# yardenas/ethz-safe-learning

Measured on AMD Instinct MI355X. Metric: planning steps/sec (CEM-MPC, N=2000 K=5 H=30), higher is better.
Workload: dtype f32

## Files before the change

### ethz_safe_learning_amd/_capi.py

```python
from __future__ import annotations

import ctypes as C
import os

CEM_ABI_VERSION = 4
CEM_MAX_ACT = 32
CEM_MAX_COST_KINDS = 4
CEM_COMM_ID_BYTES = 128
CEM_MAX_BATCH = 256
CEM_TRAIN_MAX_BATCH = 4096
CEM_INIT_COLD, CEM_INIT_EXPLICIT, CEM_INIT_SHIFT = 0, 1, 2
CEM_VARIANT_CEM, CEM_VARIANT_SAFE, CEM_VARIANT_COST = 0, 1, 2
CEM_PARTICLES_MEAN, CEM_PARTICLES_LOWER_TAIL = 0, 1
CEM_CONSTRAINT_BETA, CEM_CONSTRAINT_BUDGET = 0, 1
CEM_REFIT_UNIFORM, CEM_REFIT_SOFTMAX = 0, 1
CEM_NOISE_WHITE, CEM_NOISE_MIXED = 0, 1
CEM_FORWARD_SPLIT, CEM_FORWARD_ALL = 0, 1
CEM_TASK_SAFETY_GYM, CEM_TASK_QUADRATIC = 0, 1

_HERE = os.path.dirname(os.path.abspath(__file__))
LIB_PATH = os.environ.get('CEM_MPC_LIB') or os.path.join(_HERE, 'lib', 'libcem_mpc_gfx950.so')

EXPORTED_SYMBOLS = [
    'cem_abi_version', 'cem_status_string', 'cem_last_hip_error', 'cem_weight_blob_floats',
    'cem_packed_weight_floats', 'cem_workspace_bytes', 'cem_pack_weights_host', 'cem_plan_tiles_host', 'cem_plan_segments_host', 'cem_rollout_residency',
    'cem_planner_create', 'cem_planner_destroy', 'cem_planner_layout', 'cem_planner_set_weights', 'cem_planner_set_weights_dev',
    'cem_planner_set_normaliser', 'cem_planner_plan', 'cem_plan_begin', 'cem_plan_rollout', 'cem_plan_select',
    'cem_plan_end', 'cem_comm_unique_id', 'cem_planner_comm_init', 'cem_planner_comm_destroy', 'cem_planner_comm_ranks', 'cem_plan_exchange', 'cem_planner_graph_status', 'cem_planner_graph_nodes', 'cem_planner_launches_per_iteration', 'cem_planner_rollout_path', 'cem_planner_rollout_form', 'cem_unfold_sequences', 'cem_compute_objective', 'cem_scorer_reward', 'cem_scorer_cost', 'cem_fill_noise', 'cem_philox_words', 'cem_planner_set_timing', 'cem_planner_last_timing', 'cem_planner_last_timing_detail', 'cem_planner_select_mode', 'cem_planner_inject_fault',
    'cem_batch_workspace_bytes', 'cem_batch_planner_create', 'cem_planner_plan_batch', 'cem_planner_batch_capacity',
    'cem_planner_set_warm_start', 'cem_planner_set_initial_distribution', 'cem_planner_set_init_mode', 'cem_planner_reset_carry',
    'cem_planner_get_carry', 'cem_planner_set_carry_slots', 'cem_planner_set_particle_objective', 'cem_planner_get_particle_objective',
    'cem_planner_set_constraint', 'cem_planner_get_constraint', 'cem_planner_set_cost_budget', 'cem_planner_constraint_costs',
    'cem_planner_set_refit', 'cem_planner_get_refit', 'cem_planner_refit_stats',
    'cem_planner_set_action_noise', 'cem_planner_get_action_noise', 'cem_planner_action_noise_dev',
    'cem_planner_set_elite_carry', 'cem_planner_get_elite_carry', 'cem_planner_elite_store',
    'cem_planner_set_population_schedule', 'cem_planner_get_population_schedule', 'cem_planner_iteration_plan',
    'cem_planner_set_mean_candidate', 'cem_planner_get_mean_candidate',
    'cem_planner_set_plan_readout', 'cem_planner_get_plan_readout', 'cem_planner_plan_readout',
    'cem_planner_set_task', 'cem_planner_task_trajectories', 'cem_task_score',
    'cem_trainer_workspace_bytes', 'cem_trainer_blob_floats', 'cem_trainer_create', 'cem_trainer_destroy', 'cem_trainer_set_state',
    'cem_trainer_get_state', 'cem_trainer_weights_dev', 'cem_trainer_step', 'cem_trainer_steps', 'cem_trainer_eval', 'cem_trainer_forward',
]


class CemScorer(C.Structure):
    _fields_ = [
        ('goal_mode', C.c_int32), ('goal_lo', C.c_int32), ('goal_hi', C.c_int32),
        ('lidar_max_dist', C.c_float), ('goal_size', C.c_float), ('goal_reached_dist', C.c_float), ('reward_distance', C.c_float),
        ('reward_goal', C.c_float), ('reward_clip', C.c_float),
        ('constrain_indicator', C.c_int32), ('n_cost_kinds', C.c_int32),
        ('cost_lo', C.c_int32 * CEM_MAX_COST_KINDS), ('cost_hi', C.c_int32 * CEM_MAX_COST_KINDS),
        ('cost_size', C.c_float * CEM_MAX_COST_KINDS),
    ]


class CemConfig(C.Structure):
    _fields_ = [
        ('abi_version', C.c_int32), ('obs_dim', C.c_int32), ('act_dim', C.c_int32),
        ('units', C.c_int32), ('n_layers', C.c_int32), ('activation', C.c_int32), ('ensemble_size', C.c_int32),
        ('particles', C.c_int32), ('n_samples', C.c_int32), ('horizon', C.c_int32),
        ('n_elite', C.c_int32), ('iterations', C.c_int32),
        ('smoothing', C.c_float), ('one_minus_smoothing', C.c_float), ('stddev_threshold', C.c_float), ('noise_stddev', C.c_float),
        ('variant', C.c_int32), ('posterior_mean_threashold', C.c_float),
        ('sampling_propagation', C.c_int32), ('scale_features', C.c_int32),
        ('act_lb', C.c_float * CEM_MAX_ACT), ('act_ub', C.c_float * CEM_MAX_ACT),
        ('act_mu0', C.c_float * CEM_MAX_ACT), ('act_sigma0', C.c_float * CEM_MAX_ACT),
        ('scorer', CemScorer),
        ('world_size', C.c_int32), ('rank', C.c_int32), ('chunks_per_tile', C.c_int32), ('use_graph', C.c_int32),
        ('select_mode', C.c_int32), ('rollout_segments', C.c_int32), ('precision', C.c_int32),
    ]


class CemTrainConfig(C.Structure):
    _fields_ = [('abi_version', C.c_int32), ('inputs_dim', C.c_int32), ('outputs_dim', C.c_int32), ('units', C.c_int32),
                ('n_layers', C.c_int32), ('ensemble_size', C.c_int32), ('batch_size', C.c_int32), ('activation', C.c_int32),
                ('dropout_rate', C.c_float), ('dropout_seed_lo', C.c_uint32), ('dropout_seed_hi', C.c_uint32),
                ('beta1', C.c_float), ('beta2', C.c_float), ('epsilon', C.c_float), ('clipvalue', C.c_float)]


class CemWarmStart(C.Structure):
    _fields_ = [('shift', C.c_int32), ('tail', C.c_int32), ('sigma_rule', C.c_int32), ('sigma_floor', C.c_float * CEM_MAX_ACT)]


class CemEliteCarry(C.Structure):
    _fields_ = [('n_keep', C.c_int32), ('across_plans', C.c_int32), ('shift', C.c_int32), ('reserved', C.c_int32)]


class CemIterationPlan(C.Structure):
    _fields_ = [(n, C.c_int32) for n in ('n_samples', 'chunks_per_tile', 'n_tiles', 'n_segments', 'n_pinned', 'launches', 'rollout_path', 'reserved')]


class CemPlanReadout(C.Structure):
    _fields_ = [('score', C.c_float), ('candidate', C.c_int32), ('iteration', C.c_int32), ('flags', C.c_int32)]


class CemTask(C.Structure):
    _fields_ = [('kind', C.c_int32)] + [(n, C.POINTER(C.c_float)) for n in ('q', 'g', 'c', 'goal_mask', 'lo', 'hi', 'rho')] + \
               [('goal_radius', C.c_float), ('reward_goal', C.c_float), ('reward_clip', C.c_float)]


class CemLayout(C.Structure):
    _fields_ = [(n, C.c_size_t) for n in
                ('scores_local', 'scores_global', 'actions', 'mu_sigma', 'elite_idx', 'returns', 'costs', 'result', 'stamps', 'total',
                 'wpack', 'wpack_bytes', 'bias_h', 'bias_mu', 'bias_var', 'etab', 'etab_bytes')]


class CemError(RuntimeError):
    def __init__(self, status, where, lib=None):
        msg = lib.cem_status_string(status).decode() if lib is not None else str(status)
        hip = lib.cem_last_hip_error() if lib is not None else 0
        super().__init__('%s failed: status %d (%s)%s' % (where, status, msg, (', hip error %d' % hip) if status == 5 else ''))
        self.status = status


_lib = None


def load():
    global _lib
    if _lib is not None:
        return _lib
    if not os.path.exists(LIB_PATH):
        raise ImportError('HIP extension %s is missing: run `python -c "import __graft_entry__ as g; g.build()"` '
                          'or `make -C ethz_safe_learning_amd/csrc`. There is no CPU fallback.' % LIB_PATH)
    import torch
    lib = C.CDLL(LIB_PATH)
    vp, fp, i32p = C.c_void_p, C.POINTER(C.c_float), C.POINTER(C.c_int32)
    cfgp = C.POINTER(CemConfig)
    lib.cem_abi_version.restype = C.c_int
    lib.cem_status_string.restype = C.c_char_p
    lib.cem_status_string.argtypes = [C.c_int]
    lib.cem_last_hip_error.restype = C.c_int
    for f in ('cem_weight_blob_floats', 'cem_packed_weight_floats', 'cem_workspace_bytes'):
        getattr(lib, f).restype = C.c_size_t
        getattr(lib, f).argtypes = [cfgp]
    lib.cem_pack_weights_host.argtypes = [cfgp, vp, vp]
    lib.cem_plan_tiles_host.argtypes = [cfgp, i32p, i32p, vp, C.c_int32]
    lib.cem_plan_segments_host.argtypes = [cfgp, i32p, i32p]
    lib.cem_rollout_residency.argtypes = [C.c_int32, C.c_int32, i32p, i32p]
    lib.cem_planner_create.argtypes = [cfgp, vp, C.c_size_t, vp, C.POINTER(vp)]
    lib.cem_planner_destroy.argtypes = [vp]
    lib.cem_planner_layout.argtypes = [vp, C.POINTER(CemLayout)]
    lib.cem_planner_set_weights.argtypes = [vp, vp, C.c_size_t]
    lib.cem_planner_set_weights_dev.argtypes = [vp, vp, C.c_size_t]
    lib.cem_planner_set_normaliser.argtypes = [vp, vp, vp]
    lib.cem_planner_plan.argtypes = [vp, vp, C.c_uint64, C.c_uint64, vp, vp, vp, vp, fp, i32p]
    lib.cem_plan_begin.argtypes = [vp, vp, C.c_uint64, C.c_uint64, vp, vp]
    lib.cem_plan_rollout.argtypes = [vp, C.c_int32]
    lib.cem_plan_select.argtypes = [vp, C.c_int32]
    lib.cem_plan_end.argtypes = [vp, vp, vp, fp, i32p]
    lib.cem_unfold_sequences.argtypes = [vp, vp, vp, C.c_int32, C.c_int32, vp, C.c_uint64, C.c_uint64, vp, vp, vp]
    lib.cem_comm_unique_id.argtypes = [vp]
    lib.cem_planner_comm_init.argtypes = [vp, vp, C.c_int32, C.c_int32]
    lib.cem_planner_comm_destroy.argtypes = [vp]
    lib.cem_plan_exchange.argtypes = [vp]
    lib.cem_planner_graph_status.argtypes = [vp, i32p]
    lib.cem_planner_graph_nodes.argtypes = [vp, i32p]
    lib.cem_planner_comm_ranks.argtypes = [vp, i32p]
    lib.cem_planner_launches_per_iteration.argtypes = [vp, i32p]
    lib.cem_planner_rollout_path.argtypes = [vp, i32p]
    lib.cem_planner_rollout_form.argtypes = [vp, C.c_int32, i32p]
    lib.cem_compute_objective.argtypes = [vp, vp, C.c_int32, C.c_int32, vp]
    lib.cem_scorer_reward.argtypes = [vp, vp, vp, C.c_int32, vp, vp]
    lib.cem_scorer_cost.argtypes = [vp, vp, C.c_int32, vp]
    lib.cem_fill_noise.argtypes = [vp, C.c_uint64, C.c_uint64, vp, vp, vp]
    lib.cem_philox_words.argtypes = [vp, C.c_uint64, C.c_uint64] + [C.c_uint32] * 6 + [vp]
    lib.cem_planner_select_mode.argtypes = [vp, i32p]
    lib.cem_planner_inject_fault.argtypes = [vp, C.c_int32]
    lib.cem_planner_set_timing.argtypes = [vp, C.c_int32]
    lib.cem_planner_last_timing.argtypes = [vp, fp, i32p, fp]
    lib.cem_planner_last_timing_detail.argtypes = [vp, fp, fp]
    lib.cem_batch_workspace_bytes.restype = C.c_size_t
    lib.cem_batch_workspace_bytes.argtypes = [cfgp, C.c_int32]
    lib.cem_batch_planner_create.argtypes = [cfgp, C.c_int32, vp, C.c_size_t, vp, C.POINTER(vp)]
    lib.cem_planner_plan_batch.argtypes = [vp, C.c_int32, vp, C.c_uint64, vp, vp, vp, vp, vp, vp, vp]
    lib.cem_planner_batch_capacity.argtypes = [vp, i32p]
    lib.cem_planner_set_warm_start.argtypes = [vp, C.POINTER(CemWarmStart)]
    lib.cem_planner_set_initial_distribution.argtypes = [vp, C.c_int32, vp, vp]
    lib.cem_planner_set_init_mode.argtypes = [vp, C.c_int32, C.c_int32]
    lib.cem_planner_reset_carry.argtypes = [vp, C.c_int32]
    lib.cem_planner_get_carry.argtypes = [vp, C.c_int32, vp, vp, i32p]
    lib.cem_planner_set_carry_slots.argtypes = [vp, C.c_int32, vp]
    lib.cem_planner_set_particle_objective.argtypes = [vp, C.c_int32, C.c_int32]
    lib.cem_planner_get_particle_objective.argtypes = [vp, i32p, i32p]
    lib.cem_planner_set_constraint.argtypes = [vp, C.c_int32, C.c_int32]
    lib.cem_planner_get_constraint.argtypes = [vp, i32p, i32p]
    lib.cem_planner_set_cost_budget.argtypes = [vp, vp, C.c_int32]
    lib.cem_planner_constraint_costs.argtypes = [vp, C.c_int32, vp, C.c_int32]
    lib.cem_planner_set_refit.argtypes = [vp, C.c_int32, C.c_float]
    lib.cem_planner_get_refit.argtypes = [vp, i32p, fp]
    lib.cem_planner_refit_stats.argtypes = [vp, C.c_int32, vp, C.c_int32]
    lib.cem_planner_set_action_noise.argtypes = [vp, C.c_int32, vp]
    lib.cem_planner_get_action_noise.argtypes = [vp, i32p, vp]
    lib.cem_planner_action_noise_dev.argtypes = [vp, C.POINTER(vp), C.POINTER(C.c_size_t)]
    lib.cem_planner_set_elite_carry.argtypes = [vp, C.POINTER(CemEliteCarry)]
    lib.cem_planner_get_elite_carry.argtypes = [vp, C.POINTER(CemEliteCarry)]
    lib.cem_planner_elite_store.argtypes = [vp, C.c_int32, vp, i32p]
    lib.cem_planner_set_population_schedule.argtypes = [vp, i32p, C.c_int32]
    lib.cem_planner_get_population_schedule.argtypes = [vp, i32p, C.c_int32, i32p]
    lib.cem_planner_iteration_plan.argtypes = [vp, C.c_int32, C.POINTER(CemIterationPlan)]
    lib.cem_planner_set_mean_candidate.argtypes = [vp, C.c_int32]
    lib.cem_planner_get_mean_candidate.argtypes = [vp, i32p]
    lib.cem_planner_set_plan_readout.argtypes = [vp, C.c_int32]
    lib.cem_planner_get_plan_readout.argtypes = [vp, i32p]
    lib.cem_planner_plan_readout.argtypes = [vp, C.c_int32, C.POINTER(CemPlanReadout), vp, vp, vp]
    lib.cem_planner_set_task.argtypes = [vp, C.POINTER(CemTask)]
    lib.cem_planner_task_trajectories.argtypes = [vp, vp]
    lib.cem_task_score.argtypes = [vp, vp, vp, C.c_int32, C.c_int32, vp, vp]
    tcfgp = C.POINTER(CemTrainConfig)
    for f in ('cem_trainer_workspace_bytes', 'cem_trainer_blob_floats'):
        getattr(lib, f).restype = C.c_size_t
        getattr(lib, f).argtypes = [tcfgp]
    lib.cem_trainer_create.argtypes = [tcfgp, vp, C.c_size_t, vp, C.POINTER(vp)]
    lib.cem_trainer_destroy.argtypes = [vp]
    lib.cem_trainer_set_state.argtypes = [vp, vp, vp, vp]
    lib.cem_trainer_get_state.argtypes = [vp, vp, vp, vp]
    lib.cem_trainer_weights_dev.argtypes = [vp, C.POINTER(vp), C.POINTER(C.c_size_t)]
    lib.cem_trainer_step.argtypes = [vp, vp, vp, vp, C.c_int32, C.c_int32, C.c_int32, C.c_float, vp]
    lib.cem_trainer_steps.argtypes = [vp, vp, vp, vp, C.c_int32, C.c_int32, vp, vp, vp, vp]
    lib.cem_trainer_eval.argtypes = [vp, vp, vp, C.c_int32, fp]
    lib.cem_trainer_forward.argtypes = [vp, vp, C.c_int32, C.c_int32, vp, C.c_uint64, C.c_uint64, vp, vp, vp, vp]
    for name in EXPORTED_SYMBOLS:
        fn = getattr(lib, name)
        if name not in ('cem_status_string', 'cem_weight_blob_floats', 'cem_packed_weight_floats', 'cem_workspace_bytes',
                        'cem_batch_workspace_bytes', 'cem_trainer_workspace_bytes', 'cem_trainer_blob_floats'):
            fn.restype = C.c_int
    if lib.cem_abi_version() != CEM_ABI_VERSION:
        raise ImportError('ABI mismatch: library %d, binding %d' % (lib.cem_abi_version(), CEM_ABI_VERSION))
    _lib = lib
    return lib


def check(status, where):
    if status != 0:
        raise CemError(status, where, _lib)
```

### ethz_safe_learning_amd/csrc/cem_capi.hip

```cpp
#include "cem_device.h"
#include "cem_rollout_lean.h"
#include "cem_score.h"
#include "cem_refit_weighted.h"
#include "cem_noise_mix.h"
#include "cem_elite_carry.h"
#include "cem_plan_readout.h"
#include "cem_task_score.h"
#include "cem_population.h"
#include "cem_train.h"
#include "cem_train_tile.h"
#include "cem_forward.h"
#include "cem_rollout_split.h"
#include "cem_rollout_bf16.h"
#include "cem_rollout_wide.h"
#include "cem_pack.h"
#include "../../include/cem_mpc.h"
#include "cem_plan_options.h"

#include <dlfcn.h>
#include <link.h>

#include <algorithm>
#include <atomic>
#include <chrono>
// ... 464 lines not shown
    pl.n_seg = (d.H + pl.seg_len - 1) / pl.seg_len;
    pl.n_pinned = pl.n_seg > 1 ? (pl.n_tiles / num_cus()) * num_cus() : pl.n_tiles;
    if (c->rollout_segments > 1 && pl.n_pinned == pl.n_tiles && pl.n_seg > 1) pl.n_pinned = 0;
    return pl;
}

Layout make_layout(const cem_config_t *c, const Dims &d, size_t max_tiles, int mb = 0)
{
    Layout l{}; size_t o = 0;
    const size_t nb = mb > 0 ? (size_t)mb : 1;
    auto take = [&](size_t bytes) { size_t r = o; o = align256(o + bytes); return r; };
    l.ctrl = take(nb * sizeof(CtrlBlock));
    l.musig = take(nb * 2 * d.H * d.A * 4);
    l.act_bounds = take(64 * 4);
    l.scores_local = take(nb * d.Nloc * 4);
    l.scores_global = d.W > 1 ? take((size_t)d.N * 4) : l.scores_local;
    l.actions = take(nb * d.N * d.H * d.A * 4);
    l.act_pad = take(nb * d.N * d.H * d.act_nq * 16);
    l.elite = take(nb * d.k * 4);
    l.returns = take(nb * d.Bloc * 4);
    l.costs = take(nb * d.H * d.Bloc);
    l.result = take(mb > 0 ? nb * CEM_RESULT_WORDS * 4 : 64 * 4);
    l.wpack = take(d.wide ? (size_t)d.E * (align256(d.nat_member_floats * 4) + wide_image_floats(d) * 4) : (size_t)d.E * d.member_stride_f4 * 16);
    l.bias_h = take((size_t)d.E * d.L * CEM_U * 4);
    l.bias_mu = take((size_t)d.E * CEM_U * 4);
    l.bias_var = take((size_t)d.E * CEM_U * 4);
    l.nmin = take(CEM_U * 4);
    l.ndelta = take(CEM_U * 4);
    l.omask = take(2 * CEM_U * 4);
    l.kind_sel = take(CEM_NKIND * CEM_U * 4);
    l.etab = take((size_t)d.E * etab_rows(d) * CEM_U * 4);
    l.tiles = take(max_tiles * sizeof(TileDesc));
    l.eps_out = take(nb * CEM_MAX_ACT * 4);
    l.stamps = take(std::max<size_t>(max_tiles * 4 * 8, 128) * sizeof(long long));
    const Plan pl = make_plan(c, d);
    l.seg_queue = take(256);
    const size_t n_float = (size_t)(pl.n_tiles - pl.n_pinned);
    l.seg_flags = take(std::max<size_t>(n_float * std::max(pl.n_seg - 1, 1), 1) * 4);
    l.seg_state = take(pl.n_seg > 1 ? std::max<size_t>(n_float, 1) * (2 * d.NFW * pl.rc * 256 + 64) * 16 : 16);
    const size_t msG = ((size_t)d.N + CEM_MS_KEYS - 1) / CEM_MS_KEYS, msG2 = ((size_t)d.k + CEM_MS_EPG - 1) / CEM_MS_EPG;
    l.ms_hist = take(3 * CEM_MS_BINS * 4); l.ms_sel = take(256);
    l.ms_counts = take(msG * 2 * 4); l.ms_best_sc = take(msG * 4); l.ms_best_ix = take(msG * 4);
    l.ms_part = take(2 * msG2 * (size_t)d.H * d.A * 4); l.ms_colmean = take((size_t)d.H * d.A * 4);
    l.carry = take(nb * 2 * d.H * d.A * 4); l.expl = take(nb * 2 * d.H * d.A * 4);
    l.total = o;
    return l;
}

size_t max_tiles_of(const Dims &d) { std::vector<Tile6> t; build_plan_tiles(d, 1, t); return t.size(); }

int validate_batch(const cem_config_t *c, int32_t mb)
{
    const int st = validate(c); if (st) return st;
    if (mb < 1 || mb > CEM_MAX_BATCH) return CEM_ERR_INVALID_ARG;
    if (c->world_size > 1 || c->precision != CEM_PRECISION_FP32) return CEM_ERR_UNSUPPORTED;
    const Dims d = make_dims(c);
    if (d.wide) return CEM_ERR_UNSUPPORTED;
    if (c->select_mode == 2 || c->select_mode == 3) return CEM_ERR_UNSUPPORTED;
    if (resolve_select_mode(c->select_mode, d.N, d.k, (long long)d.H * d.A, 140 * 1024, true, nullptr) != 1) return CEM_ERR_UNSUPPORTED;
    if ((long long)mb * (long long)max_tiles_of(d) > 0x7fffffffll) return CEM_ERR_UNSUPPORTED;
    return CEM_OK;
}

}

namespace {
struct CemNcclId { char internal[CEM_COMM_ID_BYTES]; };
struct Rccl {
    void *lib = nullptr;
    int (*GetUniqueId)(CemNcclId *) = nullptr;
    int (*CommInitRank)(void **, int, CemNcclId, int) = nullptr;
    int (*CommDestroy)(void *) = nullptr;
    int (*AllGather)(const void *, void *, size_t, int, void *, hipStream_t) = nullptr;
    int (*CommCount)(void *, int *) = nullptr;
};
Rccl *rccl()
{
    static Rccl r;
    static std::once_flag once;
    std::call_once(once, [] {
        if (const char *over = std::getenv("CEM_RCCL_LIBRARY")) {
            r.lib = dlopen(over, RTLD_NOW | RTLD_LOCAL);
            if (!r.lib) std::fprintf(stderr, "cem_mpc: CEM_RCCL_LIBRARY=%s: %s\n", over, dlerror());
        } else {
            for (const char *name : {"librccl.so.1", "librccl.so", "/opt/rocm/lib/librccl.so.1"}) {
                r.lib = dlopen(name, RTLD_NOW | RTLD_LOCAL);
                if (r.lib) break;
            }
        }
        if (r.lib) {
            r.GetUniqueId = (decltype(r.GetUniqueId))dlsym(r.lib, "ncclGetUniqueId");
            r.CommInitRank = (decltype(r.CommInitRank))dlsym(r.lib, "ncclCommInitRank");
            r.CommDestroy = (decltype(r.CommDestroy))dlsym(r.lib, "ncclCommDestroy");
            r.AllGather = (decltype(r.AllGather))dlsym(r.lib, "ncclAllGather");
            r.CommCount = (decltype(r.CommCount))dlsym(r.lib, "ncclCommCount");
            if (!r.GetUniqueId || !r.CommInitRank || !r.CommDestroy || !r.AllGather) r.lib = nullptr;
        }
        if (const char *over = std::getenv("CEM_RCCL_LIBRARY"))
            std::fprintf(stderr, r.lib ? "cem_mpc: RCCL entry points bound from CEM_RCCL_LIBRARY=%s%s\n" : "cem_mpc: CEM_RCCL_LIBRARY=%s lacks a required entry point%s\n",
                         over, (r.lib && !r.CommCount) ? " (no ncclCommCount: cem_planner_comm_ranks unavailable)" : "");
    });
    return r.lib ? &r : nullptr;
}
const int kNcclFloat32 = 7;
}
#define NCCLCHK(x) do { int e_ = (x); if (e_ != 0) { g_last_hip = e_; return CEM_ERR_COMM; } } while (0)

namespace {
int count_hip_runtimes(struct dl_phdr_info *info, size_t, void *data)
{
    if (info->dlpi_name && std::strstr(info->dlpi_name, "libamdhip64")) {
        auto *v = static_cast<std::vector<std::string> *>(data);
        if (std::find(v->begin(), v->end(), std::string(info->dlpi_name)) == v->end()) v->push_back(info->dlpi_name);
    }
    return 0;
}
void warn_if_two_hip_runtimes()
{
    static std::once_flag once;
    std::call_once(once, [] {
        std::vector<std::string> libs;
        dl_iterate_phdr(count_hip_runtimes, &libs);
        if (libs.size() > 1) {
            std::fprintf(stderr, "cem_mpc: %zu HIP runtimes are loaded in this process:", libs.size());
            for (const auto &l : libs) std::fprintf(stderr, " %s", l.c_str());
            std::fprintf(stderr, "\ncem_mpc: device memory and streams of one are foreign to the other — load libcem_mpc_gfx950.so AFTER the runtime that owns them (INTEGRATION.md)\n");
        }
    });
}
}

struct IterPlan {
    Dims d;
    int rc, n_tiles, n_seg, seg_len, n_pinned;
    bool sample_in_rollout, lean_rollout;
    size_t tiles_off;
};

struct cem_planner {
    cem_config_t cfg;
    Dims d;
    Layout lay;
    char *ws;
    hipStream_t stream;
    bool own_stream;
    int rc;
    int n_tiles;
    int n_seg, seg_len, n_pinned;
    bool have_weights;
    bool in_plan;
    bool sample_in_rollout;
    bool lean_rollout;
    bool lean_branchy;
    const float *eps_act, *eps_model;
    CtrlBlock *h_ctrl;
    float *h_result;
    WarmCtl *h_warm; const WarmCtl *d_h_warm;
    uint32_t plan_seq;
    const CtrlBlock *d_h_ctrl; float *d_h_result;
    bool timing; std::vector<hipEvent_t> ev; float roll_ms, sel_ms, red_ms, samp_ms; int roll_n;
    std::vector<std::pair<int, int>> ev_kind;
    hipGraph_t graph; hipGraphExec_t gexec; bool graph_ready;
    ScorerDev sc;
    ScorerDev sc_roll;
    float alpha, beta;
    void *comm;
    int plans_since_comm;
    bool graph_failed;
    size_t sel_dyn_limit;
    int fused_resident;
    bool sel_zeroed;
    bool fuse_banned;
    bool inject_capture_fail;
    uint32_t inject_next;
    char *scratch; size_t scratch_bytes;
    std::vector<float> h_etab;
    PackDesc *pack_desc; uint32_t n_pack_desc;
    int batch;
    int n_states;
    cem_warm_start_t warm;
    std::vector<int32_t> slot_mode;
    std::vector<uint8_t> carry_valid, have_expl;
    std::vector<int32_t> carry_at;
    std::vector<int32_t> slot_of;
    bool warm_save_skipped;
    int warm_staged;
    std::vector<float> h_expl;
    PlanOptions opt;
    float *budget_dev;
    std::vector<float> h_budget;
    float *cstat_obj; size_t cstat_obj_n;
    const float *last_cstat; int last_cstat_n, last_cstat_problems;
    float refit_beta;
    float *refit_dev;
    bool refit_ran;
    std::vector<float> h_mix, h_mix_t;
    float *noise_dev;
    float *noise_eps; size_t noise_floats;
    float *elite_dev;
    int elite_cap;
    bool elite_clear;
    std::vector<IterPlan> pop;
    char *pop_dev;
    uint32_t *pop_seg_flags; f4 *pop_seg_state;
    int pop_n_ready;
    uint32_t *readout_dev;
    float *task_dev;
    TaskScoreParams task;
};

namespace {

int warm_slots(const cem_planner *h) { return h->batch ? h->batch : 1; }

struct IterView {
    const Dims *d; int rc, n_tiles, n_seg, seg_len, n_pinned; bool sample_in_rollout, lean_rollout;
    const TileDesc *tiles; uint32_t *seg_flags; f4 *seg_state;
};
IterView iter_view(const cem_planner *h, int it)
{
    const Layout &l = h->lay;
    if (h->pop.empty())
        return IterView{&h->d, h->rc, h->n_tiles, h->n_seg, h->seg_len, h->n_pinned, h->sample_in_rollout, h->lean_rollout,
                        (const TileDesc *)(h->ws + l.tiles), (uint32_t *)(h->ws + l.seg_flags), (f4 *)(h->ws + l.seg_state)};
    const IterPlan &ip = h->pop[std::min(std::max(it, 0), h->d.I - 1)];
    return IterView{&ip.d, ip.rc, ip.n_tiles, ip.n_seg, ip.seg_len, ip.n_pinned, ip.sample_in_rollout, ip.lean_rollout,
                    ip.tiles_off == (size_t)-1 ? (const TileDesc *)(h->ws + l.tiles) : (const TileDesc *)(h->pop_dev + ip.tiles_off),
                    h->pop_seg_flags, h->pop_seg_state};
}

int lean_form(const cem_planner *h, int it)
{
    const Dims &d = *iter_view(h, it).d; const ScorerDev &sc = h->sc_roll;
    bool straight = launch_rollout_lean_straight != nullptr && !h->lean_branchy && !sc.goal_mode && sc.n_cost <= 1 && d.L == 4 && d.NFW == 1;
    for (int w = 0; w < 4; ++w) straight = straight && d.wave_groups[w] == 4 + 3 * CEM_NG + (w < d.KB_obs ? CEM_NG : 0);
    return straight ? 2 : 1;
}
size_t task_tab_floats() { return (size_t)CEM_TASK_TABLES * CEM_U; }
float *task_traj(const cem_planner *h) { return h->task_dev + task_tab_floats(); }
int32_t *elite_counts(const cem_planner *h) { return reinterpret_cast<int32_t *>(h->elite_dev); }
size_t elite_count_floats(const cem_planner *h) { return ((size_t)warm_slots(h) + 63) & ~(size_t)63; }
float *elite_store(const cem_planner *h) { return h->elite_dev + elite_count_floats(h); }

int select_mode_for(const cem_planner *h, int N, bool *cache = nullptr)
{
    const Dims &d = h->d;
    const bool can_fuse = (N + CEM_MS_KEYS - 1) / CEM_MS_KEYS <= h->fused_resident && !h->fuse_banned;
    return resolve_select_mode(h->cfg.select_mode, N, d.k, (long long)d.H * d.A, h->sel_dyn_limit, can_fuse, cache);
}
int select_mode_now(const cem_planner *h, bool *cache = nullptr) { return select_mode_for(h, h->d.N, cache); }

void drop_graph(cem_planner *h)
{
    if (h->gexec) { hipGraphExecDestroy(h->gexec); h->gexec = nullptr; }
    if (h->graph) { hipGraphDestroy(h->graph); h->graph = nullptr; }
    h->graph_ready = false;
}

struct LaunchRecipe {
    bool sampler_launch;
    bool inject_elites, inject_mean;
    int lean_form;
    bool fold_reduce;
    int select_mode; bool select_cache;
    bool one_workgroup_only;
    bool weighted, keep_elites, track;
    bool task;
};
LaunchRecipe recipe_of(const cem_planner *h, int it, bool own_noise)
{
    const IterView v = iter_view(h, it); const PlanOptions &o = h->opt;
    LaunchRecipe r{};
    r.inject_elites = o.elite.n_keep != 0;
    r.inject_mean = o.mean_cand && it == h->d.I - 1;
    r.task = o.task != 0;
    const bool rewritten = r.inject_elites || r.inject_mean || r.task;
    r.sampler_launch = !v.sample_in_rollout || rewritten;
    r.lean_form = v.lean_rollout && !rewritten && !own_noise && o.noise_kind != CEM_NOISE_MIXED ? lean_form(h, it) : 0;
    r.select_mode = select_mode_for(h, v.d->N, &r.select_cache);
    r.fold_reduce = h->d.W == 1 && !h->comm && h->cfg.variant == CEM_VARIANT_CEM && !o.tail_m && r.select_mode == 1 && r.select_cache;
    r.weighted = o.refit_kind == CEM_REFIT_SOFTMAX; r.keep_elites = o.elite.n_keep != 0; r.track = o.readout != 0;
    r.one_workgroup_only = r.weighted || r.keep_elites || r.track || !h->pop.empty();
    return r;
}

int launches_of(const cem_planner *h, int it)
{
    const LaunchRecipe r = recipe_of(h, it, false);
    return 1 + r.sampler_launch + r.inject_elites + r.inject_mean + !r.fold_reduce + (r.select_mode == 2 ? 8 : r.select_mode == 3 ? 2 : 1) +
           r.weighted + r.keep_elites + r.track + r.task;
}

PlanOptions options_of(const cem_planner *h) { PlanOptions o = h->opt; o.comm = h->comm != nullptr; return o; }

constexpr long long kBudgetTotalLimit = 1ll << 23;

HandleFacts facts_of(const cem_planner *h, const PlanOptions &next)
{
    const Dims &d = h->d;
    HandleFacts f;
    f.W = d.W; f.batch = h->batch; f.variant = h->cfg.variant; f.N = d.N; f.k = d.k; f.H = d.H; f.A = d.A; f.I = d.I; f.P = d.P;
    f.select_mode = select_mode_now(h);
    for (int32_t n : next.pop) f.pop_select_mode.push_back(select_mode_for(h, n));
    f.tail_max_p = CEM_TAIL_MAX_P; f.budget_max_tail_p = CEM_BUDGET_MAX_TAIL_P; f.elite_max_k = CEM_ELITE_MAX_K; f.mix_max_h = CEM_MIX_MAX_H;
    f.readout_max_p = CEM_READOUT_MAX_P; f.max_cost_kinds = CEM_MAX_COST_KINDS; f.budget_total_limit = kBudgetTotalLimit;
    f.refit_lds_bytes = CEM_REFIT_LDS_BYTES(d.k, d.H * d.A); f.refit_lds_limit = h->sel_dyn_limit;
    f.can_mix = launch_mix_action_noise && prepare_mix_action_noise; f.can_carry = launch_elite_keep && launch_elite_inject;
    f.can_mean = launch_mean_candidate != nullptr; f.can_track = launch_plan_track != nullptr; f.can_task = launch_task_score != nullptr;
    return f;
}
int admit_on(const cem_planner *h, const PlanOptions &next, PlanChange change = PLAN_CHANGE_OTHER) { return admit(facts_of(h, next), next, change); }

template <typename SwapIn>
int commit_launch_change(cem_planner *h, PlanOptions &next, bool always, SwapIn swap_in)
{
    if (always || h->graph_ready) HIPCHK(hipStreamSynchronize(h->stream));
    if (const int st = swap_in()) return st;
    drop_graph(h);
    h->opt = std::move(next);
    return CEM_OK;
}
int commit_launch_change(cem_planner *h, PlanOptions &next, bool always) { return commit_launch_change(h, next, always, [] { return (int)CEM_OK; }); }

struct DevBlock {
    void *p = nullptr;
    DevBlock() = default;
    DevBlock(const DevBlock &) = delete; DevBlock &operator=(const DevBlock &) = delete;
    ~DevBlock() { if (p) hipFree(p); }
    hipError_t alloc(size_t bytes) { return hipMalloc(&p, bytes); }
    template <typename T> T *release() { T *q = static_cast<T *>(p); p = nullptr; return q; }
};

void release_handle(cem_planner *h)
{
    if (h->h_ctrl) hipHostFree(h->h_ctrl);
    if (h->h_result) hipHostFree(h->h_result);
    if (h->h_warm) hipHostFree(h->h_warm);
    if (h->pack_desc) hipFree(h->pack_desc);
    if (h->budget_dev) hipFree(h->budget_dev);
    if (h->refit_dev) hipFree(h->refit_dev);
    if (h->noise_dev) hipFree(h->noise_dev);
    if (h->elite_dev) hipFree(h->elite_dev);
    if (h->readout_dev) hipFree(h->readout_dev);
    if (h->task_dev) hipFree(h->task_dev);
    if (h->pop_dev) hipFree(h->pop_dev);
    if (h->cstat_obj) hipFree(h->cstat_obj);
    if (h->own_stream) hipStreamDestroy(h->stream);
    delete h;
}

}

extern "C" {

int cem_abi_version(void) { return CEM_ABI_VERSION; }
int cem_last_hip_error(void) { return g_last_hip; }

const char *cem_status_string(int s)
{
    switch (s) {
    case CEM_OK: return "ok";
    case CEM_ERR_INVALID_ARG: return "invalid argument";
    case CEM_ERR_UNSUPPORTED: return "unsupported configuration (units <= 256, obs+act <= 128, task 'goal')";
    case CEM_ERR_SPLIT: return "particles*n_samples is not divisible by ensemble_size (tf.split would raise)";
    case CEM_ERR_WORKSPACE: return "workspace too small or misaligned";
    case CEM_ERR_HIP: return "HIP runtime error (see cem_last_hip_error)";
    case CEM_ERR_NO_WEIGHTS: return "set_weights has not been called";
    case CEM_ERR_STATE: return "stepwise plan calls out of order, or a standalone call while a plan is in flight";
    case CEM_ERR_COMM: return "RCCL: library not found or a collective call failed (see cem_last_hip_error for the ncclResult_t)";
    case CEM_ERR_DEVICE: return "a kernel could not finish its work (a floating rollout segment starved of its work-queue entry, or an expired fused-select barrier whose recovery did not run): result not valid";
    default: return "unknown status";
    }
}

size_t cem_weight_blob_floats(const cem_config_t *cfg)
{
    if (validate(cfg) != CEM_OK) return 0;
    const Dims d = make_dims(cfg);
    return d.nat_member_floats * d.E;
}

size_t cem_packed_weight_floats(const cem_config_t *cfg)
{
    if (validate(cfg) != CEM_OK) return 0;
    const Dims d = make_dims(cfg);
    if (d.wide) return 0;
    return (size_t)d.member_stride_f4 * 4 * d.E;
}

size_t cem_workspace_bytes(const cem_config_t *cfg)
{
    if (validate(cfg) != CEM_OK) return 0;
    const Dims d = make_dims(cfg);
    return make_layout(cfg, d, max_tiles_of(d)).total;
}

int cem_pack_weights_host(const cem_config_t *cfg, const float *blob, float *packed)
{
    int st = validate(cfg); if (st) return st;
    if (!blob || !packed) return CEM_ERR_INVALID_ARG;
    const Dims d = make_dims(cfg);
    if (d.wide) return CEM_ERR_UNSUPPORTED;
    for (int m = 0; m < d.E; ++m) {
        if (d.chunked()) pack_member_chunked(d, blob + (size_t)m * d.nat_member_floats, reinterpret_cast<uint16_t *>(packed + (size_t)m * d.member_stride_f4 * 4));
        else pack_member(d, blob + (size_t)m * d.nat_member_floats, packed + (size_t)m * d.member_stride_f4 * 4);
    }
    return CEM_OK;
}

int cem_plan_tiles_host(const cem_config_t *cfg, int32_t *rc_out, int32_t *n_tiles_out, int32_t *tiles_out, int32_t max_tiles)
{
    int st = validate(cfg); if (st) return st;
    const Dims d = make_dims(cfg);
    const int rc = make_plan(cfg, d).rc;
    std::vector<Tile6> t; build_plan_tiles(d, rc, t);
    if (rc_out) *rc_out = rc;
    if (n_tiles_out) *n_tiles_out = (int32_t)t.size();
    if (tiles_out) {
        if ((int)t.size() > max_tiles) return CEM_ERR_INVALID_ARG;
        std::memcpy(tiles_out, t.data(), t.size() * sizeof(Tile6));
    }
    return CEM_OK;
}

int cem_plan_segments_host(const cem_config_t *cfg, int32_t *segments_out, int32_t *steps_per_segment_out)
{
    int st = validate(cfg); if (st) return st;
    const Dims d = make_dims(cfg);
    const Plan pl = make_plan(cfg, d);
    if (segments_out) *segments_out = pl.n_seg;
    if (steps_per_segment_out) *steps_per_segment_out = pl.seg_len;
    return CEM_OK;
}

int cem_rollout_residency(int32_t chunks_per_tile, int32_t input_blocks_per_wave, int32_t *table_out, int32_t *runtime_out)
{
    if (chunks_per_tile < 1 || chunks_per_tile > 4 || input_blocks_per_wave < 1 || input_blocks_per_wave > 2) return CEM_ERR_INVALID_ARG;
    for (int seg = 0; seg < 2; ++seg) {
        if (table_out) table_out[seg] = kResidentStatic[seg][input_blocks_per_wave - 1][chunks_per_tile - 1];
        if (runtime_out)
            runtime_out[seg] = with_tile_shape(chunks_per_tile, input_blocks_per_wave, 0, [&](auto R, auto F) { return query_resident<R(), F()>(seg != 0); });
    }
    return CEM_OK;
}

}

static bool lean_eligible(const cem_planner *h, const Dims &d, int rc, bool sample_in_rollout)
{
    return launch_rollout_lean != nullptr && !d.wide && !d.chunked() && rc == 1 && d.NFW == 1 && d.L == 4 && d.O % 4 == 0 && h->cfg.world_size == 1 && !h->batch &&
           sample_in_rollout && CEM_LEAN_ACT_LDS_BYTES(d.H, (d.A + 3) / 4) <= CEM_LEAN_ACT_LDS_MAX;
}

static void place_sampler(const cem_planner *h, const Dims &d, const Plan &pl, bool *sample_in_rollout, bool *lean_rollout)
{
    const size_t nb = (size_t)warm_slots(h);
    const int slots = real_cus() * ((d.wide || d.chunked()) ? 1 : resident_workgroups(d.NFW, pl.rc, pl.n_seg > 1));
    *sample_in_rollout = (long long)nb * pl.n_tiles <= slots;
    if (const char *e = std::getenv("CEM_FORCE_SAMPLER"))
        *sample_in_rollout = std::strcmp(e, "kernel") != 0;
    *lean_rollout = lean_eligible(h, d, pl.rc, *sample_in_rollout);
    if (const char *e = std::getenv("CEM_FORCE_ROLLOUT"))
        *lean_rollout = *lean_rollout && std::strcmp(e, "generic") != 0;
}

static int planner_create(const cem_config_t *cfg, int32_t mb, void *workspace, size_t workspace_bytes, void *hip_stream, cem_planner_t **out)
{
    int st = mb ? validate_batch(cfg, mb) : validate(cfg); if (st) return st;
    if (!workspace || !out) return CEM_ERR_INVALID_ARG;
    if (cfg->precision == CEM_PRECISION_BF16 && (launch_rollout_bf16 == nullptr || launch_pack_bf16 == nullptr)) return CEM_ERR_UNSUPPORTED;
    warn_if_two_hip_runtimes();
    cem_planner *h = new (std::nothrow) cem_planner();
    if (!h) return CEM_ERR_INVALID_ARG;
    h->cfg = *cfg; h->d = make_dims(cfg);
    h->batch = mb; h->n_states = warm_slots(h);
    const size_t nb = (size_t)warm_slots(h);
    h->lay = make_layout(cfg, h->d, max_tiles_of(h->d), mb);
    if (workspace_bytes < h->lay.total || ((uintptr_t)workspace & 255)) { delete h; return CEM_ERR_WORKSPACE; }
    h->ws = (char *)workspace; h->stream = (hipStream_t)hip_stream; h->own_stream = false;
    if (!h->stream) {
        if (hipStreamCreateWithFlags(&h->stream, hipStreamNonBlocking) != hipSuccess) { g_last_hip = (int)hipGetLastError(); delete h; return CEM_ERR_HIP; }
        h->own_stream = true;
    }
    { const Plan pl = make_plan(cfg, h->d, mb); h->rc = pl.rc; h->n_seg = pl.n_seg; h->seg_len = pl.seg_len; h->n_pinned = pl.n_pinned;
      place_sampler(h, h->d, pl, &h->sample_in_rollout, &h->lean_rollout); }
    { const char *e = std::getenv("CEM_FORCE_ROLLOUT"); h->lean_branchy = e && std::strcmp(e, "lean_branchy") == 0; }
    h->have_weights = false; h->in_plan = false; h->eps_act = h->eps_model = nullptr;
    h->timing = false; h->roll_ms = h->sel_ms = h->red_ms = h->samp_ms = 0.f; h->roll_n = 0;
    h->graph = nullptr; h->gexec = nullptr; h->graph_ready = false;
    h->budget_dev = nullptr; h->cstat_obj = nullptr; h->cstat_obj_n = 0; h->last_cstat = nullptr; h->last_cstat_n = h->last_cstat_problems = 0;
    h->refit_beta = 0.f; h->refit_dev = nullptr; h->refit_ran = false;
    h->noise_dev = nullptr; h->noise_eps = nullptr; h->noise_floats = 0;
    h->elite_dev = nullptr; h->elite_cap = 0; h->elite_clear = false;
    h->readout_dev = nullptr;
    h->task_dev = nullptr; h->task = TaskScoreParams{};
    h->pop_dev = nullptr; h->pop_seg_flags = nullptr; h->pop_seg_state = nullptr; h->pop_n_ready = 0;
    h->h_budget.assign(nb, std::numeric_limits<float>::infinity());
    h->comm = nullptr; h->plans_since_comm = 0; h->graph_failed = false;
    h->h_ctrl = nullptr; h->h_result = nullptr; h->h_warm = nullptr; h->d_h_warm = nullptr; h->pack_desc = nullptr; h->n_pack_desc = 0;
    h->warm = cem_warm_start_t{}; h->warm.shift = 1; h->warm_staged = 0; h->warm_save_skipped = false;
    h->slot_mode.assign(nb, CEM_INIT_COLD); h->carry_valid.assign(nb, 0); h->have_expl.assign(nb, 0); h->carry_at.assign(nb, -1);
    h->slot_of.resize(nb); for (size_t b = 0; b < nb; ++b) h->slot_of[b] = (int32_t)b;
    h->h_expl.assign(nb * 2 * h->d.H * h->d.A, 0.f);
    h->scratch = nullptr; h->scratch_bytes = 0; h->sel_zeroed = false; h->plan_seq = 0; h->fuse_banned = false; h->inject_next = 0; h->inject_capture_fail = false;
    auto fail = [&](int status) { g_last_hip = (int)hipGetLastError(); release_handle(h); return status; };
    const size_t result_bytes = mb ? nb * CEM_RESULT_WORDS * 4 : 64 * 4;
    if (hipHostMalloc((void **)&h->h_ctrl, nb * sizeof(CtrlBlock), hipHostMallocMapped | hipHostMallocCoherent) != hipSuccess ||
        hipHostMalloc((void **)&h->h_result, result_bytes, hipHostMallocMapped | hipHostMallocCoherent) != hipSuccess ||
        hipHostMalloc((void **)&h->h_warm, sizeof(WarmCtl) + nb * sizeof(WarmProb), hipHostMallocMapped | hipHostMallocCoherent) != hipSuccess) return fail(CEM_ERR_HIP);
    {
        const std::vector<PackDesc> table = build_pack_table(h->d);
        h->n_pack_desc = (uint32_t)table.size();
        const size_t image_bytes = h->d.wide ? wide_image_floats(h->d) * 4 : (size_t)h->d.member_stride_f4 * 16 - 4096;
        if (table.size() * (h->d.group_bytes() / 2) != image_bytes) return fail(CEM_ERR_STATE);
        if (hipMalloc((void **)&h->pack_desc, table.size() * sizeof(PackDesc)) != hipSuccess ||
            hipMemcpy(h->pack_desc, table.data(), table.size() * sizeof(PackDesc), hipMemcpyHostToDevice) != hipSuccess) return fail(CEM_ERR_HIP);
    }
    std::memset(h->h_warm, 0, sizeof(WarmCtl) + nb * sizeof(WarmProb));
    std::memset(h->h_ctrl, 0, nb * sizeof(CtrlBlock));
    std::memset(h->h_result, 0, result_bytes);
    {
        void *dc = nullptr, *dr = nullptr, *dw = nullptr;
        if (hipHostGetDevicePointer(&dc, h->h_ctrl, 0) != hipSuccess || hipHostGetDevicePointer(&dr, h->h_result, 0) != hipSuccess ||
            hipHostGetDevicePointer(&dw, h->h_warm, 0) != hipSuccess) return fail(CEM_ERR_HIP);
        h->d_h_ctrl = (const CtrlBlock *)dc; h->d_h_result = (float *)dr; h->d_h_warm = (const WarmCtl *)dw;
    }
    auto upload = [&](size_t off, const void *src, size_t bytes) {
        return hipMemcpyAsync(h->ws + off, src, bytes, hipMemcpyHostToDevice, h->stream) == hipSuccess;
    };

    const cem_scorer_t &s = cfg->scorer;
    ScorerDev &sc = h->sc;
    sc.goal_mode = s.goal_mode; sc.goal_lo = s.goal_lo; sc.goal_hi = s.goal_hi; sc.D = s.lidar_max_dist;
    sc.goal_thresh = s.goal_reached_dist;
    sc.reward_distance = s.reward_distance; sc.reward_goal = s.reward_goal; sc.reward_clip = s.reward_clip;
    sc.indicator = s.constrain_indicator; sc.n_cost = s.n_cost_kinds;
    for (int i = 0; i < 4; ++i) { sc.cost_lo[i] = s.cost_lo[i]; sc.cost_hi[i] = s.cost_hi[i]; sc.cost_size[i] = s.cost_size[i]; }
    h->sc_roll = sc;
    if (cfg->variant == CEM_VARIANT_COST) h->sc_roll.goal_thresh = -std::numeric_limits<float>::infinity();
    {
        const float mu = 0.5f, sg = 0.27f;
        const float alpha = (((1.0f - mu) / (sg * sg)) - 1.0f / mu) * (mu * mu);
        h->alpha = alpha; h->beta = alpha * (1.0f / mu - 1.0f);
    }

    std::vector<Tile6> tiles; build_plan_tiles(h->d, h->rc, tiles);
    h->n_tiles = (int)tiles.size();
    const Dims &d = h->d;
    std::vector<float> om(2 * CEM_U, 0.f), ks(CEM_NKIND * CEM_U, std::numeric_limits<float>::infinity());
    const float ninf = -std::numeric_limits<float>::infinity();
    for (int f = 0; f < CEM_U; ++f) {
        om[f] = f < d.O ? 1.f : 0.f;
        om[CEM_U + f] = (f >= d.O && f < d.O + d.A) ? 1.f : 0.f;
        const int ghi = s.goal_mode ? s.goal_lo + 1 : s.goal_hi;
        if (f >= s.goal_lo && f < ghi && f < d.O) ks[f] = ninf;
        for (int k = 0; k < s.n_cost_kinds; ++k)
            if (f >= s.cost_lo[k] && f < s.cost_hi[k] && f < d.O) ks[(k + 1) * CEM_U + f] = ninf;
    }
    std::vector<float> mn(CEM_U, 0.f), dl(CEM_U, 1.f);
    const size_t et_rows = etab_rows(d);
    h->h_etab.assign((size_t)d.E * et_rows * CEM_U, 0.f);
    for (int m = 0; m < d.E; ++m) {
        float *et = &h->h_etab[(size_t)m * et_rows * CEM_U];
        for (int f = 0; f < CEM_U; ++f) {
            et[CEM_ET_RDELTA * CEM_U + f] = 1.f;
            et[CEM_ET_OBS * CEM_U + f] = om[f]; et[CEM_ET_ACT * CEM_U + f] = om[CEM_U + f];
            et[CEM_ET_SEL0 * CEM_U + f] = ks[f]; et[CEM_ET_SEL1 * CEM_U + f] = ks[CEM_U + f];
        }
    }
    float bounds[64] = {0.f};
    for (int a = 0; a < d.A; ++a) { bounds[a] = cfg->act_lb[a]; bounds[32 + a] = cfg->act_ub[a]; }
    if (!upload(h->lay.act_bounds, bounds, sizeof(bounds)) ||
        !upload(h->lay.tiles, tiles.data(), tiles.size() * sizeof(Tile6)) || !upload(h->lay.omask, om.data(), om.size() * 4) ||
        !upload(h->lay.kind_sel, ks.data(), ks.size() * 4) || !upload(h->lay.nmin, mn.data(), CEM_U * 4) ||
        !upload(h->lay.ndelta, dl.data(), CEM_U * 4) || !upload(h->lay.etab, h->h_etab.data(), h->h_etab.size() * 4) ||
        hipMemsetAsync(h->ws + h->lay.act_pad, 0, nb * d.N * d.H * d.act_nq * 16, h->stream) != hipSuccess ||
        hipStreamSynchronize(h->stream) != hipSuccess)
        return fail(CEM_ERR_HIP);

    h->sel_dyn_limit = 48 * 1024;
    if (hipFuncSetAttribute(reinterpret_cast<const void *>(&cem_select_kernel<true, false>), hipFuncAttributeMaxDynamicSharedMemorySize,
                            140 * 1024) == hipSuccess &&
        hipFuncSetAttribute(reinterpret_cast<const void *>(&cem_select_kernel<true, true>), hipFuncAttributeMaxDynamicSharedMemorySize,
                            140 * 1024) == hipSuccess &&
        hipFuncSetAttribute(reinterpret_cast<const void *>(&cem_select_kernel<false, false>), hipFuncAttributeMaxDynamicSharedMemorySize,
                            140 * 1024) == hipSuccess) h->sel_dyn_limit = 140 * 1024;
    else (void)hipGetLastError();
    {
        int per_cu = 0;
        if (hipOccupancyMaxActiveBlocksPerMultiprocessor(&per_cu, cem_msel_fused_kernel, 1024, 0) != hipSuccess || per_cu < 1) { (void)hipGetLastError(); per_cu = 0; }
        h->fused_resident = per_cu * real_cus();
    }
    if (mb && select_mode_now(h) != 1) { release_handle(h); return CEM_ERR_UNSUPPORTED; }
    *out = h;
    return CEM_OK;
}

extern "C" {

int cem_planner_create(const cem_config_t *cfg, void *workspace, size_t workspace_bytes, void *hip_stream, cem_planner_t **out)
{
    return planner_create(cfg, 0, workspace, workspace_bytes, hip_stream, out);
}

size_t cem_batch_workspace_bytes(const cem_config_t *cfg, int32_t max_batch)
{
    if (validate_batch(cfg, max_batch) != CEM_OK) return 0;
    const Dims d = make_dims(cfg);
    return make_layout(cfg, d, max_tiles_of(d), max_batch).total;
}

int cem_batch_planner_create(const cem_config_t *cfg, int32_t max_batch, void *workspace, size_t workspace_bytes, void *hip_stream,
                             cem_planner_t **out)
{
    const int st = validate_batch(cfg, max_batch); if (st) return st;
    return planner_create(cfg, max_batch, workspace, workspace_bytes, hip_stream, out);
}

int cem_planner_batch_capacity(const cem_planner_t *h, int32_t *max_batch_out)
{
    if (!h || !max_batch_out) return CEM_ERR_INVALID_ARG;
    *max_batch_out = h->batch;
    return CEM_OK;
}

int cem_planner_destroy(cem_planner_t *h)
{
    if (!h) return CEM_ERR_INVALID_ARG;
    if (hipStreamSynchronize(h->stream) != hipSuccess) (void)hipGetLastError();
    if (h->scratch) hipFree(h->scratch);
    if (h->comm) { if (Rccl *r = rccl()) r->CommDestroy(h->comm); h->comm = nullptr; }
    drop_graph(h);
    for (auto e : h->ev) hipEventDestroy(e);
    release_handle(h);
    return CEM_OK;
}

int cem_planner_layout(const cem_planner_t *h, cem_layout_t *o)
{
// ... 168 lines not shown
    else hipLaunchKernelGGL(cem_rollout_wide_kernel<1>, dim3(n_tiles), dim3(256), CEM_WIDE_SMEM, h->stream, wp);
    return hipGetLastError();
}

void fill_rollout_common(const cem_planner *h, RolloutParams &p, const Dims *dv = nullptr)
{
    const Dims &d = dv ? *dv : h->d; const Layout &l = h->lay; char *ws = h->ws;
    std::memset(&p, 0, sizeof(p));
    p.wpack = (const f4 *)(ws + l.wpack); p.bias_h = (const float *)(ws + l.bias_h);
    p.bias_mu = (const float *)(ws + l.bias_mu); p.bias_var = (const float *)(ws + l.bias_var);
    p.nmin = (const float *)(ws + l.nmin); p.nrdelta = (const float *)(ws + l.ndelta);
    p.omask = (const float *)(ws + l.omask); p.kind_sel = (const float *)(ws + l.kind_sel);
    p.etab = (const float *)(ws + l.etab);
    p.act_pad = (const f4 *)(ws + l.act_pad); p.act_pad_bytes = (uint32_t)((size_t)d.N * d.H * d.act_nq * 16); p.act_q0 = d.act_q0; p.act_nq = d.act_nq;
    p.ctrl = (const CtrlBlock *)(ws + l.ctrl);
    p.member_stride_f4 = d.member_stride_f4;
    for (int w = 0; w < 4; ++w) { p.wave_off_f4[w] = d.wave_off_f4[w]; p.wave_groups[w] = (uint32_t)d.wave_groups[w]; }
    p.O = d.O; p.A = d.A; p.L = d.L; p.KB_in = d.KB_in; p.KB_obs = d.KB_obs;
    p.sampling = h->cfg.sampling_propagation; p.sc = h->sc_roll;
}

hipEvent_t get_event(cem_planner *h, size_t i)
{
    while (h->ev.size() <= i) { hipEvent_t e; hipEventCreate(&e); h->ev.push_back(e); }
    return h->ev[i];
}

struct TimedLaunch {
    cem_planner *h; size_t e0;
    TimedLaunch(cem_planner *h_, int kind) : h(h_->timing ? h_ : nullptr), e0(0)
    {
        if (!h) return;
        e0 = h->ev_kind.size() * 2; h->ev_kind.push_back({(int)e0, kind}); hipEventRecord(get_event(h, e0), h->stream);
    }
    void stop() { if (h) hipEventRecord(get_event(h, e0 + 1), h->stream); h = nullptr; }
    ~TimedLaunch() { stop(); }
};

void warm_handed_over(cem_planner *h);

int enqueue_begin(cem_planner *h)
{
    const Dims &d = h->d; const Layout &l = h->lay;
    InitParams ip{}; ip.ctrl = (CtrlBlock *)(h->ws + l.ctrl); ip.musig = (float *)(h->ws + l.musig); ip.HA = d.H * d.A; ip.A = d.A;
    ip.host_ctrl = h->d_h_ctrl;
    for (int a = 0; a < d.A; ++a) { ip.mu0[a] = h->cfg.act_mu0[a]; ip.sigma0[a] = h->cfg.act_sigma0[a]; }
    if (!h->pop.empty()) {
        if (h->pop_n_ready > 0) { ip.seg_queue = (uint32_t *)(h->ws + l.seg_queue); ip.seg_flags = h->pop_seg_flags; ip.n_ready = h->pop_n_ready; }
    } else
    if (h->n_seg > 1) { ip.seg_queue = (uint32_t *)(h->ws + l.seg_queue); ip.seg_flags = (uint32_t *)(h->ws + l.seg_flags); ip.n_ready = (h->n_tiles - h->n_pinned) * (h->n_seg - 1); }
    ip.n_prob = h->batch;
    ip.warm = h->d_h_warm; ip.carry = (float *)(h->ws + l.carry); ip.expl = (const float *)(h->ws + l.expl);
    const int n = warm_slots(h) * std::max<int>(ip.HA, (int)(sizeof(CtrlBlock) / 4));
    hipLaunchKernelGGL(cem_init_kernel, dim3((n + 255) / 256), dim3(256), 0, h->stream, ip);
    HIPCHK(hipGetLastError());
    if (h->opt.noise_kind == CEM_NOISE_MIXED && !h->eps_act) {
        MixParams mp{}; mp.mix_t = h->noise_dev; mp.eps = h->noise_eps; mp.ctrl = (const CtrlBlock *)(h->ws + l.ctrl);
        mp.I = d.I; mp.N = d.N; mp.H = d.H; mp.A = d.A;
        HIPCHK(launch_mix_action_noise(mp, warm_slots(h), h->stream));
    }
    {
        hipStreamCaptureStatus cs = hipStreamCaptureStatusNone;
        if (hipStreamIsCapturing(h->stream, &cs) != hipSuccess) { (void)hipGetLastError(); cs = hipStreamCaptureStatusNone; }
        if (cs == hipStreamCaptureStatusNone) warm_handed_over(h);
    }
    return CEM_OK;
}

void note_plan_cstat(cem_planner *h)
{
    const int nb = warm_slots(h);
    h->last_cstat = h->budget_dev + nb; h->last_cstat_n = h->d.Nloc; h->last_cstat_problems = nb;
}

ReduceParams fill_score(const cem_planner *h, const float *ret, const uint8_t *costs, float *scores, float *cstat, int Nloc, int H, int check_done, bool clear_select)
{
    ReduceParams p{}; p.ret = ret; p.costs = costs; p.scores = scores; p.ctrl = (const CtrlBlock *)(h->ws + h->lay.ctrl);
    p.Nloc = Nloc; p.P = h->d.P; p.H = H; p.variant = h->cfg.variant; p.check_done = check_done;
    p.alpha = h->alpha; p.beta = h->beta; p.thr = h->cfg.posterior_mean_threashold;
    if (clear_select) { p.zero = (uint32_t *)(h->ws + h->lay.ms_hist); p.zero_n = CEM_MS_CLEAR_BYTES / 4; }
    p.m = h->opt.cost_m ? h->opt.cost_m : h->opt.tail_m; p.cstat = cstat; p.budget = h->budget_dev;
    return p;
}

hipError_t launch_score(const cem_planner *h, const ReduceParams &p, int n_problems)
{
    const dim3 grid((p.Nloc + 63) / 64, n_problems), block(CEM_SCORE_THREADS);
    if (h->cfg.variant == CEM_VARIANT_COST) hipLaunchKernelGGL(cem_constraint_reduce_kernel, grid, block, 0, h->stream, p);
    else if (h->opt.cost_m) hipLaunchKernelGGL(cem_constrained_budget_kernel, grid, block, CEM_BUDGET_LDS_BYTES(p.P, p.m), h->stream, p);
    else if (h->opt.tail_m) hipLaunchKernelGGL(cem_constraint_tail_kernel, grid, block, CEM_TAIL_LDS_BYTES(p.P), h->stream, p);
    else hipLaunchKernelGGL(cem_reduce_kernel, grid, block, 0, h->stream, p);
    return hipGetLastError();
}

EliteCarryParams fill_elite(const cem_planner *h, int it)
{
    const IterView v = iter_view(h, it);
    const Dims &d = *v.d; const Layout &l = h->lay; char *ws = h->ws;
    EliteCarryParams ep{}; ep.scores = (const float *)(ws + l.scores_global); ep.actions = (float *)(ws + l.actions); ep.act_pad = (float *)(ws + l.act_pad);
    ep.ctrl = (const CtrlBlock *)(ws + l.ctrl); ep.elite_idx = (const int32_t *)(ws + l.elite); ep.store = elite_store(h); ep.count = elite_counts(h);
    ep.N = d.N; ep.k = d.k; ep.m = h->opt.elite.n_keep; ep.H = d.H; ep.A = d.A; ep.it = it; ep.shift = h->opt.elite.across_plans ? h->opt.elite.shift : 0;
    ep.pad_shift = d.O - 4 * d.act_q0; ep.pad_floats = 4 * d.act_nq;
    return ep;
}

int enqueue_rollout(cem_planner *h, int it, bool whole_plan)
{
    const LaunchRecipe rc = recipe_of(h, it, h->eps_act || h->eps_model);
    const IterView v = iter_view(h, it);
    const Dims &d = *v.d; const Layout &l = h->lay; char *ws = h->ws;
    const bool queued = v.n_seg > 1 && !h->eps_model && !rc.task;
    if (rc.task && !h->task_dev) return CEM_ERR_UNSUPPORTED;
    RolloutParams rp; fill_rollout_common(h, rp, v.d);
    rp.tiles = v.tiles; rp.s0 = nullptr; rp.actions = (const float *)(ws + l.actions);
    rp.eps_model = h->eps_model ? h->eps_model + (size_t)it * d.H * h->d.Btot * d.O : nullptr;
    const bool cost_obj = h->cfg.variant == CEM_VARIANT_COST;
    rp.ret = (float *)(ws + l.returns); rp.costs = h->cfg.variant != CEM_VARIANT_CEM ? (uint8_t *)(ws + l.costs) : nullptr;
    rp.H = d.H; rp.Bloc = d.Bloc; rp.Btot = d.Btot; rp.it = it; rp.variant = cost_obj ? (int)CEM_VARIANT_SAFE : h->cfg.variant; rp.check_done = 1;
    rp.stamps = (long long *)(ws + l.stamps);
    const float *eps_act = h->eps_act ? h->eps_act : (h->opt.noise_kind == CEM_NOISE_MIXED ? h->noise_eps : nullptr);
    rp.musig = (const float *)(ws + l.musig); rp.eps_act = eps_act ? eps_act + (size_t)it * h->d.N * d.H * d.A : nullptr;
    rp.act_bounds = (const float *)(ws + l.act_bounds); rp.actions_w = (float *)(ws + l.actions); rp.act_pad_w = (float *)(ws + l.act_pad);
    rp.pad_shift = d.O - 4 * d.act_q0; rp.pad_floats = 4 * d.act_nq; rp.N = d.N; rp.Nloc = d.Nloc; rp.n_off = d.n_off; rp.n_tiles = v.n_tiles;
    const int nb = warm_slots(h);
    rp.tiles_per_problem = h->batch ? v.n_tiles : 0;
    rp.eps_act_pstride = (long long)d.I * h->d.N * d.H * d.A; rp.eps_model_pstride = (long long)d.I * d.H * h->d.Btot * d.O;
    if (rc.sampler_launch) {
        const int total = d.N * d.H * ((d.A + 3) / 4);
        TimedLaunch timed(h, 3);
        hipLaunchKernelGGL(cem_sample_kernel, dim3(std::min((total + 255) / 256, 2048), nb), dim3(256), 0, h->stream, rp);
        HIPCHK(hipGetLastError());
        rp.musig = nullptr;
        if (rc.inject_elites && (it > 0 || h->opt.elite.across_plans)) {
            EliteCarryParams ep = fill_elite(h, it);
            HIPCHK(launch_elite_inject(ep, nb, h->stream));
        }
        if (rc.inject_mean) {
            MeanCandidateParams mc{}; mc.musig = (const float *)(ws + l.musig); mc.act_bounds = rp.act_bounds; mc.ctrl = rp.ctrl;
            mc.actions = rp.actions_w; mc.act_pad = rp.act_pad_w; mc.N = d.N; mc.row = d.N - 1; mc.H = d.H; mc.A = d.A;
            mc.pad_shift = rp.pad_shift; mc.pad_floats = rp.pad_floats;
            HIPCHK(launch_mean_candidate(mc, nb, h->stream));
        }
    }
    const bool mode1 = rp.eps_model || rc.task;
    if (rc.task) rp.traj = task_traj(h);
    TimedLaunch timed(h, 0);
    const auto queue_grid = [&] {
        rp.seg_queue = (uint32_t *)(ws + l.seg_queue); rp.seg_flags = v.seg_flags; rp.seg_state = v.seg_state;
        rp.seg_len = v.seg_len; rp.n_seg = v.n_seg; rp.n_pinned = v.n_pinned;
        return v.n_pinned + v.n_seg * (v.n_tiles - v.n_pinned);
    };
    if (rc.lean_form) {
        const int grid = queued ? queue_grid() : v.n_tiles;
        if (rc.lean_form == 2 && (rp.variant == 1) == (rp.costs != nullptr)) HIPCHK(launch_rollout_lean_straight(rp, grid, h->stream, queued));
        else HIPCHK(launch_rollout_lean(rp, grid, h->stream, queued));
    }
    else if (d.wide) HIPCHK(launch_rollout_wide(h, rp, v.n_tiles, mode1 ? 1 : 0));
    else if (d.chunked()) HIPCHK(launch_rollout_chunked(d, v.rc, mode1 ? 1 : 0, rp, v.n_tiles, h->stream));
    else if (mode1) HIPCHK(launch_rollout<1>(v.rc, d.NFW, rp, nb * v.n_tiles, h->stream));
    else if (queued) HIPCHK(launch_rollout_seg(v.rc, d.NFW, rp, queue_grid(), h->stream));
    else HIPCHK(launch_rollout<0>(v.rc, d.NFW, rp, nb * v.n_tiles, h->stream));
    timed.stop();
    if (rc.task) {
        TaskScoreParams tp = h->task;
        tp.traj = rp.traj; tp.actions = rp.actions; tp.ctrl = rp.ctrl; tp.ret = rp.ret; tp.costs = rp.costs;
        tp.rows = d.Bloc; tp.N = d.N; tp.H = d.H; tp.O = d.O; tp.A = d.A; tp.variant = rp.variant; tp.check_done = 1;
        if (cost_obj) tp.r2 = 0.f;
        TimedLaunch timed_task(h, 2);
        HIPCHK(launch_task_score(tp, h->stream));
    }
    if (whole_plan && rc.fold_reduce) return CEM_OK;

    const ReduceParams sp = fill_score(h, rp.ret, rp.costs, (float *)(ws + l.scores_local), h->opt.cost_m ? h->budget_dev + nb : nullptr, d.Nloc, d.H, 1, true);
    h->sel_zeroed = true;
    if (h->opt.cost_m) note_plan_cstat(h);
    TimedLaunch timed_reduce(h, 2);
    HIPCHK(launch_score(h, sp, nb));
    return CEM_OK;
}

int enqueue_select(cem_planner *h, int it, bool whole_plan, bool have_eps_out = false, bool *folded = nullptr)
{
    if (folded) *folded = false;
    const LaunchRecipe rc = recipe_of(h, it, h->eps_act || h->eps_model);
    const bool fold_reduce = whole_plan && rc.fold_reduce, fold_final = whole_plan;
    const Dims &d = *iter_view(h, it).d; const Layout &l = h->lay; char *ws = h->ws;
    SelectParams p{}; p.scores = (const float *)(ws + l.scores_global); p.actions = (const float *)(ws + l.actions);
    p.musig = (float *)(ws + l.musig); p.ctrl = (CtrlBlock *)(ws + l.ctrl); p.elite_idx = (int32_t *)(ws + l.elite);
    p.N = d.N; p.k = d.k; p.HA = d.H * d.A; p.A = d.A; p.check_done = 1;
    p.smoothing = h->cfg.smoothing; p.one_minus_smoothing = h->cfg.one_minus_smoothing; p.threshold = h->cfg.stddev_threshold;
    p.stamps = (long long *)(ws + l.stamps) + 64;
    if (fold_reduce) { p.ret = (const float *)(ws + l.returns); p.P = d.P; p.scores_w = (float *)(ws + l.scores_local); }
    size_t lds = (size_t)((d.k + 3) & ~3) * 4 + (size_t)2 * d.H * d.A * 4;
    const int G = (d.N + CEM_MS_KEYS - 1) / CEM_MS_KEYS;
    const int mode = rc.select_mode; const bool cache = rc.select_cache;
    if (mode == 0) return CEM_ERR_UNSUPPORTED;
    const bool weighted = rc.weighted;
    if (rc.one_workgroup_only && (mode != 1 || (weighted && !h->refit_dev) || (rc.keep_elites && !h->elite_dev) || (rc.track && !h->readout_dev))) return CEM_ERR_UNSUPPORTED;
    if (weighted) { p.musig = h->refit_dev; p.threshold = -std::numeric_limits<float>::infinity(); }
    TimedLaunch timed(h, 1);
    if (mode >= 2) {
        MSelParams m{}; m.scores = p.scores; m.actions = p.actions; m.musig = p.musig; m.ctrl = p.ctrl; m.elite_idx = p.elite_idx;
        m.hist = (uint32_t *)(ws + l.ms_hist); m.sel = (uint32_t *)(ws + l.ms_sel); m.wg_counts = (uint32_t *)(ws + l.ms_counts);
        m.bar = m.sel + 8;
        m.best_sc = (float *)(ws + l.ms_best_sc); m.best_ix = (int32_t *)(ws + l.ms_best_ix);
        m.part = (float *)(ws + l.ms_part); m.colmean = (float *)(ws + l.ms_colmean);
        m.N = d.N; m.k = d.k; m.HA = p.HA; m.A = d.A; m.check_done = 1; m.smoothing = p.smoothing; m.one_minus_smoothing = p.one_minus_smoothing; m.threshold = p.threshold;
        m.G = G; m.G2 = (d.k + CEM_MS_EPG - 1) / CEM_MS_EPG;
        if (!h->sel_zeroed) HIPCHK(hipMemsetAsync(m.hist, 0, CEM_MS_CLEAR_BYTES, h->stream));
        h->sel_zeroed = false;
        if (mode == 3) {
            hipLaunchKernelGGL(cem_msel_fused_kernel, dim3(m.G), dim3(1024), 0, h->stream, m);
            hipLaunchKernelGGL(cem_msel_solo_kernel, dim3(1), dim3(1024), 0, h->stream, m);
        } else {
            hipLaunchKernelGGL(cem_msel_hist_kernel<0>, dim3(m.G), dim3(1024), 0, h->stream, m);
            hipLaunchKernelGGL(cem_msel_hist_kernel<1>, dim3(m.G), dim3(1024), 0, h->stream, m);
            hipLaunchKernelGGL(cem_msel_hist_kernel<2>, dim3(m.G), dim3(1024), 0, h->stream, m);
            hipLaunchKernelGGL(cem_msel_count_kernel, dim3(m.G), dim3(1024), 0, h->stream, m);
            hipLaunchKernelGGL(cem_msel_compact_kernel, dim3(m.G), dim3(1024), 0, h->stream, m);
            hipLaunchKernelGGL(cem_msel_moments_kernel<0>, dim3(m.G2), dim3(256), 0, h->stream, m);
            hipLaunchKernelGGL(cem_msel_moments_kernel<1>, dim3(m.G2), dim3(256), 0, h->stream, m);
            hipLaunchKernelGGL(cem_msel_final_kernel, dim3(1), dim3(256), 0, h->stream, m);
        }
    } else {
        if (fold_final && !h->batch && !weighted) {
            p.is_last = it == d.I - 1;
            p.result = h->d_h_result; p.result_dev = (uint32_t *)(ws + l.result); p.eps_out = have_eps_out ? (const float *)(ws + l.eps_out) : nullptr; p.noise_stddev = h->cfg.noise_stddev;
            if (folded) *folded = true;
        }
        if (cache) lds += (size_t)CEM_SEL_KWORDS(d.N) * 4;
        const dim3 grid(warm_slots(h));
        if (cache && h->cfg.variant != CEM_VARIANT_CEM) hipLaunchKernelGGL((cem_select_kernel<true, true>), grid, dim3(1024), lds, h->stream, p);
        else if (cache) hipLaunchKernelGGL((cem_select_kernel<true, false>), grid, dim3(1024), lds, h->stream, p);
        else hipLaunchKernelGGL((cem_select_kernel<false, false>), grid, dim3(1024), lds, h->stream, p);
        if (weighted) {
            HIPCHK(hipGetLastError());
            RefitWeightedParams rw{}; rw.scores = p.scores; rw.actions = p.actions; rw.musig = (float *)(ws + l.musig); rw.ctrl = p.ctrl; rw.elite_idx = p.elite_idx;
            rw.stat = h->refit_dev + (size_t)warm_slots(h) * 2 * p.HA;
            rw.N = d.N; rw.k = d.k; rw.HA = p.HA; rw.I = d.I; rw.beta = h->refit_beta;
            rw.smoothing = p.smoothing; rw.one_minus_smoothing = p.one_minus_smoothing; rw.threshold = h->cfg.stddev_threshold;
            HIPCHK(launch_refit_weighted(rw, warm_slots(h), h->stream));
            h->refit_ran = true;
        }
        if (rc.keep_elites) {
            HIPCHK(hipGetLastError());
            const EliteCarryParams ep = fill_elite(h, it);
            HIPCHK(launch_elite_keep(ep, warm_slots(h), h->stream));
        }
        if (rc.track) {
            HIPCHK(hipGetLastError());
            PlanTrackParams tp{}; tp.scores = p.scores; tp.actions = p.actions; tp.ret = (const float *)(ws + l.returns);
            tp.costs = h->cfg.variant != CEM_VARIANT_CEM ? (const uint8_t *)(ws + l.costs) : nullptr;
            tp.ctrl = p.ctrl; tp.elite_idx = p.elite_idx; tp.block = h->readout_dev;
            tp.N = d.N; tp.k = d.k; tp.H = d.H; tp.A = d.A; tp.P = d.P; tp.it = it; tp.stride = (int32_t)CEM_READOUT_WORDS(h->d.H, h->d.A, h->d.P);
            HIPCHK(launch_plan_track(tp, warm_slots(h), h->stream));
        }
    }
    HIPCHK(hipGetLastError());
    return CEM_OK;
}

int enqueue_exchange(cem_planner *h)
{
    if (!h->comm) return CEM_OK;
    Rccl *r = rccl(); if (!r) return CEM_ERR_COMM;
    const Dims &d = h->d; const Layout &l = h->lay;
    NCCLCHK(r->AllGather(h->ws + l.scores_local, h->ws + l.scores_global, (size_t)d.Nloc, kNcclFloat32, h->comm, h->stream));
    return CEM_OK;
}

int enqueue_end(cem_planner *h, bool have_eps_out)
{
    const Dims &d = h->d; const Layout &l = h->lay; char *ws = h->ws;
    if (h->batch) {
        FinalBatchParams fb{}; fb.ctrl = (const CtrlBlock *)(ws + l.ctrl); fb.eps_out = have_eps_out ? (const float *)(ws + l.eps_out) : nullptr;
        fb.result = h->d_h_result; fb.result_dev = (uint32_t *)(ws + l.result); fb.A = d.A; fb.n_prob = h->batch; fb.noise_stddev = h->cfg.noise_stddev;
        hipLaunchKernelGGL(cem_final_batch_kernel, dim3(1), dim3(256), 0, h->stream, fb);
        HIPCHK(hipGetLastError());
        return CEM_OK;
    }
    FinalParams fp{}; fp.ctrl = (const CtrlBlock *)(ws + l.ctrl); fp.eps_out = have_eps_out ? (const float *)(ws + l.eps_out) : nullptr;
    fp.result = h->d_h_result; fp.result_dev = (uint32_t *)(ws + l.result); fp.A = d.A; fp.noise_stddev = h->cfg.noise_stddev;
    hipLaunchKernelGGL(cem_final_kernel, dim3(1), dim3(64), 0, h->stream, fp);
    HIPCHK(hipGetLastError());
    return CEM_OK;
}

void collect_timing(cem_planner *h)
{
    h->roll_ms = 0.f; h->sel_ms = 0.f; h->red_ms = 0.f; h->samp_ms = 0.f; h->roll_n = 0;
    for (auto &ek : h->ev_kind) {
        float ms = 0.f;
        if (hipEventElapsedTime(&ms, h->ev[ek.first], h->ev[ek.first + 1]) == hipSuccess) {
            if (ek.second == 0) { h->roll_ms += ms; h->roll_n++; }
            else if (ek.second == 1) h->sel_ms += ms;
            else if (ek.second == 2) h->red_ms += ms;
            else h->samp_ms += ms;
        }
    }
    h->ev_kind.clear();
}

bool finite_bits(float x) { uint32_t u; std::memcpy(&u, &x, 4); return (u & 0x7f800000u) != 0x7f800000u; }

int check_warm(const cem_planner *h, int n)
{
    for (int b = 0; b < n; ++b) {
// ... 696 lines not shown
    return commit_launch_change(h, next, false);
}

int cem_planner_get_mean_candidate(const cem_planner_t *h, int32_t *enable_out)
{
    if (!h || !enable_out) return CEM_ERR_INVALID_ARG;
    *enable_out = h->opt.mean_cand;
    return CEM_OK;
}

int cem_planner_set_initial_distribution(cem_planner_t *h, int32_t slot, const float *mu, const float *sigma)
{
    if (!h || !mu || !sigma || slot < 0 || slot >= warm_slots(h)) return CEM_ERR_INVALID_ARG;
    if (h->in_plan) return CEM_ERR_STATE;
    const size_t HA = (size_t)h->d.H * h->d.A;
    for (size_t i = 0; i < HA; ++i) if (!finite_bits(mu[i]) || !finite_bits(sigma[i]) || sigma[i] < 0.f) return CEM_ERR_INVALID_ARG;
    float *dst = h->h_expl.data() + (size_t)slot * 2 * HA;
    std::memcpy(dst, mu, HA * 4); std::memcpy(dst + HA, sigma, HA * 4);
    HIPCHK(hipMemcpyAsync(h->ws + h->lay.expl + (size_t)slot * 2 * HA * 4, dst, 2 * HA * 4, hipMemcpyHostToDevice, h->stream));
    h->have_expl[slot] = 1;
    return CEM_OK;
}

int cem_planner_set_init_mode(cem_planner_t *h, int32_t slot, int32_t mode)
{
    if (!h || slot < -1 || slot >= warm_slots(h)) return CEM_ERR_INVALID_ARG;
    if (mode != CEM_INIT_COLD && mode != CEM_INIT_EXPLICIT && mode != CEM_INIT_SHIFT) return CEM_ERR_INVALID_ARG;
    for (int s = 0; s < warm_slots(h); ++s) if (slot < 0 || s == slot) h->slot_mode[s] = mode;
    return CEM_OK;
}

int cem_planner_reset_carry(cem_planner_t *h, int32_t slot)
{
    if (!h || slot < -1 || slot >= warm_slots(h)) return CEM_ERR_INVALID_ARG;
    for (int s = 0; s < warm_slots(h); ++s) if (slot < 0 || s == slot) { h->carry_valid[s] = 0; h->carry_at[s] = -1; }
    if (h->elite_dev) HIPCHK(hipMemsetAsync(elite_counts(h) + (slot < 0 ? 0 : slot), 0, (size_t)(slot < 0 ? warm_slots(h) : 1) * 4, h->stream));
    return CEM_OK;
}

int cem_planner_get_carry(cem_planner_t *h, int32_t slot, float *mu, float *sigma, int32_t *valid)
{
    if (!h || slot < 0 || slot >= warm_slots(h)) return CEM_ERR_INVALID_ARG;
    const size_t HA = (size_t)h->d.H * h->d.A;
    if (h->in_plan) return CEM_ERR_STATE;
    const bool ok = h->carry_valid[slot] != 0;
    if (valid) *valid = ok ? 1 : 0;
    if (!ok) {
        if (mu) std::memset(mu, 0, HA * 4);
        if (sigma) std::memset(sigma, 0, HA * 4);
        return CEM_OK;
    }
    const char *src = h->carry_at[slot] >= 0 ? h->ws + h->lay.musig + (size_t)h->carry_at[slot] * 2 * HA * 4 : h->ws + h->lay.carry + (size_t)slot * 2 * HA * 4;
    if (mu) HIPCHK(hipMemcpyAsync(mu, src, HA * 4, hipMemcpyDeviceToHost, h->stream));
    if (sigma) HIPCHK(hipMemcpyAsync(sigma, src + HA * 4, HA * 4, hipMemcpyDeviceToHost, h->stream));
    HIPCHK(hipStreamSynchronize(h->stream));
    return CEM_OK;
}

int cem_planner_set_carry_slots(cem_planner_t *h, int32_t n, const int32_t *slots)
{
    if (!h) return CEM_ERR_INVALID_ARG;
    if (!h->batch) return CEM_ERR_STATE;
    if (n < 1 || n > h->batch) return CEM_ERR_INVALID_ARG;
    std::vector<int32_t> map(h->batch); std::vector<uint8_t> used(h->batch, 0);
    for (int b = 0; b < n; ++b) {
        const int32_t s = slots ? slots[b] : b;
        if (s < 0 || s >= h->batch || used[s]) return CEM_ERR_INVALID_ARG;
        used[s] = 1; map[b] = s;
    }
    for (int b = n, s = 0; b < h->batch; ++b) { while (used[s]) ++s; used[s] = 1; map[b] = s; }
    h->slot_of.swap(map);
    return CEM_OK;
}

int cem_comm_unique_id(void *id_out)
{
    if (!id_out) return CEM_ERR_INVALID_ARG;
    Rccl *r = rccl(); if (!r) return CEM_ERR_COMM;
    CemNcclId id;
    NCCLCHK(r->GetUniqueId(&id));
    std::memcpy(id_out, id.internal, CEM_COMM_ID_BYTES);
    return CEM_OK;
}

int cem_planner_comm_init(cem_planner_t *h, const void *id, int32_t n_ranks, int32_t rank)
{
    if (!h || !id) return CEM_ERR_INVALID_ARG;
    if (h->batch) return CEM_ERR_STATE;
    if (n_ranks != h->d.W || rank != h->d.R) return CEM_ERR_INVALID_ARG;
    if (h->in_plan) return CEM_ERR_STATE;
    PlanOptions next = options_of(h); next.comm = true;
    { const int st = admit_on(h, next); if (st) return st; }
    Rccl *r = rccl(); if (!r) return CEM_ERR_COMM;
    if (h->comm) { r->CommDestroy(h->comm); h->comm = nullptr; }
    CemNcclId nid; std::memcpy(nid.internal, id, CEM_COMM_ID_BYTES);
    void *comm = nullptr;
    NCCLCHK(r->CommInitRank(&comm, n_ranks, nid, rank));
    h->comm = comm; h->plans_since_comm = 0;
    drop_graph(h); h->graph_failed = false;
    return CEM_OK;
}

int cem_planner_comm_ranks(const cem_planner_t *h, int32_t *n_ranks_out)
{
    if (!h || !n_ranks_out) return CEM_ERR_INVALID_ARG;
    *n_ranks_out = 0;
    if (!h->comm) return CEM_OK;
    Rccl *r = rccl(); if (!r || !r->CommCount) return CEM_ERR_COMM;
    int n = 0;
    NCCLCHK(r->CommCount(h->comm, &n));
    *n_ranks_out = n;
    return CEM_OK;
}

int cem_planner_comm_destroy(cem_planner_t *h)
{
    if (!h) return CEM_ERR_INVALID_ARG;
    if (h->in_plan) return CEM_ERR_STATE;
    if (h->comm) {
        HIPCHK(hipStreamSynchronize(h->stream));
        if (Rccl *r = rccl()) r->CommDestroy(h->comm);
        h->comm = nullptr;
        drop_graph(h);
    }
    return CEM_OK;
}

int cem_planner_graph_status(const cem_planner_t *h, int32_t *status_out)
{
    if (!h || !status_out) return CEM_ERR_INVALID_ARG;
    *status_out = h->graph_ready ? 1 : (h->graph_failed ? 2 : 0);
    return CEM_OK;
}

int cem_planner_graph_nodes(const cem_planner_t *h, int32_t *nodes_out)
{
    if (!h || !nodes_out) return CEM_ERR_INVALID_ARG;
    size_t n = 0;
    if (h->graph_ready && h->graph) HIPCHK(hipGraphGetNodes(h->graph, nullptr, &n));
    *nodes_out = (int32_t)n;
    return CEM_OK;
}

int cem_planner_rollout_path(const cem_planner_t *h, int32_t *path_out)
{
    if (!h || !path_out) return CEM_ERR_INVALID_ARG;
    *path_out = recipe_of(h, 0, false).lean_form ? 1 : 0;
    return CEM_OK;
}

int cem_planner_rollout_form(const cem_planner_t *h, int32_t it, int32_t *form_out)
{
    if (!h || !form_out || it < 0 || it >= h->d.I) return CEM_ERR_INVALID_ARG;
    *form_out = recipe_of(h, it, false).lean_form;
    return CEM_OK;
}

int cem_planner_launches_per_iteration(const cem_planner_t *h, int32_t *launches_out)
{
    if (!h || !launches_out) return CEM_ERR_INVALID_ARG;
    *launches_out = launches_of(h, 0);
    return CEM_OK;
}

int cem_planner_iteration_plan(const cem_planner_t *h, int32_t it, cem_iteration_plan_t *out)
{
    if (!h || !out || it < 0 || it >= h->d.I) return CEM_ERR_INVALID_ARG;
    const IterView v = iter_view(h, it);
    out->n_samples = v.d->N; out->chunks_per_tile = v.rc; out->n_tiles = v.n_tiles; out->n_segments = v.n_seg; out->n_pinned = v.n_pinned;
    out->launches = launches_of(h, it);
    out->rollout_path = recipe_of(h, it, false).lean_form ? 1 : 0;
    out->reserved = 0;
    return CEM_OK;
}

int cem_plan_exchange(cem_planner_t *h)
{
    if (!h) return CEM_ERR_INVALID_ARG;
    if (!h->in_plan || !h->comm) return CEM_ERR_STATE;
    return enqueue_exchange(h);
}

static int ensure_scratch(cem_planner *h, size_t bytes)
{
    if (bytes <= h->scratch_bytes) return CEM_OK;
    if (h->scratch) { HIPCHK(hipStreamSynchronize(h->stream)); HIPCHK(hipFree(h->scratch)); h->scratch = nullptr; h->scratch_bytes = 0; }
    const size_t want = align256(bytes + bytes / 2);
    HIPCHK(hipMalloc((void **)&h->scratch, want));
    h->scratch_bytes = want;
    return CEM_OK;
}

static int upload_key(cem_planner *h, uint64_t seed, uint64_t call)
{
    CtrlBlock *c = h->h_ctrl;
    c->seed_lo = (uint32_t)seed; c->seed_hi = (uint32_t)(seed >> 32); c->call_lo = (uint32_t)call; c->call_hi = (uint32_t)(call >> 32);
    HIPCHK(hipMemcpyAsync(h->ws + h->lay.ctrl, c, 16, hipMemcpyHostToDevice, h->stream));
    return CEM_OK;
}

int cem_unfold_sequences(cem_planner_t *h, const float *s0_dev, const float *actions_dev, int32_t n_rows, int32_t horizon,
                         const float *eps_model_dev, uint64_t seed, uint64_t call, float *traj_out_dev, float *mu_out_dev, float *sd_out_dev)
{
    if (!h || !s0_dev || !actions_dev || n_rows < 1 || horizon < 1 || horizon > 65535) return CEM_ERR_INVALID_ARG;
    if (h->batch) return CEM_ERR_STATE;
    if (!h->have_weights) return CEM_ERR_NO_WEIGHTS;
    if (h->in_plan) return CEM_ERR_STATE;
    const Dims &d = h->d;
    if (n_rows % d.E != 0) return CEM_ERR_SPLIT;
    if ((long long)n_rows * (horizon + 1) * d.O > 0x7fffffff00ll) return CEM_ERR_UNSUPPORTED;
    const int chunk = n_rows / d.E;
    const int rc = d.wide ? 1 : (d.split() ? (n_rows >= 256 * 32 ? 2 : 1) : (n_rows >= 256 * 64 ? 4 : (n_rows >= 256 * 32 ? 2 : 1)));
    std::vector<Tile6> tiles;
    for (int m = 0; m < d.E; ++m)
        for (int r = m * chunk; r < (m + 1) * chunk; r += 16 * rc) {
            Tile6 t; t.v[0] = r; t.v[1] = std::min(16 * rc, (m + 1) * chunk - r); t.v[2] = m; t.v[3] = r; t.v[4] = r; t.v[5] = r;
            tiles.push_back(t);
        }
    const size_t tile_bytes = align256(tiles.size() * sizeof(Tile6));
    int st = ensure_scratch(h, tile_bytes + (size_t)n_rows * 4); if (st) return st;
    TileDesc *dt = (TileDesc *)h->scratch; float *ret = (float *)(h->scratch + tile_bytes);
    HIPCHK(hipMemcpyAsync(dt, tiles.data(), tiles.size() * sizeof(Tile6), hipMemcpyHostToDevice, h->stream));
    st = upload_key(h, seed, call); if (st) return st;
    RolloutParams rp; fill_rollout_common(h, rp);
    rp.tiles = dt; rp.s0 = s0_dev; rp.actions = actions_dev; rp.eps_model = eps_model_dev; rp.ret = ret; rp.costs = nullptr;
    rp.traj = traj_out_dev; rp.mu_out = mu_out_dev; rp.sd_out = sd_out_dev;
    rp.H = horizon; rp.Bloc = n_rows; rp.Btot = n_rows; rp.it = 0; rp.variant = 0; rp.check_done = 0;
    hipError_t e = d.wide ? launch_rollout_wide(h, rp, (int)tiles.size(), 1)
                 : d.chunked() ? launch_rollout_chunked(d, rc, 1, rp, (int)tiles.size(), h->stream)
                               : launch_rollout<1>(rc, d.NFW, rp, (int)tiles.size(), h->stream);
    hipError_t e2 = hipStreamSynchronize(h->stream);
    HIPCHK(e); HIPCHK(e2);
    return CEM_OK;
}

int cem_compute_objective(cem_planner_t *h, const float *traj_dev, int32_t n_rows, int32_t horizon, float *scores_out_dev)
{
    if (!h || !traj_dev || !scores_out_dev || n_rows < 1 || horizon < 1 || horizon > 65535) return CEM_ERR_INVALID_ARG;
    if (h->batch) return CEM_ERR_STATE;
    const Dims &d = h->d;
    if (n_rows % d.P != 0) return CEM_ERR_INVALID_ARG;
    if ((long long)n_rows * horizon > 0x7fffffffll) return CEM_ERR_UNSUPPORTED;
    const bool cost_obj = h->cfg.variant == CEM_VARIANT_COST;
    const bool safe = h->cfg.variant == CEM_VARIANT_SAFE || cost_obj;
    if (h->opt.cost_m && (long long)horizon * h->opt.cost_m * CEM_MAX_COST_KINDS >= kBudgetTotalLimit) return CEM_ERR_UNSUPPORTED;
    const size_t ret_bytes = align256((size_t)n_rows * 4);
    int st = ensure_scratch(h, ret_bytes + (safe ? (size_t)n_rows * horizon : 0)); if (st) return st;
    ObjectiveParams op{}; op.traj = traj_dev; op.ret = (float *)h->scratch; op.costs = safe ? (uint8_t *)(h->scratch + ret_bytes) : nullptr;
    op.B = n_rows; op.H = horizon; op.O = d.O; op.variant = safe ? (int)CEM_VARIANT_SAFE : h->cfg.variant; op.sc = h->sc_roll;
    hipLaunchKernelGGL(cem_objective_kernel, dim3((unsigned)(((size_t)n_rows * 16 + 255) / 256)), dim3(256), 0, h->stream, op);
    HIPCHK(hipGetLastError());
    const int n_cand = n_rows / d.P;
    if (h->opt.cost_m && (size_t)n_cand > h->cstat_obj_n) {
        if (h->cstat_obj) { HIPCHK(hipStreamSynchronize(h->stream)); HIPCHK(hipFree(h->cstat_obj)); h->cstat_obj = nullptr; h->cstat_obj_n = 0; if (h->last_cstat_problems == 0) h->last_cstat = nullptr; }
        const size_t want = (size_t)n_cand + (size_t)n_cand / 2;
        HIPCHK(hipMalloc((void **)&h->cstat_obj, want * 4));
        h->cstat_obj_n = want;
    }
    const ReduceParams sp = fill_score(h, op.ret, op.costs, scores_out_dev, h->opt.cost_m ? h->cstat_obj : nullptr, n_cand, horizon, 0, false);
    HIPCHK(launch_score(h, sp, 1));
    HIPCHK(hipStreamSynchronize(h->stream));
    if (h->opt.cost_m) { h->last_cstat = sp.cstat; h->last_cstat_n = n_cand; h->last_cstat_problems = 0; }
    return CEM_OK;
}

static int scorer_op(cem_planner *h, const float *obs, const float *next_obs, int32_t n, float *out, uint8_t *flag, int what)
{
    ScorerOpParams sp{}; sp.obs = obs; sp.next_obs = next_obs; sp.out = out; sp.flag = flag; sp.n = n; sp.O = h->d.O; sp.what = what; sp.sc = h->sc;
    hipLaunchKernelGGL(cem_scorer_kernel, dim3((unsigned)(((size_t)n * 16 + 255) / 256)), dim3(256), 0, h->stream, sp);
    HIPCHK(hipGetLastError());
    HIPCHK(hipStreamSynchronize(h->stream));
    return CEM_OK;
}

int cem_scorer_reward(cem_planner_t *h, const float *obs_dev, const float *next_obs_dev, int32_t n, float *reward_out_dev,
                      uint8_t *goal_achieved_out_dev)
{
    if (!h || !obs_dev || !next_obs_dev || !reward_out_dev || n < 1) return CEM_ERR_INVALID_ARG;
    if (h->batch) return CEM_ERR_STATE;
    return scorer_op(h, obs_dev, next_obs_dev, n, reward_out_dev, goal_achieved_out_dev, 0);
}

int cem_scorer_cost(cem_planner_t *h, const float *obs_dev, int32_t n, float *cost_out_dev)
{
    if (!h || !obs_dev || !cost_out_dev || n < 1) return CEM_ERR_INVALID_ARG;
    if (h->batch) return CEM_ERR_STATE;
    return scorer_op(h, obs_dev, nullptr, n, cost_out_dev, nullptr, 1);
}

int cem_fill_noise(cem_planner_t *h, uint64_t seed, uint64_t call, float *eps_act_dev, float *eps_model_dev, float *eps_out_dev)
{
    if (!h) return CEM_ERR_INVALID_ARG;
    if (h->in_plan) return CEM_ERR_STATE;
    const Dims &d = h->d;
    int st = upload_key(h, seed, call); if (st) return st;
    FillParams fp{}; fp.eps_act = eps_act_dev; fp.eps_model = eps_model_dev; fp.eps_out = eps_out_dev;
    fp.ctrl = (const CtrlBlock *)(h->ws + h->lay.ctrl); fp.I = d.I; fp.N = d.N; fp.H = d.H; fp.A = d.A; fp.B = d.Btot; fp.O = d.O;
    hipLaunchKernelGGL(cem_fill_noise_kernel, dim3(2048), dim3(256), 0, h->stream, fp);
    HIPCHK(hipGetLastError());
    HIPCHK(hipStreamSynchronize(h->stream));
    return CEM_OK;
}

int cem_philox_words(cem_planner_t *h, uint64_t seed, uint64_t call, uint32_t stream, uint32_t iteration, uint32_t t, uint32_t sub,
                     uint32_t idx0, uint32_t n, uint32_t *words_out_dev)
{
// ... 342 lines not shown
```

### ethz_safe_learning_amd/csrc/cem_rollout_lean.h

```cpp
#pragma once
#include "cem_device.h"

#define CEM_LEAN_ACT_LDS_BYTES(H_, AZ_) (((size_t)(H_) + 1) * (AZ_) * (32 + 17 * 16))
#define CEM_LEAN_LDS_BYTES(H_, AZ_) (CEM_ROLLOUT_LDS_BYTES(1) + CEM_LEAN_ACT_LDS_BYTES(H_, AZ_))
#define CEM_LEAN_ACT_LDS_MAX 16384

__attribute__((weak)) hipError_t launch_rollout_lean(const RolloutParams &p, int grid, hipStream_t st, bool seg);
__attribute__((weak)) hipError_t launch_rollout_lean_straight(const RolloutParams &p, int grid, hipStream_t st, bool seg);

template <int V> struct LeanConst { static constexpr int value = V; };
```

### ethz_safe_learning_amd/csrc/cem_rollout_lean.hip

```cpp
#define CEM_DEVICE_PRIMITIVES_ONLY
#include "cem_rollout_lean.h"

namespace {

template <int KF, int NOWN, bool L0IN>
__device__ __forceinline__ void cem_lean_stage(f4 (&acc0)[1], f4 (&acc1)[1], f4 (&hB)[CEM_NG][1], WRing &wq, const char *const *rb, const int xoff)
{
    static_assert(KF % 4 == 0, "stage lengths must keep the ring phase");
#pragma unroll
    for (int P = 0; P < KF; ++P) {
        wq.slot[(P + 3) & 3] = wq.ld(wq.pos);
        wq.pos = (wq.pos + 1 == wq.n) ? 0 : wq.pos + 1;
        __builtin_amdgcn_sched_barrier(0);
        if (P == 1) {
            __syncthreads();
#pragma unroll
            for (int Q = NOWN; Q < KF; ++Q) hB[Q][0] = *reinterpret_cast<const f4 *>(rb[Q - NOWN] + xoff + (Q - NOWN) * 1024);
        }
        const AGroup g = wq.slot[P & 3];
        const int Pb = (!L0IN && P < 2) ? (P ^ 1) : P;
#pragma unroll
        for (int r = 0; r < 4; ++r) {
            acc0[0] = CEM_MFMA(g.a[r], hB[P][0][r], acc0[0]);
            acc1[0] = CEM_MFMA(g.b[r], hB[Pb][0][r], acc1[0]);
        }
    }
}

#define CEM_LEAN_TILE_TEMPLATE template <bool SEG>
#define CEM_LEAN_TILE cem_lean_tile
#define CEM_LEAN_HANDOVER_DECL const int wbk = 0; const __amdgpu_buffer_rsrc_t seg_rs = CEM_LEAN_SEG_RSRC();
#define CEM_LEAN_BKWAVE (w == wbk)
#define CEM_LEAN_HANDOVER seg_rs
#define CEM_LEAN_RING WRing wq; wq.init(p.wpack + (size_t)member_u * p.member_stride_f4 + p.wave_off_f4[w], lane, (int)p.wave_groups[w]);
#define CEM_LEAN_STAGE(KF, NOWN, L0IN, BASE) cem_lean_stage<KF, NOWN, L0IN>
#define CEM_LEAN_BOOKS_DECL \
    const int nk = 1 + p.sc.n_cost; \
    const float csz[4] = {p.sc.cost_size[0], p.sc.cost_size[1], p.sc.cost_size[2], p.sc.cost_size[3]}; \
    const float ind_cap = p.sc.indicator ? 1.0f : __builtin_inff(), clipv = p.sc.reward_clip > 0.f ? p.sc.reward_clip : __builtin_inff(); \
    const __amdgpu_buffer_rsrc_t cost_rs = __builtin_amdgcn_make_buffer_rsrc(p.costs, 0, p.costs ? (uint32_t)(H * p.Bloc) : 0u, 0x00020000);
#define CEM_LEAN_SCORE_D p.sc.D
#define CEM_LEAN_STORE_TERMS CEM_RARE_KINDS_AND_STORE(RC, NFW, p, part, w, q, j, nk, s, pm, tab_v, CEM_SEL0_LDS, tabl)
#define CEM_LEAN_PRIO_DECL \
    const bool prio_rot = !(SEG && tile_idx >= p.n_pinned); \
    const int prio_r0 = (tile_idx >> 8) % 3;
#define CEM_LEAN_PRIO_STEP \
    if (prio_rot) { \
        const int lvl = (t + prio_r0) % 3; \
        if (lvl == 0) __builtin_amdgcn_s_setprio(0); else if (lvl == 1) __builtin_amdgcn_s_setprio(1); else __builtin_amdgcn_s_setprio(2); \
    }
#define CEM_LEAN_BOOKS_AT(T_) CEM_BOOKKEEP(p, td, part, w, wbk, lane, nk, csz, ind_cap, clipv, cost_rs, d_prev, c_prev, cum, done, T_);
#define CEM_LEAN_BOOKS_STEP if (!(resumed && first)) CEM_LEAN_BOOKS_AT(t - 1)
#define CEM_LEAN_BOOKS_END CEM_LEAN_BOOKS_AT(t_end - 1)
#define CEM_LEAN_HIDDEN_LAYERS _Pragma("unroll") for (int l = 1; l < 4; ++l) CEM_LEAN_HIDDEN(l + 1 < 4 ? l + 1 : 0, 0)
#define CEM_LEAN_HEADS (w < p.KB_obs)
#define CEM_LEAN_ISACT const f4 isact4 = CEM_TAB(tabl, CEM_ET_ACT, tv);
#define CEM_LEAN_NEXT_INPUT \
    f4 xin = sn; \
    if (wact) { \
        f4 act4; CEM_LEAN_ACTION(act4, e4, tn); \
        CEM_LEAN_KEEP(act4, t + 1); \
        xin = __builtin_elementwise_fma(isact4, act4, sn); \
    } \
    const f4 x = cem_sub4(xin, mn4) * rd4; \
    *reinterpret_cast<f4 *>(pub0 + xw) = x; \
    hB[0][0] = x;
#include "cem_rollout_lean_tile.h"
#undef CEM_LEAN_BOOKS_AT

}

__global__ __launch_bounds__(256) void cem_rollout_lean_kernel(const RolloutParams p)
{
    extern __shared__ __attribute__((aligned(16))) char smem[];
    if (p.check_done && p.ctrl->done) return;
    cem_lean_tile<false>(p, smem, (int)blockIdx.x, 0, p.H);
}

__global__ __launch_bounds__(256) void cem_rollout_lean_seg_kernel(const RolloutParams p)
{
    extern __shared__ __attribute__((aligned(16))) char smem[];
    __shared__ uint32_t item_s;
    if (p.check_done && p.ctrl->done) return;
    if ((int)blockIdx.x < p.n_pinned) {
        cem_lean_tile<true>(p, smem, (int)blockIdx.x, 0, p.H);
        return;
    }
    CEM_SEG_SCHEDULE(p, item_s, tile, seg, t0, t1, (cem_lean_tile<true>(p, smem, tile, t0, t1)))
}

hipError_t launch_rollout_lean(const RolloutParams &p, int grid, hipStream_t st, bool seg)
{
    const size_t lds = CEM_LEAN_LDS_BYTES(p.H, (p.A + 3) / 4);
    if (seg) hipLaunchKernelGGL(cem_rollout_lean_seg_kernel, dim3(grid), dim3(256), lds, st, p);
    else hipLaunchKernelGGL(cem_rollout_lean_kernel, dim3(grid), dim3(256), lds, st, p);
    return hipGetLastError();
}
```

### ethz_safe_learning_amd/csrc/cem_rollout_lean_straight.hip

```cpp
#define CEM_DEVICE_PRIMITIVES_ONLY
#include "cem_rollout_lean.h"

namespace {

constexpr int SL_GROUPS_BODY = 4 + 3 * CEM_NG, SL_GROUPS_HEADS = SL_GROUPS_BODY + CEM_NG;

struct StraightRing {
    __amdgpu_buffer_rsrc_t rsrc;
    int voff, n;
    AGroup slot[4];
    template <int G> __device__ __forceinline__ AGroup ld() const
    {
        const int g = G < SL_GROUPS_BODY ? G : (G >= n ? G - n : G);
        const int soff = (g >> 1) * 4096;
        constexpr int half = (G & 1) * 2048;
        AGroup r;
        r.a = __builtin_bit_cast(f4, __builtin_amdgcn_raw_buffer_load_b128(rsrc, voff + half, soff, 0));
        r.b = __builtin_bit_cast(f4, __builtin_amdgcn_raw_buffer_load_b128(rsrc, voff + half + 1024, soff, 0));
        return r;
    }
    __device__ __forceinline__ void init(const f4 *b, int lane_, int n_)
    {
        rsrc = __builtin_amdgcn_make_buffer_rsrc(const_cast<f4 *>(b), 0, n_ * 2048, 0x00020000);
        voff = lane_ * 16; n = n_;
        slot[0] = ld<0>(); slot[1] = ld<1>(); slot[2] = ld<2>(); slot[3] = slot[2];
    }
};

template <int KF, int NOWN, bool L0IN, int BASE>
__device__ __forceinline__ void cem_straight_stage(f4 (&acc0)[1], f4 (&acc1)[1], f4 (&hB)[CEM_NG][1], StraightRing &wq, const char *const *rb, const int xoff)
{
    static_assert(KF % 4 == 0 && BASE % 4 == 0, "stage lengths must keep the ring phase");
    auto group = [&](auto PC) __attribute__((always_inline)) {
        constexpr int P = decltype(PC)::value;
        wq.slot[(P + 3) & 3] = wq.template ld<BASE + P + 3>();
        __builtin_amdgcn_sched_barrier(0);
        if (P == 1) {
            __syncthreads();
#pragma unroll
            for (int Q = NOWN; Q < KF; ++Q) hB[Q][0] = *reinterpret_cast<const f4 *>(rb[Q - NOWN] + xoff + (Q - NOWN) * 1024);
        }
        const AGroup g = wq.slot[P & 3];
        constexpr int Pb = (!L0IN && P < 2) ? (P ^ 1) : P;
#pragma unroll
        for (int r = 0; r < 4; ++r) {
            acc0[0] = CEM_MFMA(g.a[r], hB[P][0][r], acc0[0]);
            acc1[0] = CEM_MFMA(g.b[r], hB[Pb][0][r], acc1[0]);
        }
    };
    group(LeanConst<0>{}); group(LeanConst<1>{}); group(LeanConst<2>{}); group(LeanConst<3>{});
    if constexpr (KF == 8) { group(LeanConst<4>{}); group(LeanConst<5>{}); group(LeanConst<6>{}); group(LeanConst<7>{}); }
}

#define CEM_LEAN_TILE_TEMPLATE template <bool SEG, bool SAFE>
#define CEM_LEAN_TILE cem_straight_tile
#define CEM_LEAN_BKWAVE bkwave
#define CEM_LEAN_HANDOVER_DECL const bool bkwave = w == 0; auto seg_buffer = [&]() __attribute__((always_inline)) { return CEM_LEAN_SEG_RSRC(); };
#define CEM_LEAN_HANDOVER seg_buffer()
#define CEM_LEAN_RING \
    const bool heads = w < p.KB_obs; \
    StraightRing wq; \
    wq.init(p.wpack + (size_t)member_u * p.member_stride_f4 + p.wave_off_f4[w], lane, heads ? SL_GROUPS_HEADS : SL_GROUPS_BODY);
#define CEM_LEAN_STAGE(KF, NOWN, L0IN, BASE) cem_straight_stage<KF, NOWN, L0IN, BASE>
#define CEM_LEAN_BOOKS_DECL \
    const float scD = p.sc.D, goal_thresh = p.sc.goal_thresh, reward_distance = p.sc.reward_distance, reward_goal = p.sc.reward_goal; \
    const float clipv = p.sc.reward_clip > 0.f ? p.sc.reward_clip : __builtin_inff(); \
    const float csz0 = p.sc.n_cost > 0 ? p.sc.cost_size[0] : -__builtin_inff(); \
    auto terms = [&](float &dn, float &cn) __attribute__((always_inline)) { \
        dn = CEM_PART_MIN4(part, lane, 0); \
        const float dk = CEM_PART_MIN4(part, lane, 1); \
        cn = (dk <= csz0) ? 1.0f : 0.0f;                       \
    }; \
    auto settle = [&](const float dn, const float cn, const int T) __attribute__((always_inline)) { \
        const bool ga = d_prev <= goal_thresh; \
        float r = (d_prev - dn) * reward_distance + (ga ? 1.0f : 0.0f) * reward_goal; \
        r = fminf(fmaxf(r, -clipv), clipv); \
        if (SAFE) { \
            done = done || ga; \
            const float nd = done ? 0.0f : 1.0f; \
            const float cst = c_prev * nd; \
            if (lane < td.cnt) { \
                const __amdgpu_buffer_rsrc_t cost_rs = __builtin_amdgcn_make_buffer_rsrc(p.costs, 0, (uint32_t)(H * p.Bloc), 0x00020000); \
                __builtin_amdgcn_raw_buffer_store_b8((uint8_t)cst, cost_rs, td.row_base + lane, __builtin_amdgcn_readfirstlane(T * p.Bloc), 0); \
            } \
            cum = cum + r * nd; \
        } else { \
            const float nd = done ? 0.0f : 1.0f; \
            cum = cum + r * nd; \
            done = done || ga; \
        } \
        d_prev = dn; c_prev = cn; \
    };
#define CEM_LEAN_SCORE_D scD
#define CEM_LEAN_STORE_TERMS CEM_PAIR_MIN_STORE(part, w, q, j, 0, pm[0][0], pm[1][0], true, 0)
#define CEM_LEAN_PRIO_DECL \
    static_assert(CEM_FLOAT_PRIO == 3, "level 3 of the step's priority switch is the floating segments' priority"); \
    int lvl = (SEG && tile_idx >= p.n_pinned) ? 3 : (t_begin + (tile_idx >> 8) % 3) % 3;
#define CEM_LEAN_PRIO_STEP \
    if (lvl < 2) { if (lvl == 0) __builtin_amdgcn_s_setprio(0); else __builtin_amdgcn_s_setprio(1); } \
    else { if (lvl == 2) __builtin_amdgcn_s_setprio(2); else __builtin_amdgcn_s_setprio(3); } \
    lvl = lvl == 2 ? 0 : (lvl == 3 ? 3 : lvl + 1); \
    asm volatile("" : "+s"(lvl));
#define CEM_LEAN_BOOKS_STEP \
    if (bkwave) { \
        if (first) { \
            if (!resumed) terms(d_prev, c_prev); \
        } else { \
            float dn, cn; \
            terms(dn, cn); \
            settle(dn, cn, t - 1); \
        } \
    }
#define CEM_LEAN_BOOKS_END \
    if (bkwave) { \
        float dn, cn; \
        terms(dn, cn); \
        settle(dn, cn, t_end - 1); \
    }
#define CEM_LEAN_HIDDEN_LAYERS CEM_LEAN_HIDDEN(2, 4) CEM_LEAN_HIDDEN(3, 12) CEM_LEAN_HIDDEN(0, 20)
#define CEM_LEAN_HEADS heads
#define CEM_LEAN_ISACT
#define CEM_LEAN_NEXT_INPUT \
    if (wact) { \
        const f4 isact4 = CEM_TAB(tabl, CEM_ET_ACT, tv); \
        f4 act4; CEM_LEAN_ACTION(act4, e4, tn); \
        CEM_LEAN_KEEP(act4, t + 1); \
        const f4 x = cem_sub4(__builtin_elementwise_fma(isact4, act4, sn), mn4) * rd4; \
        *reinterpret_cast<f4 *>(pub0 + xw) = x; \
        hB[0][0] = x; \
    } else { \
        const f4 x = cem_sub4(sn, mn4) * rd4; \
        *reinterpret_cast<f4 *>(pub0 + xw) = x; \
        hB[0][0] = x; \
    }
#include "cem_rollout_lean_tile.h"

}

template <bool SAFE>
__global__ __launch_bounds__(256) void cem_rollout_lean_straight_kernel(const RolloutParams p)
{
    extern __shared__ __attribute__((aligned(16))) char smem[];
    if (p.check_done && p.ctrl->done) return;
    cem_straight_tile<false, SAFE>(p, smem, (int)blockIdx.x, 0, p.H);
}

template <bool SAFE>
__global__ __launch_bounds__(256) void cem_rollout_lean_straight_seg_kernel(const RolloutParams p)
{
    extern __shared__ __attribute__((aligned(16))) char smem[];
    __shared__ uint32_t item_s;
    if (p.check_done && p.ctrl->done) return;
    if ((int)blockIdx.x < p.n_pinned) {
        cem_straight_tile<true, SAFE>(p, smem, (int)blockIdx.x, 0, p.H);
        return;
    }
    CEM_SEG_SCHEDULE(p, item_s, tile, seg, t0, t1, (cem_straight_tile<true, SAFE>(p, smem, tile, t0, t1)))
}

hipError_t launch_rollout_lean_straight(const RolloutParams &p, int grid, hipStream_t st, bool seg)
{
    const size_t lds = CEM_LEAN_LDS_BYTES(p.H, (p.A + 3) / 4);
    const bool safe = p.variant == 1;
    if (seg) {
        if (safe) hipLaunchKernelGGL(cem_rollout_lean_straight_seg_kernel<true>, dim3(grid), dim3(256), lds, st, p);
        else hipLaunchKernelGGL(cem_rollout_lean_straight_seg_kernel<false>, dim3(grid), dim3(256), lds, st, p);
    } else {
        if (safe) hipLaunchKernelGGL(cem_rollout_lean_straight_kernel<true>, dim3(grid), dim3(256), lds, st, p);
        else hipLaunchKernelGGL(cem_rollout_lean_straight_kernel<false>, dim3(grid), dim3(256), lds, st, p);
    }
    return hipGetLastError();
}
```

### ethz_safe_learning_amd/csrc/cem_rollout_lean_tile.h

```cpp

#define CEM_LEAN_SEG_RSRC() __builtin_amdgcn_make_buffer_rsrc( \
        SEG ? const_cast<f4 *>(p.seg_state + (size_t)(tile_idx - p.n_pinned) * (2 * 256 + 64)) : const_cast<f4 *>(p.wpack), 0, (2 * 256 + 64) * 16, 0x00020000)
CEM_LEAN_TILE_TEMPLATE
__device__ __forceinline__ void CEM_LEAN_TILE(const RolloutParams &p, char *smem, const int tile_idx, const int t_begin, const int t_end)
{
    constexpr int RC = 1, NFW = 1;
    const int tid = (int)((threadIdx.x + 64u * (unsigned)((tile_idx + (tile_idx >> 8)) & 3)) & 255u);
    const int w = __builtin_amdgcn_readfirstlane(tid >> 6);
    const int lane = tid & 63;
    const int j = lane & 15, q = lane >> 4;
    const TileDesc td = p.tiles[tile_idx];
    const bool resumed = SEG && t_begin > 0;
    CEM_LEAN_HANDOVER_DECL
    const int O = p.O, A = p.A, H = p.H, AZ = (A + 3) >> 2;
    constexpr int XB = CEM_NG * 1024;
    float *part = reinterpret_cast<float *>(smem + 2 * XB);
    const CtrlBlock *const ctrl = p.ctrl;
    const PhiloxKey key = cem_key(ctrl);
    const float rscale = p.sampling ? CEM_BM_RSCALE : 0.0f;

    const int member_u = __builtin_amdgcn_readfirstlane(td.member);
    CEM_LEAN_RING

    const __amdgpu_buffer_rsrc_t et_rs = __builtin_amdgcn_make_buffer_rsrc(
        const_cast<float *>(p.etab + (size_t)member_u * (CEM_ET_ROWS + p.L) * CEM_U), 0, (CEM_ET_ROWS + p.L) * CEM_U * 4, 0x00020000);
    const int tab_v = 64 * w + 16 * q;
    const int bias_v = 128 * w + 16 * q;
    const char *tabl = smem + 2 * XB + CEM_PART_FLOATS * 4;
    const char *actl = tabl + CEM_TAB_LDS_BYTES;
    {
        const int ht = (int)threadIdx.x;
        *reinterpret_cast<f4 *>(const_cast<char *>(tabl) + ht * 16) = cem_ld_tab(et_rs, (ht & 31) * 16, (ht >> 5) * 512);
        const int HA = H * A;
        for (int idx = ht; idx < (H + 1) * AZ; idx += 256) {
            const int t = idx / AZ, z = idx - t * AZ;
            const float *lo = t < H ? p.musig + HA + t * A : p.act_bounds, *hi = t < H ? p.musig + t * A : p.act_bounds + 32;
            f4 u = {0.f, 0.f, 0.f, 0.f}, v = u;
#pragma unroll
            for (int r = 0; r < 4; ++r) if (4 * z + r < A) { u[r] = lo[4 * z + r]; v[r] = hi[4 * z + r]; }
            *reinterpret_cast<f4 *>(const_cast<char *>(actl) + idx * 32) = u;
            *reinterpret_cast<f4 *>(const_cast<char *>(actl) + idx * 32 + 16) = v;
        }
    }
    __syncthreads();

    f4 s[NFW][RC];
    const int slot0 = j < td.cnt ? j : td.cnt - 1;
    {
        const int f0 = 16 * w + 4 * q;
        if (resumed) s[0][0] = cem_ld_coherent(CEM_LEAN_HANDOVER, tid * 16);
        else {
#pragma unroll
            for (int r = 0; r < 4; ++r) {
                const int f = f0 + r;
                float v = 0.f;
                if (f < O) v = td.s0_base < 0 ? ctrl->state[f] : p.s0[(size_t)(td.s0_base + slot0) * O + f];
                s[0][0][r] = v;
            }
        }
    }

    const int zq = 4 * w + q - (O >> 2);
    const bool actlane = zq >= 0 && zq < AZ;
    const bool wact = 4 * w + 3 >= (O >> 2) && 4 * w < (O >> 2) + AZ;
    const int zc = actlane ? zq : 0;
    const uint32_t pc0 = (uint32_t)((actlane ? td.act_base : td.noise_row_base) + slot0);
    const uint32_t pc2 = actlane ? ((uint32_t)zc | (CEM_STREAM_ACT << 16)) : ((uint32_t)(4 * w + q) | (CEM_STREAM_MODEL << 16));
    const uint32_t pc1 = ((uint32_t)p.it << 16) + (actlane ? 1u : 0u);
    const float prs = actlane ? CEM_BM_RSCALE : rscale;
    const char *const actl_v = actl + zc * 32;
#define CEM_LEAN_ACTION(DST, E_, T_) do { \
        const char *m_ = actl_v + (T_) * AZ * 32, *b_ = actl_v + H * AZ * 32; \
        const f4 sg_ = *reinterpret_cast<const f4 *>(m_), mu_ = *reinterpret_cast<const f4 *>(m_ + 16); \
        const f4 lb_ = *reinterpret_cast<const f4 *>(b_), ub_ = *reinterpret_cast<const f4 *>(b_ + 16); \
        f4 v_ = (E_) * sg_; v_ = v_ + mu_; \
        _Pragma("unroll") for (int r = 0; r < 4; ++r) DST[r] = fminf(fmaxf(v_[r], lb_[r]), ub_[r]); } while (0)
    const bool act_keep = actlane && j < td.cnt && td.row_base < p.Nloc;
    char *const stage = const_cast<char *>(actl) + (H + 1) * AZ * 32;
    char *const stage_v = stage + ((act_keep ? j : 16) * (H + 1) * AZ + zc) * 16;
#define CEM_LEAN_KEEP(V_, T_) do { *reinterpret_cast<f4 *>(stage_v + (T_) * AZ * 16) = (V_); } while (0)

    float d_prev = 0.f, c_prev = 0.f, cum = 0.f;
    bool done = false;
    CEM_LEAN_BOOKS_DECL

    f4 hB[CEM_NG][RC];
    if (resumed) {
        const __amdgpu_buffer_rsrc_t ho = CEM_LEAN_HANDOVER;
        const f4 x = cem_ld_coherent(ho, (256 + tid) * 16);
        hB[0][0] = x;
        *reinterpret_cast<f4 *>(smem + (w * 64 + lane) * 16) = x;
        if (CEM_LEAN_BKWAVE) {
            const f4 b = cem_ld_coherent(ho, (2 * 256 + lane) * 16);
            d_prev = b[0]; c_prev = b[1]; cum = b[2]; done = b[3] != 0.f;
        }
    } else {
        float pm[2][RC];
        pm[0][0] = __builtin_inff(); pm[1][0] = __builtin_inff();
        const int tv = tab_v;
        const f4 mn4 = CEM_TAB(tabl, CEM_ET_NMIN, tv), rd4 = CEM_TAB(tabl, CEM_ET_RDELTA, tv);
        const f4 isact4 = CEM_TAB(tabl, CEM_ET_ACT, tv);
        const f4 sel0 = CEM_TAB(tabl, CEM_ET_SEL0, tv), sel1 = CEM_TAB(tabl, CEM_ET_SEL1, tv);
        const f4 e0 = cem_normal4(pc0, 0u, (uint32_t)p.it, (uint32_t)zc, CEM_STREAM_ACT, key);
        const f4 sn = s[0][0];
        f4 xin = sn;
        if (wact) {
            f4 act4; CEM_LEAN_ACTION(act4, e0, 0);
            CEM_LEAN_KEEP(act4, 0);
            xin = __builtin_elementwise_fma(isact4, act4, sn);
        }
        cem_scorer_terms(sn, CEM_LEAN_SCORE_D, sel0, sel1, pm[0][0], pm[1][0]);
        const f4 x = cem_sub4(xin, mn4) * rd4;
        *reinterpret_cast<f4 *>(smem + (w * 64 + lane) * 16) = x;
        hB[0][0] = x;
        CEM_LEAN_STORE_TERMS;
    }
    f4 nb0 = cem_ld_tab(et_rs, bias_v, CEM_ET_ROWS * 512);
    f4 nb1 = cem_ld_tab(et_rs, bias_v + 64, CEM_ET_ROWS * 512);

    const char *rbh[6], *rb0[3];
#pragma unroll
    for (int k = 0; k < 6; ++k) rbh[k] = smem + lane * 16 + (k < 2 * w ? 0 : 2048);
#pragma unroll
    for (int k = 0; k < 3; ++k) rb0[k] = smem + lane * 16 + (k < w ? 0 : 1024);
    char *const pubh = smem + (2 * w * 64 + lane) * 16, *const pub0 = smem + (w * 64 + lane) * 16;
    CEM_LEAN_PRIO_DECL
    auto step = [&](auto XW0, const int t, const bool first) __attribute__((always_inline)) {
        int xw = decltype(XW0)::value;
        CEM_LEAN_PRIO_STEP
#define CEM_RELU_PUBLISH() do { \
            f4 h0 = acc0[0], h1 = acc1[0]; \
            _Pragma("unroll") for (int r = 0; r < 4; ++r) { h0[r] = fmaxf(h0[r], 0.f); h1[r] = fmaxf(h1[r], 0.f); } \
            *reinterpret_cast<f4 *>(pubh + xw) = h0; \
            *reinterpret_cast<f4 *>(pubh + xw + 1024) = h1; \
            hB[0][0] = h0; hB[1][0] = h1; \
            xw ^= XB; } while (0)
#define CEM_NEXT_BIAS(LN) do { \
            nb0 = cem_ld_tab(et_rs, bias_v, (CEM_ET_ROWS + (LN)) * 512); \
            nb1 = cem_ld_tab(et_rs, bias_v + 64, (CEM_ET_ROWS + (LN)) * 512); } while (0)
#define CEM_LEAN_HIDDEN(LN, BASE) { \
            f4 acc0[RC], acc1[RC]; \
            acc0[0] = nb0; acc1[0] = nb1; \
            CEM_NEXT_BIAS(LN); \
            CEM_LEAN_STAGE(CEM_NG, 2, false, BASE)(acc0, acc1, hB, wq, rbh, xw ^ XB); \
            CEM_RELU_PUBLISH(); }
        {
            f4 acc0[RC], acc1[RC];
            acc0[0] = nb0; acc1[0] = nb1;
            CEM_NEXT_BIAS(1);
            CEM_LEAN_STAGE(4, 1, true, 0)(acc0, acc1, hB, wq, rb0, xw ^ XB);
            CEM_LEAN_BOOKS_STEP
            CEM_RELU_PUBLISH();
        }
        CEM_LEAN_HIDDEN_LAYERS
#undef CEM_LEAN_HIDDEN
#undef CEM_RELU_PUBLISH
#undef CEM_NEXT_BIAS

        float pm[2][RC];
        pm[0][0] = __builtin_inff(); pm[1][0] = __builtin_inff();
        const int tn = (t + 1 < H) ? t + 1 : H - 1;
        {
            const int tv = tab_v;
            f4 accm[RC], accv[RC];
            accm[0] = CEM_TAB(tabl, CEM_ET_BMU, tv); accv[0] = CEM_TAB(tabl, CEM_ET_BVAR, tv);
            if (CEM_LEAN_HEADS) CEM_LEAN_STAGE(CEM_NG, 2, false, 28)(accm, accv, hB, wq, rbh, xw ^ XB);
            else __syncthreads();
            const f4 e4 = cem_normal4(pc0, pc1 + (uint32_t)t, 0u, pc2, 0u, key, prs);
            const f4 mn4 = CEM_TAB(tabl, CEM_ET_NMIN, tv), rd4 = CEM_TAB(tabl, CEM_ET_RDELTA, tv);
            const f4 om4 = CEM_TAB(tabl, CEM_ET_OBS, tv); CEM_LEAN_ISACT
            const f4 sel0 = CEM_TAB(tabl, CEM_ET_SEL0, tv), sel1 = CEM_TAB(tabl, CEM_ET_SEL1, tv);

            const f4 mu = accm[0];
            const f4 var = cem_softplus4(accv[0]) + 1e-4f;
            f4 sd;
#pragma unroll
            for (int r = 0; r < 4; ++r) sd[r] = __builtin_amdgcn_sqrtf(var[r]);
            const f4 d = mu + sd * e4;
            const f4 sn = s[0][0] + d * om4;
            s[0][0] = sn;
            cem_scorer_terms(sn, CEM_LEAN_SCORE_D, sel0, sel1, pm[0][0], pm[1][0]);
            CEM_LEAN_NEXT_INPUT
        }
        CEM_LEAN_STORE_TERMS;
    };
    for (int t = t_begin; t < t_end; t += 2) {
        step(LeanConst<XB>{}, t, t == t_begin);
        if (t + 1 >= t_end) break;
        step(LeanConst<0>{}, t + 1, false);
    }
    __syncthreads();
    CEM_LEAN_BOOKS_END
    if (td.row_base < p.Nloc) {
        const int tlo = resumed ? t_begin + 1 : 0, thi = t_end < H ? t_end : H - 1;
        const int per = (thi - tlo + 1) * A;
        const float *const stagef = reinterpret_cast<const float *>(stage);
        for (int idx = (int)threadIdx.x; idx < td.cnt * per; idx += 256) {
            const int row = idx / per, rem = idx - row * per, tt = tlo + rem / A, a = rem - (rem / A) * A;
            p.actions_w[((size_t)(td.act_base + row) * H + tt) * A + a] = stagef[((row * (H + 1) + tt) * AZ) * 4 + a];
        }
    }
    if (!SEG || t_end == H) {
        if (CEM_LEAN_BKWAVE && lane < td.cnt) p.ret[td.row_base + lane] = cum;
    } else {
        const __amdgpu_buffer_rsrc_t ho = CEM_LEAN_HANDOVER;
        cem_st_coherent(ho, tid * 16, s[0][0]);
        cem_st_coherent(ho, (256 + tid) * 16, hB[0][0]);
        if (CEM_LEAN_BKWAVE) cem_st_coherent(ho, (2 * 256 + lane) * 16, (f4){d_prev, c_prev, cum, done ? 1.0f : 0.0f});
    }
}
#undef CEM_LEAN_ACTION
#undef CEM_LEAN_KEEP
#undef CEM_LEAN_SEG_RSRC
#undef CEM_LEAN_TILE_TEMPLATE
#undef CEM_LEAN_TILE
#undef CEM_LEAN_HANDOVER_DECL
#undef CEM_LEAN_HANDOVER
#undef CEM_LEAN_BKWAVE
#undef CEM_LEAN_RING
#undef CEM_LEAN_STAGE
#undef CEM_LEAN_BOOKS_DECL
#undef CEM_LEAN_SCORE_D
#undef CEM_LEAN_STORE_TERMS
#undef CEM_LEAN_PRIO_DECL
#undef CEM_LEAN_PRIO_STEP
#undef CEM_LEAN_BOOKS_STEP
#undef CEM_LEAN_BOOKS_END
#undef CEM_LEAN_HIDDEN_LAYERS
#undef CEM_LEAN_HEADS
#undef CEM_LEAN_ISACT
#undef CEM_LEAN_NEXT_INPUT
```

### ethz_safe_learning_amd/planner.py

```python
from __future__ import annotations

import ctypes as C
import math
from dataclasses import dataclass, field
from typing import List, NamedTuple, Optional, Sequence, Tuple

import numpy as np

from . import _capi


@dataclass
class ScorerConfig:
    goal_slice: Tuple[int, int]
    observe_goal_lidar: bool = True
    lidar_max_dist: float = 4.0
    goal_size: float = 0.3
    reward_distance: float = 1.0
    reward_goal: float = 1.0
    reward_clip: float = 10.0
    constrain_indicator: bool = True
    cost_kinds: List[Tuple[int, int, float]] = field(default_factory=list)


# ... 324 lines not shown
    def _wait_inputs(self):
        self.stream.wait_stream(self._torch.cuda.current_stream(self.device))

    def stream_context(self):
        return self._torch.cuda.stream(self.stream)

    def synchronize(self):
        self.stream.synchronize()

    def _view(self, off, count, dtype, sync=True):
        t = self._torch
        if sync:
            self.stream.synchronize()
        nb = count * t.tensor([], dtype=dtype).element_size()
        return self._ws_view[off:off + nb].view(dtype)

    @property
    def n_local(self):
        return self.cfg.n_samples // self.cfg.world_size

    def scores_local(self, sync=True):
        return self._view(self.layout.scores_local, self.n_local, self._torch.float32, sync)

    def scores_global(self, sync=True):
        return self._view(self.layout.scores_global, self.cfg.n_samples, self._torch.float32, sync)

    def actions(self, sync=True):
        c = self.cfg
        return self._view(self.layout.actions, c.n_samples * c.horizon * c.act_dim, self._torch.float32, sync).view(
            c.n_samples, c.horizon, c.act_dim)

    def mu_sigma(self, sync=True):
        c = self.cfg
        return self._view(self.layout.mu_sigma, 2 * c.horizon * c.act_dim, self._torch.float32, sync).view(2, c.horizon, c.act_dim)

    def elite_idx(self, sync=True):
        return self._view(self.layout.elite_idx, self.cfg.n_elite, self._torch.int32, sync)

    def returns(self, sync=True):
        c = self.cfg
        return self._view(self.layout.returns, c.particles * self.n_local, self._torch.float32, sync).view(c.particles, self.n_local)

    def costs(self, sync=True):
        c = self.cfg
        return self._view(self.layout.costs, c.horizon * c.particles * self.n_local, self._torch.uint8, sync).view(
            c.horizon, c.particles, self.n_local)

    def result_block(self, sync=True):
        return self._view(self.layout.result, 38, self._torch.int32, sync)

    def set_weights(self, weights):
        blob = flatten_weights(weights)
        expect = self.lib.cem_weight_blob_floats(C.byref(self.ccfg))
        if blob.size != expect:
            raise ValueError('weight blob has %d floats, expected %d' % (blob.size, expect))
        _capi.check(self.lib.cem_planner_set_weights(self.h, _np_ptr(blob), blob.size), 'cem_planner_set_weights')
        self.have_device_weights = False

    def set_weights_dev(self, blob):
        t = self._torch
        if not (t.is_tensor(blob) and blob.is_cuda and blob.device == self.device and blob.dtype == t.float32 and blob.is_contiguous()):
            raise ValueError('set_weights_dev takes a contiguous float32 tensor on %s' % (self.device,))
        self._wait_inputs()
        _capi.check(self.lib.cem_planner_set_weights_dev(self.h, _ptr(blob), blob.numel()), 'cem_planner_set_weights_dev')
        blob.record_stream(self.stream)
        self.have_device_weights = True

    def set_weights_from(self, trainer):
        if trainer.device != self.device:
            self.set_weights(trainer.get_weights())
            return
        t = self._torch
        blob = trainer.weights_dev()
        if trainer.stream != self.stream:
            ev = t.cuda.Event()
            ev.record(trainer.stream)
            self.stream.wait_event(ev)
        _capi.check(self.lib.cem_planner_set_weights_dev(self.h, _ptr(blob), blob.numel()), 'cem_planner_set_weights_dev')
        if trainer.stream != self.stream:
            packed = t.cuda.Event()
            packed.record(self.stream)
            trainer.stream.wait_event(packed)
        self.have_device_weights = True

    def weight_images(self):
        t, lay, c = self._torch, self.layout, self.cfg
        sizes = dict(wpack=lay.wpack_bytes, bias_h=c.ensemble_size * c.n_layers * 512, bias_mu=c.ensemble_size * 512,
                     bias_var=c.ensemble_size * 512, etab=lay.etab_bytes)
        return {k: self._view(getattr(lay, k), n // 4, t.int32).cpu().numpy().view(np.uint32) for k, n in sizes.items()}

    def set_normaliser(self, inputs_min, inputs_max):
        mn = np.ascontiguousarray(np.asarray(inputs_min, np.float32))
        mx = np.ascontiguousarray(np.asarray(inputs_max, np.float32))
        if mn.shape != (self.cfg.obs_dim + self.cfg.act_dim,) or mx.shape != mn.shape:
            raise ValueError('normaliser must have shape [obs_dim + act_dim]')
        _capi.check(self.lib.cem_planner_set_normaliser(self.h, _np_ptr(mn), _np_ptr(mx)), 'cem_planner_set_normaliser')

    def comm_init(self, group=None):
        c = self.cfg
        buf = (C.c_char * _capi.CEM_COMM_ID_BYTES)()
        if c.world_size > 1:
            import torch.distributed as dist
            if not (dist.is_available() and dist.is_initialized()):
                raise RuntimeError('comm_init for world_size > 1 needs an initialised torch.distributed process group (it carries the id)')
            if dist.get_world_size(group) != c.world_size or dist.get_rank(group) != c.rank:
                raise ValueError('the process group does not match the planner\'s (world_size, rank)')
            box = [None]
            if c.rank == 0:
                _capi.check(self.lib.cem_comm_unique_id(buf), 'cem_comm_unique_id')
                box[0] = bytes(buf.raw)
            src = dist.get_global_rank(group, 0) if group is not None else 0
            dist.broadcast_object_list(box, src=src, group=group)
            buf.raw = box[0]
        else:
            _capi.check(self.lib.cem_comm_unique_id(buf), 'cem_comm_unique_id')
        with self._torch.cuda.device(self.device):
            _capi.check(self.lib.cem_planner_comm_init(self.h, buf, c.world_size, c.rank), 'cem_planner_comm_init')
        self.has_comm = True

    def comm_ranks(self):
        n = C.c_int32()
        _capi.check(self.lib.cem_planner_comm_ranks(self.h, C.byref(n)), 'cem_planner_comm_ranks')
        return n.value

    def comm_destroy(self):
        _capi.check(self.lib.cem_planner_comm_destroy(self.h), 'cem_planner_comm_destroy')
        self.has_comm = False

    def graph_status(self):
        st = C.c_int32()
        _capi.check(self.lib.cem_planner_graph_status(self.h, C.byref(st)), 'cem_planner_graph_status')
        return ('eager', 'graph', 'graph-unsupported')[st.value]

    def graph_nodes(self):
        n = C.c_int32()
        _capi.check(self.lib.cem_planner_graph_nodes(self.h, C.byref(n)), 'cem_planner_graph_nodes')
        return n.value

    def launches_per_iteration(self):
        n = C.c_int32()
        _capi.check(self.lib.cem_planner_launches_per_iteration(self.h, C.byref(n)), 'cem_planner_launches_per_iteration')
        return n.value

    def rollout_path(self):
        n = C.c_int32()
        _capi.check(self.lib.cem_planner_rollout_path(self.h, C.byref(n)), 'cem_planner_rollout_path')
        return ('generic', 'lean')[n.value]

    def rollout_form(self, it=0):
        n = C.c_int32()
        _capi.check(self.lib.cem_planner_rollout_form(self.h, int(it), C.byref(n)), 'cem_planner_rollout_form')
        return n.value

    def set_particle_objective(self, kind='mean', m=0):
        if kind not in PARTICLE_OBJECTIVES:
            raise ValueError("kind is 'mean' or 'lower_tail'")
        _capi.check(self.lib.cem_planner_set_particle_objective(self.h, PARTICLE_OBJECTIVES[kind], int(m)), 'cem_planner_set_particle_objective')

    def particle_objective(self):
        kind, m = C.c_int32(), C.c_int32()
        _capi.check(self.lib.cem_planner_get_particle_objective(self.h, C.byref(kind), C.byref(m)), 'cem_planner_get_particle_objective')
        return ('mean', 'lower_tail')[kind.value], m.value

    def set_constraint(self, kind='beta', worst_cost_particles=0):
        if kind not in CONSTRAINTS:
            raise ValueError("kind is 'beta' or 'budget'")
        _capi.check(self.lib.cem_planner_set_constraint(self.h, CONSTRAINTS[kind], int(worst_cost_particles)), 'cem_planner_set_constraint')

    def constraint(self):
        kind, m = C.c_int32(), C.c_int32()
        _capi.check(self.lib.cem_planner_get_constraint(self.h, C.byref(kind), C.byref(m)), 'cem_planner_get_constraint')
        return ('beta', 'budget')[kind.value], m.value

    def set_cost_budget(self, budget):
        b = np.ascontiguousarray(np.asarray(budget, np.float32).reshape(-1))
        self.budget_staged = None
        _capi.check(self.lib.cem_planner_set_cost_budget(self.h, _np_ptr(b), b.size), 'cem_planner_set_cost_budget')

    def constraint_costs(self, problem=0, n=None):
        out = np.zeros(self.n_local if n is None else int(n), np.float32)
        _capi.check(self.lib.cem_planner_constraint_costs(self.h, int(problem), _np_ptr(out), out.size), 'cem_planner_constraint_costs')
        return out

    def set_refit(self, kind='uniform', temperature=0.0):
        if kind not in REFITS:
            raise ValueError("kind is 'uniform' or 'softmax'")
        _capi.check(self.lib.cem_planner_set_refit(self.h, REFITS[kind], float(temperature)), 'cem_planner_set_refit')

    def refit(self):
        kind, t = C.c_int32(), C.c_float()
        _capi.check(self.lib.cem_planner_get_refit(self.h, C.byref(kind), C.byref(t)), 'cem_planner_get_refit')
        return ('uniform', 'softmax')[kind.value], t.value

    def refit_stats(self, problem=0, n=None):
        out = np.zeros(self.cfg.iterations if n is None else int(n), np.float32)
        _capi.check(self.lib.cem_planner_refit_stats(self.h, int(problem), _np_ptr(out), out.size), 'cem_planner_refit_stats')
        return out

    def set_action_noise(self, kind_or_matrix='white', param=None):
        H = self.cfg.horizon
        if isinstance(kind_or_matrix, str):
            M = mixing_matrix(kind_or_matrix, 0.0 if param is None else param, H)
        else:
            M = np.ascontiguousarray(np.asarray(kind_or_matrix, np.float32))
            if M.shape != (H, H):
                raise ValueError('the mixing matrix must have shape [%d, %d]' % (H, H))
        kind = _capi.CEM_NOISE_WHITE if M is None else _capi.CEM_NOISE_MIXED
        _capi.check(self.lib.cem_planner_set_action_noise(self.h, kind, _np_ptr(M)), 'cem_planner_set_action_noise')

    def action_noise(self):
        kind = C.c_int32()
        M = np.zeros((self.cfg.horizon, self.cfg.horizon), np.float32)
        _capi.check(self.lib.cem_planner_get_action_noise(self.h, C.byref(kind), _np_ptr(M)), 'cem_planner_get_action_noise')
        return ('white', None) if kind.value == _capi.CEM_NOISE_WHITE else ('mixed', M)

    def action_noise_floats(self):
        ptr, n = C.c_void_p(), C.c_size_t()
        _capi.check(self.lib.cem_planner_action_noise_dev(self.h, C.byref(ptr), C.byref(n)), 'cem_planner_action_noise_dev')
        return int(n.value) if ptr.value else 0

    def action_noise_tensor(self, problem=0):
        c, t = self.cfg, self._torch
        ptr, n = C.c_void_p(), C.c_size_t()
        _capi.check(self.lib.cem_planner_action_noise_dev(self.h, C.byref(ptr), C.byref(n)), 'cem_planner_action_noise_dev')
        per = c.iterations * c.n_samples * c.horizon * c.act_dim
        if not ptr.value:
            raise RuntimeError('the handle has no mixed action noise (set_action_noise was never given a matrix)')
        if not 0 <= int(problem) < n.value // per:
            raise ValueError('problem out of range')

        class _Dev:
            __cuda_array_interface__ = dict(shape=(per,), typestr='<f4', data=(ptr.value + 4 * per * int(problem), False), version=2)
        self.synchronize()
        with t.cuda.device(self.device):
            out = t.as_tensor(_Dev(), device=self.device).cpu().numpy().copy()
        return out.reshape(c.iterations, c.n_samples, c.horizon, c.act_dim)

    def set_elite_carry(self, n_keep, across_plans=False, shift=1):
        ec = _capi.CemEliteCarry(n_keep=int(n_keep), across_plans=int(bool(across_plans)), shift=int(shift), reserved=0)
        _capi.check(self.lib.cem_planner_set_elite_carry(self.h, C.byref(ec)), 'cem_planner_set_elite_carry')

    def elite_carry(self):
        ec = _capi.CemEliteCarry()
        _capi.check(self.lib.cem_planner_get_elite_carry(self.h, C.byref(ec)), 'cem_planner_get_elite_carry')
        return ec.n_keep, bool(ec.across_plans), ec.shift

    def elite_store(self, problem=0):
        c = self.cfg
        E = np.zeros((self.elite_carry()[0], c.horizon, c.act_dim), np.float32)
        n = C.c_int32()
        _capi.check(self.lib.cem_planner_elite_store(self.h, int(problem), _np_ptr(E), C.byref(n)), 'cem_planner_elite_store')
        return E, n.value

    def set_population_schedule(self, n=None):
        if n is None or len(n) == 0:
            _capi.check(self.lib.cem_planner_set_population_schedule(self.h, None, 0), 'cem_planner_set_population_schedule')
            return
        arr = (C.c_int32 * len(n))(*[int(x) for x in n])
        _capi.check(self.lib.cem_planner_set_population_schedule(self.h, arr, len(n)), 'cem_planner_set_population_schedule')

    def population_schedule(self):
        arr = (C.c_int32 * self.cfg.iterations)()
        on = C.c_int32()
        _capi.check(self.lib.cem_planner_get_population_schedule(self.h, arr, self.cfg.iterations, C.byref(on)), 'cem_planner_get_population_schedule')
        return list(arr), bool(on.value)

    def iteration_plan(self, it):
        ip = _capi.CemIterationPlan()
        _capi.check(self.lib.cem_planner_iteration_plan(self.h, int(it), C.byref(ip)), 'cem_planner_iteration_plan')
        return dict(n_samples=ip.n_samples, chunks_per_tile=ip.chunks_per_tile, n_tiles=ip.n_tiles, n_segments=ip.n_segments,
                    n_pinned=ip.n_pinned, launches=ip.launches, rollout_path='lean' if ip.rollout_path else 'generic')

    def set_mean_candidate(self, enable=True):
        _capi.check(self.lib.cem_planner_set_mean_candidate(self.h, 1 if enable else 0), 'cem_planner_set_mean_candidate')

    def mean_candidate(self):
        on = C.c_int32()
        _capi.check(self.lib.cem_planner_get_mean_candidate(self.h, C.byref(on)), 'cem_planner_get_mean_candidate')
        return bool(on.value)

    def set_plan_readout(self, on=True):
        _capi.check(self.lib.cem_planner_set_plan_readout(self.h, 1 if on else 0), 'cem_planner_set_plan_readout')

    def plan_readout_enabled(self):
        on = C.c_int32()
        _capi.check(self.lib.cem_planner_get_plan_readout(self.h, C.byref(on)), 'cem_planner_get_plan_readout')
        return bool(on.value)

    def plan_readout(self, problem=0) -> 'PlanReadout':
        c = self.cfg
        seq = np.zeros((c.horizon, c.act_dim), np.float32)
        pret = np.zeros(c.particles, np.float32)
        cnt = np.zeros(c.horizon, np.int32)
        head = _capi.CemPlanReadout()
        _capi.check(self.lib.cem_planner_plan_readout(self.h, int(problem), C.byref(head), _np_ptr(seq), _np_ptr(pret), _np_ptr(cnt)),
                    'cem_planner_plan_readout')
        return PlanReadout(seq, np.float32(head.score), int(head.candidate), int(head.iteration), pret, cnt, int(head.flags))

    def set_task(self, task=None):
        if task is None:
            _capi.check(self.lib.cem_planner_set_task(self.h, None), 'cem_planner_set_task')
            self.task = None
            return
        tb = task.tables(self.cfg.obs_dim, self.cfg.act_dim)
        fp = C.POINTER(C.c_float)
        ct = _capi.CemTask(kind=_capi.CEM_TASK_QUADRATIC, goal_radius=float(task.goal_radius), reward_goal=float(task.reward_goal),
# ... 605 lines not shown
```

### include/cem_mpc.h

```cpp
#ifndef CEM_MPC_H
#define CEM_MPC_H

#include <stddef.h>
#include <stdint.h>

#ifdef __cplusplus
extern "C" {
#endif

#define CEM_ABI_VERSION 4
#define CEM_MAX_ACT 32
#define CEM_MAX_COST_KINDS 4
#define CEM_MAX_BATCH 256

enum cem_status {
    CEM_OK = 0,
    CEM_ERR_INVALID_ARG = 1,
    CEM_ERR_UNSUPPORTED = 2,
    CEM_ERR_SPLIT = 3,
    CEM_ERR_WORKSPACE = 4,
    CEM_ERR_HIP = 5,
    CEM_ERR_NO_WEIGHTS = 6,
    CEM_ERR_STATE = 7,
    CEM_ERR_COMM = 8,
    CEM_ERR_DEVICE = 9
};

enum cem_variant { CEM_VARIANT_CEM = 0 , CEM_VARIANT_SAFE = 1 , CEM_VARIANT_COST = 2  };

enum cem_activation { CEM_ACT_RELU = 0, CEM_ACT_TANH = 1, CEM_ACT_SIGMOID = 2, CEM_ACT_ELU = 3, CEM_ACT_LEAKY_RELU = 4, CEM_ACT_SOFTPLUS = 5, CEM_ACT_SELU = 6,
                      CEM_ACT_SWISH = 7, CEM_ACT_GELU = 8 };

typedef struct cem_scorer {
    int32_t goal_mode;
    int32_t goal_lo, goal_hi;
    float lidar_max_dist;
    float goal_size;
    float goal_reached_dist;
    float reward_distance;
    float reward_goal;
    float reward_clip;
    int32_t constrain_indicator;
    int32_t n_cost_kinds;
    int32_t cost_lo[CEM_MAX_COST_KINDS];
    int32_t cost_hi[CEM_MAX_COST_KINDS];
    float cost_size[CEM_MAX_COST_KINDS];
} cem_scorer_t;

enum cem_precision { CEM_PRECISION_FP32 = 0, CEM_PRECISION_SPLIT_BF16X3 = 1, CEM_PRECISION_BF16 = 2 };

typedef struct cem_config {
    int32_t abi_version;
    int32_t obs_dim, act_dim;
    int32_t units, n_layers;
    int32_t activation;
    int32_t ensemble_size;
    int32_t particles;
    int32_t n_samples;
    int32_t horizon;
    int32_t n_elite;
    int32_t iterations;
    float smoothing;
    float one_minus_smoothing;
    float stddev_threshold;
    float noise_stddev;
    int32_t variant;
    float posterior_mean_threashold;
    int32_t sampling_propagation;
    int32_t scale_features;
    float act_lb[CEM_MAX_ACT], act_ub[CEM_MAX_ACT], act_mu0[CEM_MAX_ACT], act_sigma0[CEM_MAX_ACT];
    cem_scorer_t scorer;
    int32_t world_size, rank;
    int32_t chunks_per_tile;
    int32_t use_graph;
    int32_t select_mode;
    int32_t rollout_segments;
    int32_t precision;
} cem_config_t;

typedef struct cem_layout {
    size_t scores_local;
    size_t scores_global;
    size_t actions;
    size_t mu_sigma;
    size_t elite_idx;
    size_t returns;
    size_t costs;
    size_t result;
    size_t stamps;
    size_t total;
    size_t wpack, wpack_bytes;
    size_t bias_h;
    size_t bias_mu, bias_var;
    size_t etab, etab_bytes;
} cem_layout_t;

typedef struct cem_planner cem_planner_t;

int cem_abi_version(void);
const char *cem_status_string(int status);
int cem_last_hip_error(void);

size_t cem_weight_blob_floats(const cem_config_t *cfg);
size_t cem_packed_weight_floats(const cem_config_t *cfg);
size_t cem_workspace_bytes(const cem_config_t *cfg);

int cem_pack_weights_host(const cem_config_t *cfg, const float *blob, float *packed);
int cem_plan_tiles_host(const cem_config_t *cfg, int32_t *chunks_per_tile_out, int32_t *n_tiles_out,
                        int32_t *tiles_out , int32_t max_tiles);
int cem_plan_segments_host(const cem_config_t *cfg, int32_t *segments_out, int32_t *steps_per_segment_out);

int cem_rollout_residency(int32_t chunks_per_tile, int32_t input_blocks_per_wave, int32_t *table_out, int32_t *runtime_out);

int cem_planner_create(const cem_config_t *cfg, void *workspace, size_t workspace_bytes, void *hip_stream, cem_planner_t **out);
int cem_planner_destroy(cem_planner_t *h);
int cem_planner_layout(const cem_planner_t *h, cem_layout_t *out);

int cem_planner_set_weights(cem_planner_t *h, const float *blob, size_t n_floats);
int cem_planner_set_normaliser(cem_planner_t *h, const float *inputs_min, const float *inputs_max );
int cem_planner_set_weights_dev(cem_planner_t *h, const float *blob_dev, size_t n_floats);

int cem_planner_plan(cem_planner_t *h, const float *state, uint64_t seed, uint64_t call,
                     const float *eps_act_dev, const float *eps_model_dev, const float *eps_out_host,
                     float *action_out, float *best_score_out, int32_t *iters_out);

int cem_plan_begin(cem_planner_t *h, const float *state, uint64_t seed, uint64_t call,
                   const float *eps_act_dev, const float *eps_model_dev);
int cem_plan_rollout(cem_planner_t *h, int32_t it);
int cem_plan_select(cem_planner_t *h, int32_t it);
int cem_plan_end(cem_planner_t *h, const float *eps_out_host, float *action_out, float *best_score_out, int32_t *iters_out);

#define CEM_COMM_ID_BYTES 128
int cem_comm_unique_id(void *id_out );
int cem_planner_comm_init(cem_planner_t *h, const void *id , int32_t n_ranks, int32_t rank);
int cem_planner_comm_destroy(cem_planner_t *h);
int cem_planner_comm_ranks(const cem_planner_t *h, int32_t *n_ranks_out);
int cem_plan_exchange(cem_planner_t *h);
int cem_planner_select_mode(const cem_planner_t *h, int32_t *mode_out);
int cem_planner_inject_fault(cem_planner_t *h, int32_t kind);
int cem_planner_graph_status(const cem_planner_t *h, int32_t *status_out);
int cem_planner_graph_nodes(const cem_planner_t *h, int32_t *nodes_out);
int cem_planner_launches_per_iteration(const cem_planner_t *h, int32_t *launches_out);
int cem_planner_rollout_path(const cem_planner_t *h, int32_t *path_out);
int cem_planner_rollout_form(const cem_planner_t *h, int32_t it, int32_t *form_out);

int cem_unfold_sequences(cem_planner_t *h, const float *s0_dev, const float *actions_dev, int32_t n_rows, int32_t horizon,
                         const float *eps_model_dev, uint64_t seed, uint64_t call,
                         float *traj_out_dev, float *mu_out_dev, float *sd_out_dev);

int cem_compute_objective(cem_planner_t *h, const float *traj_dev, int32_t n_rows, int32_t horizon, float *scores_out_dev);

int cem_scorer_reward(cem_planner_t *h, const float *obs_dev, const float *next_obs_dev, int32_t n, float *reward_out_dev,
                      uint8_t *goal_achieved_out_dev);
int cem_scorer_cost(cem_planner_t *h, const float *obs_dev, int32_t n, float *cost_out_dev);

int cem_fill_noise(cem_planner_t *h, uint64_t seed, uint64_t call, float *eps_act_dev, float *eps_model_dev, float *eps_out_dev);

int cem_philox_words(cem_planner_t *h, uint64_t seed, uint64_t call, uint32_t stream, uint32_t iteration, uint32_t t, uint32_t sub,
                     uint32_t idx0, uint32_t n, uint32_t *words_out_dev);

int cem_planner_set_timing(cem_planner_t *h, int32_t enable);
int cem_planner_last_timing(cem_planner_t *h, float *rollout_ms_total, int32_t *rollout_launches, float *select_ms_total);
int cem_planner_last_timing_detail(cem_planner_t *h, float *reduce_ms_total, float *sampler_ms_total);

size_t cem_batch_workspace_bytes(const cem_config_t *cfg, int32_t max_batch);
int cem_batch_planner_create(const cem_config_t *cfg, int32_t max_batch, void *workspace, size_t workspace_bytes, void *hip_stream,
                             cem_planner_t **out);
int cem_planner_plan_batch(cem_planner_t *h, int32_t n_states, const float *states, uint64_t seed, const uint64_t *calls,
                           const float *eps_act_dev, const float *eps_model_dev, const float *eps_out_host, float *actions_out,
                           float *best_scores_out, int32_t *iters_out);
int cem_planner_batch_capacity(const cem_planner_t *h, int32_t *max_batch_out);

enum cem_init_mode { CEM_INIT_COLD = 0, CEM_INIT_EXPLICIT = 1, CEM_INIT_SHIFT = 2 };
typedef struct cem_warm_start {
    int32_t shift;
    int32_t tail;
    int32_t sigma_rule;
    float sigma_floor[CEM_MAX_ACT];
} cem_warm_start_t;
int cem_planner_set_warm_start(cem_planner_t *h, const cem_warm_start_t *ws);
int cem_planner_set_initial_distribution(cem_planner_t *h, int32_t slot, const float *mu, const float *sigma);
int cem_planner_set_init_mode(cem_planner_t *h, int32_t slot, int32_t mode);
int cem_planner_reset_carry(cem_planner_t *h, int32_t slot);
int cem_planner_get_carry(cem_planner_t *h, int32_t slot, float *mu, float *sigma, int32_t *valid);
int cem_planner_set_carry_slots(cem_planner_t *h, int32_t n, const int32_t *slots);

enum cem_particle_objective { CEM_PARTICLES_MEAN = 0, CEM_PARTICLES_LOWER_TAIL = 1 };
int cem_planner_set_particle_objective(cem_planner_t *h, int32_t kind, int32_t m);
int cem_planner_get_particle_objective(const cem_planner_t *h, int32_t *kind_out, int32_t *m_out);

enum cem_constraint_kind { CEM_CONSTRAINT_BETA = 0, CEM_CONSTRAINT_BUDGET = 1 };
int cem_planner_set_constraint(cem_planner_t *h, int32_t kind, int32_t worst_cost_particles);
int cem_planner_get_constraint(const cem_planner_t *h, int32_t *kind_out, int32_t *worst_cost_particles_out);
int cem_planner_set_cost_budget(cem_planner_t *h, const float *budgets, int32_t n);
int cem_planner_constraint_costs(cem_planner_t *h, int32_t problem, float *out_host, int32_t n);

#if defined(__HIPCC__)
#define CEM_INLINE static inline __host__ __device__
#else
#define CEM_INLINE static inline
#endif
#define CEM_INFEASIBLE_BELOW (-0x1p100f)
CEM_INLINE float cem_f32_encode_infeasible(int32_t total) { return -((float)(8388608 + total)) * 0x1p77f; }
CEM_INLINE int cem_f32_score_is_feasible(float score) { return score > CEM_INFEASIBLE_BELOW; }
CEM_INLINE int32_t cem_f32_decode_infeasible(float score) { return (int32_t)(-score * 0x1p-77f) - 8388608; }

enum cem_refit { CEM_REFIT_UNIFORM = 0, CEM_REFIT_SOFTMAX = 1 };
int cem_planner_set_refit(cem_planner_t *h, int32_t kind, float temperature);
int cem_planner_get_refit(const cem_planner_t *h, int32_t *kind_out, float *temperature_out);
int cem_planner_refit_stats(cem_planner_t *h, int32_t problem, float *ess_out_host, int32_t n);

enum cem_action_noise { CEM_NOISE_WHITE = 0, CEM_NOISE_MIXED = 1 };
int cem_planner_set_action_noise(cem_planner_t *h, int32_t kind, const float *mix_host );
int cem_planner_get_action_noise(const cem_planner_t *h, int32_t *kind_out, float *mix_out_host );
int cem_planner_action_noise_dev(cem_planner_t *h, const float **eps_dev_out, size_t *n_floats_out);

typedef struct { int32_t n_keep, across_plans, shift, reserved; } cem_elite_carry_t;
int cem_planner_set_elite_carry(cem_planner_t *h, const cem_elite_carry_t *carry);
int cem_planner_get_elite_carry(const cem_planner_t *h, cem_elite_carry_t *carry_out);
int cem_planner_elite_store(cem_planner_t *h, int32_t problem, float *out_host , int32_t *count_out);

int cem_planner_set_population_schedule(cem_planner_t *h, const int32_t *n , int32_t count);
int cem_planner_get_population_schedule(const cem_planner_t *h, int32_t *n_out , int32_t count, int32_t *enabled_out);
typedef struct { int32_t n_samples, chunks_per_tile, n_tiles, n_segments, n_pinned, launches, rollout_path, reserved; } cem_iteration_plan_t;
int cem_planner_iteration_plan(const cem_planner_t *h, int32_t it, cem_iteration_plan_t *out);

int cem_planner_set_mean_candidate(cem_planner_t *h, int32_t enable);
int cem_planner_get_mean_candidate(const cem_planner_t *h, int32_t *enable_out);

typedef struct { float score; int32_t candidate, iteration, flags; } cem_plan_readout_t;
int cem_planner_set_plan_readout(cem_planner_t *h, int32_t enable);
int cem_planner_get_plan_readout(const cem_planner_t *h, int32_t *enable_out);
int cem_planner_plan_readout(cem_planner_t *h, int32_t problem, cem_plan_readout_t *out,
                             float *sequence_out_host ,
                             float *particle_returns_out_host ,
                             int32_t *cost_counts_out_host );

enum cem_task_kind { CEM_TASK_SAFETY_GYM = 0, CEM_TASK_QUADRATIC = 1 };
typedef struct {
    int32_t kind;
    const float *q, *g, *c, *goal_mask, *lo, *hi;
    const float *rho;
    float goal_radius, reward_goal, reward_clip;
} cem_task_t;
int cem_planner_set_task(cem_planner_t *h, const cem_task_t *task);
int cem_planner_task_trajectories(cem_planner_t *h, float *out_dev);
int cem_task_score(cem_planner_t *h, const float *traj_dev, const float *actions_dev, int32_t n_rows, int32_t horizon,
                   float *ret_out_dev, uint8_t *costs_out_dev);

#define CEM_TRAIN_MAX_BATCH 4096
typedef struct cem_train_config {
    int32_t abi_version;
    int32_t inputs_dim, outputs_dim, units, n_layers, ensemble_size;
    int32_t batch_size;
    int32_t activation;
    float dropout_rate;
    uint32_t dropout_seed_lo, dropout_seed_hi;
    float beta1, beta2, epsilon, clipvalue;
} cem_train_config_t;
typedef struct cem_trainer cem_trainer_t;

size_t cem_trainer_workspace_bytes(const cem_train_config_t *cfg);
size_t cem_trainer_blob_floats(const cem_train_config_t *cfg);
int cem_trainer_create(const cem_train_config_t *cfg, void *workspace, size_t workspace_bytes, void *hip_stream, cem_trainer_t **out);
int cem_trainer_destroy(cem_trainer_t *h);
int cem_trainer_set_state(cem_trainer_t *h, const float *weights, const float *m, const float *v);
int cem_trainer_get_state(cem_trainer_t *h, float *weights, float *m, float *v);
int cem_trainer_weights_dev(cem_trainer_t *h, const float **blob_dev_out, size_t *n_floats_out);
int cem_trainer_step(cem_trainer_t *h, const float *x_dev, const float *y_dev, const int32_t *perm_dev, int32_t nperm,
                     int32_t offset, int32_t bt, float lr_t, float *loss_dev);
int cem_trainer_steps(cem_trainer_t *h, const float *x_dev, const float *y_dev, const int32_t *perm_dev, int32_t nperm,
                      int32_t n_steps, const int32_t *offsets, const int32_t *bts, const float *lr_ts, float *loss_dev);
int cem_trainer_eval(cem_trainer_t *h, const float *x_dev, const float *y_dev, int32_t n, float *loss_out);

enum cem_forward_map { CEM_FORWARD_SPLIT = 0, CEM_FORWARD_ALL = 1 };
int cem_trainer_forward(cem_trainer_t *h, const float *x_dev, int32_t n_rows, int32_t map, const float *eps_dev, uint64_t seed, uint64_t call,
                        float *mu_out_dev, float *var_out_dev, float *sd_out_dev, float *sample_out_dev);

#ifdef __cplusplus
}
#endif
#endif
```

Baseline: 553.9.

## Add resident lean rollout kernel holding table rows in registers with unrolled priority rounds

```diff
diff --git a/ethz_safe_learning_amd/_capi.py b/ethz_safe_learning_amd/_capi.py
--- a/ethz_safe_learning_amd/_capi.py
+++ b/ethz_safe_learning_amd/_capi.py
@@ -26,7 +26,7 @@
     'cem_packed_weight_floats', 'cem_workspace_bytes', 'cem_pack_weights_host', 'cem_plan_tiles_host', 'cem_plan_segments_host', 'cem_rollout_residency',
     'cem_planner_create', 'cem_planner_destroy', 'cem_planner_layout', 'cem_planner_set_weights', 'cem_planner_set_weights_dev',
     'cem_planner_set_normaliser', 'cem_planner_plan', 'cem_plan_begin', 'cem_plan_rollout', 'cem_plan_select',
-    'cem_plan_end', 'cem_comm_unique_id', 'cem_planner_comm_init', 'cem_planner_comm_destroy', 'cem_planner_comm_ranks', 'cem_plan_exchange', 'cem_planner_graph_status', 'cem_planner_graph_nodes', 'cem_planner_launches_per_iteration', 'cem_planner_rollout_path', 'cem_planner_rollout_form', 'cem_unfold_sequences', 'cem_compute_objective', 'cem_scorer_reward', 'cem_scorer_cost', 'cem_fill_noise', 'cem_philox_words', 'cem_planner_set_timing', 'cem_planner_last_timing', 'cem_planner_last_timing_detail', 'cem_planner_select_mode', 'cem_planner_inject_fault',
+    'cem_plan_end', 'cem_comm_unique_id', 'cem_planner_comm_init', 'cem_planner_comm_destroy', 'cem_planner_comm_ranks', 'cem_plan_exchange', 'cem_planner_graph_status', 'cem_planner_graph_nodes', 'cem_planner_launches_per_iteration', 'cem_planner_rollout_path', 'cem_planner_rollout_form', 'cem_planner_lean_form', 'cem_unfold_sequences', 'cem_compute_objective', 'cem_scorer_reward', 'cem_scorer_cost', 'cem_fill_noise', 'cem_philox_words', 'cem_planner_set_timing', 'cem_planner_last_timing', 'cem_planner_last_timing_detail', 'cem_planner_select_mode', 'cem_planner_inject_fault',
     'cem_batch_workspace_bytes', 'cem_batch_planner_create', 'cem_planner_plan_batch', 'cem_planner_batch_capacity',
     'cem_planner_set_warm_start', 'cem_planner_set_initial_distribution', 'cem_planner_set_init_mode', 'cem_planner_reset_carry',
     'cem_planner_get_carry', 'cem_planner_set_carry_slots', 'cem_planner_set_particle_objective', 'cem_planner_get_particle_objective',
@@ -160,6 +160,7 @@
     lib.cem_planner_launches_per_iteration.argtypes = [vp, i32p]
     lib.cem_planner_rollout_path.argtypes = [vp, i32p]
     lib.cem_planner_rollout_form.argtypes = [vp, C.c_int32, i32p]
+    lib.cem_planner_lean_form.argtypes = [vp, C.c_int32, i32p]
     lib.cem_compute_objective.argtypes = [vp, vp, C.c_int32, C.c_int32, vp]
     lib.cem_scorer_reward.argtypes = [vp, vp, vp, C.c_int32, vp, vp]
     lib.cem_scorer_cost.argtypes = [vp, vp, C.c_int32, vp]
diff --git a/ethz_safe_learning_amd/csrc/cem_capi.hip b/ethz_safe_learning_amd/csrc/cem_capi.hip
--- a/ethz_safe_learning_amd/csrc/cem_capi.hip
+++ b/ethz_safe_learning_amd/csrc/cem_capi.hip
@@ -640,6 +640,7 @@
     bool sample_in_rollout;
     bool lean_rollout;
     bool lean_branchy;
+    bool lean_straight;
     const float *eps_act, *eps_model;
     CtrlBlock *h_ctrl;
     float *h_result;
@@ -722,7 +723,8 @@
     const Dims &d = *iter_view(h, it).d; const ScorerDev &sc = h->sc_roll;
     bool straight = launch_rollout_lean_straight != nullptr && !h->lean_branchy && !sc.goal_mode && sc.n_cost <= 1 && d.L == 4 && d.NFW == 1;
     for (int w = 0; w < 4; ++w) straight = straight && d.wave_groups[w] == 4 + 3 * CEM_NG + (w < d.KB_obs ? CEM_NG : 0);
-    return straight ? 2 : 1;
+    if (!straight) return 1;
+    return launch_rollout_lean_resident != nullptr && !h->lean_straight ? 3 : 2;
 }
 size_t task_tab_floats() { return (size_t)CEM_TASK_TABLES * CEM_U; }
 float *task_traj(const cem_planner *h) { return h->task_dev + task_tab_floats(); }
@@ -972,7 +974,8 @@
     }
     { const Plan pl = make_plan(cfg, h->d, mb); h->rc = pl.rc; h->n_seg = pl.n_seg; h->seg_len = pl.seg_len; h->n_pinned = pl.n_pinned;
       place_sampler(h, h->d, pl, &h->sample_in_rollout, &h->lean_rollout); }
-    { const char *e = std::getenv("CEM_FORCE_ROLLOUT"); h->lean_branchy = e && std::strcmp(e, "lean_branchy") == 0; }
+    { const char *e = std::getenv("CEM_FORCE_ROLLOUT"); h->lean_branchy = e && std::strcmp(e, "lean_branchy") == 0;
+      h->lean_straight = e && std::strcmp(e, "lean_straight") == 0; }
     h->have_weights = false; h->in_plan = false; h->eps_act = h->eps_model = nullptr;
     h->timing = false; h->roll_ms = h->sel_ms = h->red_ms = h->samp_ms = 0.f; h->roll_n = 0;
     h->graph = nullptr; h->gexec = nullptr; h->graph_ready = false;
@@ -1447,7 +1450,9 @@
     };
     if (rc.lean_form) {
         const int grid = queued ? queue_grid() : v.n_tiles;
-        if (rc.lean_form == 2 && (rp.variant == 1) == (rp.costs != nullptr)) HIPCHK(launch_rollout_lean_straight(rp, grid, h->stream, queued));
+        const bool fixed_objective = (rp.variant == 1) == (rp.costs != nullptr);
+        if (rc.lean_form == 3 && fixed_objective) HIPCHK(launch_rollout_lean_resident(rp, grid, h->stream, queued));
+        else if (rc.lean_form >= 2 && fixed_objective) HIPCHK(launch_rollout_lean_straight(rp, grid, h->stream, queued));
         else HIPCHK(launch_rollout_lean(rp, grid, h->stream, queued));
     }
     else if (d.wide) HIPCHK(launch_rollout_wide(h, rp, v.n_tiles, mode1 ? 1 : 0));
@@ -2450,6 +2455,13 @@
 int cem_planner_rollout_form(const cem_planner_t *h, int32_t it, int32_t *form_out)
 {
     if (!h || !form_out || it < 0 || it >= h->d.I) return CEM_ERR_INVALID_ARG;
+    *form_out = std::min(recipe_of(h, it, false).lean_form, 2);
+    return CEM_OK;
+}
+
+int cem_planner_lean_form(const cem_planner_t *h, int32_t it, int32_t *form_out)
+{
+    if (!h || !form_out || it < 0 || it >= h->d.I) return CEM_ERR_INVALID_ARG;
     *form_out = recipe_of(h, it, false).lean_form;
     return CEM_OK;
 }
diff --git a/ethz_safe_learning_amd/csrc/cem_rollout_lean.h b/ethz_safe_learning_amd/csrc/cem_rollout_lean.h
--- a/ethz_safe_learning_amd/csrc/cem_rollout_lean.h
+++ b/ethz_safe_learning_amd/csrc/cem_rollout_lean.h
@@ -7,5 +7,13 @@
 
 __attribute__((weak)) hipError_t launch_rollout_lean(const RolloutParams &p, int grid, hipStream_t st, bool seg);
 __attribute__((weak)) hipError_t launch_rollout_lean_straight(const RolloutParams &p, int grid, hipStream_t st, bool seg);
+__attribute__((weak)) hipError_t launch_rollout_lean_resident(const RolloutParams &p, int grid, hipStream_t st, bool seg);
 
 template <int V> struct LeanConst { static constexpr int value = V; };
+
+#define CEM_LEAN_TWO_STEP_ROUNDS(...) \
+    for (int t = t_begin; t < t_end; t += 2) { \
+        step(LeanConst<XB>{}, t, t == t_begin __VA_ARGS__); \
+        if (t + 1 >= t_end) break; \
+        step(LeanConst<0>{}, t + 1, false __VA_ARGS__); \
+    }
diff --git a/ethz_safe_learning_amd/csrc/cem_rollout_lean.hip b/ethz_safe_learning_amd/csrc/cem_rollout_lean.hip
--- a/ethz_safe_learning_amd/csrc/cem_rollout_lean.hip
+++ b/ethz_safe_learning_amd/csrc/cem_rollout_lean.hip
@@ -49,6 +49,10 @@
         const int lvl = (t + prio_r0) % 3; \
         if (lvl == 0) __builtin_amdgcn_s_setprio(0); else if (lvl == 1) __builtin_amdgcn_s_setprio(1); else __builtin_amdgcn_s_setprio(2); \
     }
+#define CEM_LEAN_STEP_ARGS
+#define CEM_LEAN_STEP_LOOP CEM_LEAN_TWO_STEP_ROUNDS()
+#define CEM_LEAN_TAB_DECL
+#define CEM_LEAN_TAB(ROW) CEM_TAB(tabl, ROW, tv)
 #define CEM_LEAN_BOOKS_AT(T_) CEM_BOOKKEEP(p, td, part, w, wbk, lane, nk, csz, ind_cap, clipv, cost_rs, d_prev, c_prev, cum, done, T_);
 #define CEM_LEAN_BOOKS_STEP if (!(resumed && first)) CEM_LEAN_BOOKS_AT(t - 1)
 #define CEM_LEAN_BOOKS_END CEM_LEAN_BOOKS_AT(t_end - 1)
diff --git a/ethz_safe_learning_amd/csrc/cem_rollout_lean_resident.hip b/ethz_safe_learning_amd/csrc/cem_rollout_lean_resident.hip
--- /dev/null
+++ b/ethz_safe_learning_amd/csrc/cem_rollout_lean_resident.hip
@@ -0,0 +1,132 @@
+#define CEM_DEVICE_PRIMITIVES_ONLY
+#include "cem_rollout_lean.h"
+
+#ifndef CEM_RESIDENT_ROUND
+#define CEM_RESIDENT_ROUND 1
+#endif
+#ifndef CEM_RESIDENT_QUADS
+#define CEM_RESIDENT_QUADS 3
+#endif
+
+namespace {
+
+#include "cem_rollout_lean_straight.h"
+#define CEM_LEAN_TILE_TEMPLATE template <bool SEG, bool SAFE, bool FLT>
+#define CEM_LEAN_TILE cem_resident_tile
+#if CEM_RESIDENT_ROUND
+#define CEM_LEAN_PRIO_DECL \
+    static_assert(CEM_FLOAT_PRIO == 3 && !(FLT && !SEG), "a floating segment stays on the priority its kernel set"); \
+    const int lvl0 = __builtin_amdgcn_readfirstlane((t_begin + (tile_idx >> 8) % 3) % 3);
+#define CEM_LEAN_STEP_ARGS , auto LVL
+#define CEM_LEAN_PRIO_STEP if constexpr (decltype(LVL)::value >= 0) __builtin_amdgcn_s_setprio(decltype(LVL)::value);
+#define CEM_RESIDENT_STEP(XW_, LVL_) { step(LeanConst<XW_>{}, t, t == t_begin, LeanConst<LVL_>{}); if (++t >= t_end) break; }
+#define CEM_RESIDENT_STEP_ODD(LVL_) { step(LeanConst<0>{}, t, false, LeanConst<LVL_>{}); if (++t >= t_end) break; }
+#define CEM_LEAN_STEP_LOOP \
+    if constexpr (FLT) { CEM_LEAN_TWO_STEP_ROUNDS(, LeanConst<-1>{}) } \
+    else if (t_begin < t_end) { \
+        int t = t_begin, skip = lvl0 == 0 ? 0 : (lvl0 == 2 ? 1 : 2);       \
+        for (;;) { \
+            if (skip < 1) { CEM_RESIDENT_STEP(XB, 0) CEM_RESIDENT_STEP_ODD(1) } \
+            if (skip < 2) { CEM_RESIDENT_STEP(XB, 2) CEM_RESIDENT_STEP_ODD(0) } \
+            CEM_RESIDENT_STEP(XB, 1) CEM_RESIDENT_STEP_ODD(2) \
+            skip = 0; \
+        } \
+    }
+#else
+#define CEM_LEAN_PRIO_DECL \
+    static_assert(CEM_FLOAT_PRIO == 3, "level 3 of the step's priority switch is the floating segments' priority"); \
+    int lvl = (SEG && tile_idx >= p.n_pinned) ? 3 : (t_begin + (tile_idx >> 8) % 3) % 3;
+#define CEM_LEAN_PRIO_STEP \
+    if (lvl < 2) { if (lvl == 0) __builtin_amdgcn_s_setprio(0); else __builtin_amdgcn_s_setprio(1); } \
+    else { if (lvl == 2) __builtin_amdgcn_s_setprio(2); else __builtin_amdgcn_s_setprio(3); } \
+    lvl = lvl == 2 ? 0 : (lvl == 3 ? 3 : lvl + 1); \
+    asm volatile("" : "+s"(lvl));
+#define CEM_LEAN_STEP_ARGS
+#define CEM_LEAN_STEP_LOOP CEM_LEAN_TWO_STEP_ROUNDS()
+#endif
+#define CEM_RESIDENT_HOLD(ROW) const f4 held_##ROW = CEM_TAB(tabl, ROW, tab_v);
+#define CEM_LEAN_TAB(ROW) (held_##ROW)
+#if CEM_RESIDENT_QUADS >= 1
+#define CEM_RESIDENT_HOLD_1 CEM_RESIDENT_HOLD(CEM_ET_NMIN)
+#else
+#define CEM_RESIDENT_HOLD_1
+#define held_CEM_ET_NMIN CEM_TAB(tabl, CEM_ET_NMIN, tv)
+#endif
+#if CEM_RESIDENT_QUADS >= 2
+#define CEM_RESIDENT_HOLD_2 CEM_RESIDENT_HOLD(CEM_ET_RDELTA)
+#else
+#define CEM_RESIDENT_HOLD_2
+#define held_CEM_ET_RDELTA CEM_TAB(tabl, CEM_ET_RDELTA, tv)
+#endif
+#if CEM_RESIDENT_QUADS >= 3
+#define CEM_RESIDENT_HOLD_3 CEM_RESIDENT_HOLD(CEM_ET_OBS)
+#else
+#define CEM_RESIDENT_HOLD_3
+#define held_CEM_ET_OBS CEM_TAB(tabl, CEM_ET_OBS, tv)
+#endif
+#if CEM_RESIDENT_QUADS >= 4
+#define CEM_RESIDENT_HOLD_4 CEM_RESIDENT_HOLD(CEM_ET_BMU)
+#else
+#define CEM_RESIDENT_HOLD_4
+#define held_CEM_ET_BMU CEM_TAB(tabl, CEM_ET_BMU, tv)
+#endif
+#if CEM_RESIDENT_QUADS >= 5
+#define CEM_RESIDENT_HOLD_5 CEM_RESIDENT_HOLD(CEM_ET_BVAR)
+#else
+#define CEM_RESIDENT_HOLD_5
+#define held_CEM_ET_BVAR CEM_TAB(tabl, CEM_ET_BVAR, tv)
+#endif
+#if CEM_RESIDENT_QUADS >= 6
+#define CEM_RESIDENT_HOLD_6 CEM_RESIDENT_HOLD(CEM_ET_SEL0)
+#else
+#define CEM_RESIDENT_HOLD_6
+#define held_CEM_ET_SEL0 CEM_TAB(tabl, CEM_ET_SEL0, tv)
+#endif
+#if CEM_RESIDENT_QUADS >= 7
+#define CEM_RESIDENT_HOLD_7 CEM_RESIDENT_HOLD(CEM_ET_SEL1)
+#else
+#define CEM_RESIDENT_HOLD_7
+#define held_CEM_ET_SEL1 CEM_TAB(tabl, CEM_ET_SEL1, tv)
+#endif
+#define CEM_LEAN_TAB_DECL CEM_RESIDENT_HOLD_1 CEM_RESIDENT_HOLD_2 CEM_RESIDENT_HOLD_3 CEM_RESIDENT_HOLD_4 CEM_RESIDENT_HOLD_5 CEM_RESIDENT_HOLD_6 CEM_RESIDENT_HOLD_7
+#include "cem_rollout_lean_tile.h"
+#undef CEM_RESIDENT_STEP
+#undef CEM_RESIDENT_STEP_ODD
+#undef CEM_RESIDENT_HOLD
+
+}
+
+template <bool SAFE>
+__global__ __launch_bounds__(256) void cem_rollout_lean_resident_kernel(const RolloutParams p)
+{
+    extern __shared__ __attribute__((aligned(16))) char smem[];
+    if (p.check_done && p.ctrl->done) return;
+    cem_resident_tile<false, SAFE, false>(p, smem, (int)blockIdx.x, 0, p.H);
+}
+
+template <bool SAFE>
+__global__ __launch_bounds__(256) void cem_rollout_lean_resident_seg_kernel(const RolloutParams p)
+{
+    extern __shared__ __attribute__((aligned(16))) char smem[];
+    __shared__ uint32_t item_s;
+    if (p.check_done && p.ctrl->done) return;
+    if ((int)blockIdx.x < p.n_pinned) {
+        cem_resident_tile<true, SAFE, false>(p, smem, (int)blockIdx.x, 0, p.H);
+        return;
+    }
+    CEM_SEG_SCHEDULE(p, item_s, tile, seg, t0, t1, (cem_resident_tile<true, SAFE, CEM_RESIDENT_ROUND != 0>(p, smem, tile, t0, t1)))
+}
+
+hipError_t launch_rollout_lean_resident(const RolloutParams &p, int grid, hipStream_t st, bool seg)
+{
+    const size_t lds = CEM_LEAN_LDS_BYTES(p.H, (p.A + 3) / 4);
+    const bool safe = p.variant == 1;
+    if (seg) {
+        if (safe) hipLaunchKernelGGL(cem_rollout_lean_resident_seg_kernel<true>, dim3(grid), dim3(256), lds, st, p);
+        else hipLaunchKernelGGL(cem_rollout_lean_resident_seg_kernel<false>, dim3(grid), dim3(256), lds, st, p);
+    } else {
+        if (safe) hipLaunchKernelGGL(cem_rollout_lean_resident_kernel<true>, dim3(grid), dim3(256), lds, st, p);
+        else hipLaunchKernelGGL(cem_rollout_lean_resident_kernel<false>, dim3(grid), dim3(256), lds, st, p);
+    }
+    return hipGetLastError();
+}
diff --git a/ethz_safe_learning_amd/csrc/cem_rollout_lean_straight.h b/ethz_safe_learning_amd/csrc/cem_rollout_lean_straight.h
--- /dev/null
+++ b/ethz_safe_learning_amd/csrc/cem_rollout_lean_straight.h
@@ -0,0 +1,121 @@
+
+constexpr int SL_GROUPS_BODY = 4 + 3 * CEM_NG, SL_GROUPS_HEADS = SL_GROUPS_BODY + CEM_NG;
+
+struct StraightRing {
+    __amdgpu_buffer_rsrc_t rsrc;
+    int voff, n;
+    AGroup slot[4];
+    template <int G> __device__ __forceinline__ AGroup ld() const
+    {
+        const int g = G < SL_GROUPS_BODY ? G : (G >= n ? G - n : G);
+        const int soff = (g >> 1) * 4096;
+        constexpr int half = (G & 1) * 2048;
+        AGroup r;
+        r.a = __builtin_bit_cast(f4, __builtin_amdgcn_raw_buffer_load_b128(rsrc, voff + half, soff, 0));
+        r.b = __builtin_bit_cast(f4, __builtin_amdgcn_raw_buffer_load_b128(rsrc, voff + half + 1024, soff, 0));
+        return r;
+    }
+    __device__ __forceinline__ void init(const f4 *b, int lane_, int n_)
+    {
+        rsrc = __builtin_amdgcn_make_buffer_rsrc(const_cast<f4 *>(b), 0, n_ * 2048, 0x00020000);
+        voff = lane_ * 16; n = n_;
+        slot[0] = ld<0>(); slot[1] = ld<1>(); slot[2] = ld<2>(); slot[3] = slot[2];
+    }
+};
+
+template <int KF, int NOWN, bool L0IN, int BASE>
+__device__ __forceinline__ void cem_straight_stage(f4 (&acc0)[1], f4 (&acc1)[1], f4 (&hB)[CEM_NG][1], StraightRing &wq, const char *const *rb, const int xoff)
+{
+    static_assert(KF % 4 == 0 && BASE % 4 == 0, "stage lengths must keep the ring phase");
+    auto group = [&](auto PC) __attribute__((always_inline)) {
+        constexpr int P = decltype(PC)::value;
+        wq.slot[(P + 3) & 3] = wq.template ld<BASE + P + 3>();
+        __builtin_amdgcn_sched_barrier(0);
+        if (P == 1) {
+            __syncthreads();
+#pragma unroll
+            for (int Q = NOWN; Q < KF; ++Q) hB[Q][0] = *reinterpret_cast<const f4 *>(rb[Q - NOWN] + xoff + (Q - NOWN) * 1024);
+        }
+        const AGroup g = wq.slot[P & 3];
+        constexpr int Pb = (!L0IN && P < 2) ? (P ^ 1) : P;
+#pragma unroll
+        for (int r = 0; r < 4; ++r) {
+            acc0[0] = CEM_MFMA(g.a[r], hB[P][0][r], acc0[0]);
+            acc1[0] = CEM_MFMA(g.b[r], hB[Pb][0][r], acc1[0]);
+        }
+    };
+    group(LeanConst<0>{}); group(LeanConst<1>{}); group(LeanConst<2>{}); group(LeanConst<3>{});
+    if constexpr (KF == 8) { group(LeanConst<4>{}); group(LeanConst<5>{}); group(LeanConst<6>{}); group(LeanConst<7>{}); }
+}
+
+#define CEM_LEAN_BKWAVE bkwave
+#define CEM_LEAN_HANDOVER_DECL const bool bkwave = w == 0; auto seg_buffer = [&]() __attribute__((always_inline)) { return CEM_LEAN_SEG_RSRC(); };
+#define CEM_LEAN_HANDOVER seg_buffer()
+#define CEM_LEAN_RING \
+    const bool heads = w < p.KB_obs; \
+    StraightRing wq; \
+    wq.init(p.wpack + (size_t)member_u * p.member_stride_f4 + p.wave_off_f4[w], lane, heads ? SL_GROUPS_HEADS : SL_GROUPS_BODY);
+#define CEM_LEAN_STAGE(KF, NOWN, L0IN, BASE) cem_straight_stage<KF, NOWN, L0IN, BASE>
+#define CEM_LEAN_BOOKS_DECL \
+    const float scD = p.sc.D, goal_thresh = p.sc.goal_thresh, reward_distance = p.sc.reward_distance, reward_goal = p.sc.reward_goal; \
+    const float clipv = p.sc.reward_clip > 0.f ? p.sc.reward_clip : __builtin_inff(); \
+    const float csz0 = p.sc.n_cost > 0 ? p.sc.cost_size[0] : -__builtin_inff(); \
+    auto terms = [&](float &dn, float &cn) __attribute__((always_inline)) { \
+        dn = CEM_PART_MIN4(part, lane, 0); \
+        const float dk = CEM_PART_MIN4(part, lane, 1); \
+        cn = (dk <= csz0) ? 1.0f : 0.0f;                       \
+    }; \
+    auto settle = [&](const float dn, const float cn, const int T) __attribute__((always_inline)) { \
+        const bool ga = d_prev <= goal_thresh; \
+        float r = (d_prev - dn) * reward_distance + (ga ? 1.0f : 0.0f) * reward_goal; \
+        r = fminf(fmaxf(r, -clipv), clipv); \
+        if (SAFE) { \
+            done = done || ga; \
+            const float nd = done ? 0.0f : 1.0f; \
+            const float cst = c_prev * nd; \
+            if (lane < td.cnt) { \
+                const __amdgpu_buffer_rsrc_t cost_rs = __builtin_amdgcn_make_buffer_rsrc(p.costs, 0, (uint32_t)(H * p.Bloc), 0x00020000); \
+                __builtin_amdgcn_raw_buffer_store_b8((uint8_t)cst, cost_rs, td.row_base + lane, __builtin_amdgcn_readfirstlane(T * p.Bloc), 0); \
+            } \
+            cum = cum + r * nd; \
+        } else { \
+            const float nd = done ? 0.0f : 1.0f; \
+            cum = cum + r * nd; \
+            done = done || ga; \
+        } \
+        d_prev = dn; c_prev = cn; \
+    };
+#define CEM_LEAN_SCORE_D scD
+#define CEM_LEAN_STORE_TERMS CEM_PAIR_MIN_STORE(part, w, q, j, 0, pm[0][0], pm[1][0], true, 0)
+#define CEM_LEAN_BOOKS_STEP \
+    if (bkwave) { \
+        if (first) { \
+            if (!resumed) terms(d_prev, c_prev); \
+        } else { \
+            float dn, cn; \
+            terms(dn, cn); \
+            settle(dn, cn, t - 1); \
+        } \
+    }
+#define CEM_LEAN_BOOKS_END \
+    if (bkwave) { \
+        float dn, cn; \
+        terms(dn, cn); \
+        settle(dn, cn, t_end - 1); \
+    }
+#define CEM_LEAN_HIDDEN_LAYERS CEM_LEAN_HIDDEN(2, 4) CEM_LEAN_HIDDEN(3, 12) CEM_LEAN_HIDDEN(0, 20)
+#define CEM_LEAN_HEADS heads
+#define CEM_LEAN_ISACT
+#define CEM_LEAN_NEXT_INPUT \
+    if (wact) { \
+        const f4 isact4 = CEM_TAB(tabl, CEM_ET_ACT, tv); \
+        f4 act4; CEM_LEAN_ACTION(act4, e4, tn); \
+        CEM_LEAN_KEEP(act4, t + 1); \
+        const f4 x = cem_sub4(__builtin_elementwise_fma(isact4, act4, sn), mn4) * rd4; \
+        *reinterpret_cast<f4 *>(pub0 + xw) = x; \
+        hB[0][0] = x; \
+    } else { \
+        const f4 x = cem_sub4(sn, mn4) * rd4; \
+        *reinterpret_cast<f4 *>(pub0 + xw) = x; \
+        hB[0][0] = x; \
+    }
diff --git a/ethz_safe_learning_amd/csrc/cem_rollout_lean_straight.hip b/ethz_safe_learning_amd/csrc/cem_rollout_lean_straight.hip
--- a/ethz_safe_learning_amd/csrc/cem_rollout_lean_straight.hip
+++ b/ethz_safe_learning_amd/csrc/cem_rollout_lean_straight.hip
@@ -3,96 +3,9 @@
 
 namespace {
 
-constexpr int SL_GROUPS_BODY = 4 + 3 * CEM_NG, SL_GROUPS_HEADS = SL_GROUPS_BODY + CEM_NG;
-
-struct StraightRing {
-    __amdgpu_buffer_rsrc_t rsrc;
-    int voff, n;
-    AGroup slot[4];
-    template <int G> __device__ __forceinline__ AGroup ld() const
-    {
-        const int g = G < SL_GROUPS_BODY ? G : (G >= n ? G - n : G);
-        const int soff = (g >> 1) * 4096;
-        constexpr int half = (G & 1) * 2048;
-        AGroup r;
-        r.a = __builtin_bit_cast(f4, __builtin_amdgcn_raw_buffer_load_b128(rsrc, voff + half, soff, 0));
-        r.b = __builtin_bit_cast(f4, __builtin_amdgcn_raw_buffer_load_b128(rsrc, voff + half + 1024, soff, 0));
-        return r;
-    }
-    __device__ __forceinline__ void init(const f4 *b, int lane_, int n_)
-    {
-        rsrc = __builtin_amdgcn_make_buffer_rsrc(const_cast<f4 *>(b), 0, n_ * 2048, 0x00020000);
-        voff = lane_ * 16; n = n_;
-        slot[0] = ld<0>(); slot[1] = ld<1>(); slot[2] = ld<2>(); slot[3] = slot[2];
-    }
-};
-
-template <int KF, int NOWN, bool L0IN, int BASE>
-__device__ __forceinline__ void cem_straight_stage(f4 (&acc0)[1], f4 (&acc1)[1], f4 (&hB)[CEM_NG][1], StraightRing &wq, const char *const *rb, const int xoff)
-{
-    static_assert(KF % 4 == 0 && BASE % 4 == 0, "stage lengths must keep the ring phase");
-    auto group = [&](auto PC) __attribute__((always_inline)) {
-        constexpr int P = decltype(PC)::value;
-        wq.slot[(P + 3) & 3] = wq.template ld<BASE + P + 3>();
-        __builtin_amdgcn_sched_barrier(0);
-        if (P == 1) {
-            __syncthreads();
-#pragma unroll
-            for (int Q = NOWN; Q < KF; ++Q) hB[Q][0] = *reinterpret_cast<const f4 *>(rb[Q - NOWN] + xoff + (Q - NOWN) * 1024);
-        }
-        const AGroup g = wq.slot[P & 3];
-        constexpr int Pb = (!L0IN && P < 2) ? (P ^ 1) : P;
-#pragma unroll
-        for (int r = 0; r < 4; ++r) {
-            acc0[0] = CEM_MFMA(g.a[r], hB[P][0][r], acc0[0]);
-            acc1[0] = CEM_MFMA(g.b[r], hB[Pb][0][r], acc1[0]);
-        }
-    };
-    group(LeanConst<0>{}); group(LeanConst<1>{}); group(LeanConst<2>{}); group(LeanConst<3>{});
-    if constexpr (KF == 8) { group(LeanConst<4>{}); group(LeanConst<5>{}); group(LeanConst<6>{}); group(LeanConst<7>{}); }
-}
-
+#include "cem_rollout_lean_straight.h"
 #define CEM_LEAN_TILE_TEMPLATE template <bool SEG, bool SAFE>
 #define CEM_LEAN_TILE cem_straight_tile
-#define CEM_LEAN_BKWAVE bkwave
-#define CEM_LEAN_HANDOVER_DECL const bool bkwave = w == 0; auto seg_buffer = [&]() __attribute__((always_inline)) { return CEM_LEAN_SEG_RSRC(); };
-#define CEM_LEAN_HANDOVER seg_buffer()
-#define CEM_LEAN_RING \
-    const bool heads = w < p.KB_obs; \
-    StraightRing wq; \
-    wq.init(p.wpack + (size_t)member_u * p.member_stride_f4 + p.wave_off_f4[w], lane, heads ? SL_GROUPS_HEADS : SL_GROUPS_BODY);
-#define CEM_LEAN_STAGE(KF, NOWN, L0IN, BASE) cem_straight_stage<KF, NOWN, L0IN, BASE>
-#define CEM_LEAN_BOOKS_DECL \
-    const float scD = p.sc.D, goal_thresh = p.sc.goal_thresh, reward_distance = p.sc.reward_distance, reward_goal = p.sc.reward_goal; \
-    const float clipv = p.sc.reward_clip > 0.f ? p.sc.reward_clip : __builtin_inff(); \
-    const float csz0 = p.sc.n_cost > 0 ? p.sc.cost_size[0] : -__builtin_inff(); \
-    auto terms = [&](float &dn, float &cn) __attribute__((always_inline)) { \
-        dn = CEM_PART_MIN4(part, lane, 0); \
-        const float dk = CEM_PART_MIN4(part, lane, 1); \
-        cn = (dk <= csz0) ? 1.0f : 0.0f;                       \
-    }; \
-    auto settle = [&](const float dn, const float cn, const int T) __attribute__((always_inline)) { \
-        const bool ga = d_prev <= goal_thresh; \
-        float r = (d_prev - dn) * reward_distance + (ga ? 1.0f : 0.0f) * reward_goal; \
-        r = fminf(fmaxf(r, -clipv), clipv); \
-        if (SAFE) { \
-            done = done || ga; \
-            const float nd = done ? 0.0f : 1.0f; \
-            const float cst = c_prev * nd; \
-            if (lane < td.cnt) { \
-                const __amdgpu_buffer_rsrc_t cost_rs = __builtin_amdgcn_make_buffer_rsrc(p.costs, 0, (uint32_t)(H * p.Bloc), 0x00020000); \
-                __builtin_amdgcn_raw_buffer_store_b8((uint8_t)cst, cost_rs, td.row_base + lane, __builtin_amdgcn_readfirstlane(T * p.Bloc), 0); \
-            } \
-            cum = cum + r * nd; \
-        } else { \
-            const float nd = done ? 0.0f : 1.0f; \
-            cum = cum + r * nd; \
-            done = done || ga; \
-        } \
-        d_prev = dn; c_prev = cn; \
-    };
-#define CEM_LEAN_SCORE_D scD
-#define CEM_LEAN_STORE_TERMS CEM_PAIR_MIN_STORE(part, w, q, j, 0, pm[0][0], pm[1][0], true, 0)
 #define CEM_LEAN_PRIO_DECL \
     static_assert(CEM_FLOAT_PRIO == 3, "level 3 of the step's priority switch is the floating segments' priority"); \
     int lvl = (SEG && tile_idx >= p.n_pinned) ? 3 : (t_begin + (tile_idx >> 8) % 3) % 3;
@@ -101,38 +14,10 @@
     else { if (lvl == 2) __builtin_amdgcn_s_setprio(2); else __builtin_amdgcn_s_setprio(3); } \
     lvl = lvl == 2 ? 0 : (lvl == 3 ? 3 : lvl + 1); \
     asm volatile("" : "+s"(lvl));
-#define CEM_LEAN_BOOKS_STEP \
-    if (bkwave) { \
-        if (first) { \
-            if (!resumed) terms(d_prev, c_prev); \
-        } else { \
-            float dn, cn; \
-            terms(dn, cn); \
-            settle(dn, cn, t - 1); \
-        } \
-    }
-#define CEM_LEAN_BOOKS_END \
-    if (bkwave) { \
-        float dn, cn; \
-        terms(dn, cn); \
-        settle(dn, cn, t_end - 1); \
-    }
-#define CEM_LEAN_HIDDEN_LAYERS CEM_LEAN_HIDDEN(2, 4) CEM_LEAN_HIDDEN(3, 12) CEM_LEAN_HIDDEN(0, 20)
-#define CEM_LEAN_HEADS heads
-#define CEM_LEAN_ISACT
-#define CEM_LEAN_NEXT_INPUT \
-    if (wact) { \
-        const f4 isact4 = CEM_TAB(tabl, CEM_ET_ACT, tv); \
-        f4 act4; CEM_LEAN_ACTION(act4, e4, tn); \
-        CEM_LEAN_KEEP(act4, t + 1); \
-        const f4 x = cem_sub4(__builtin_elementwise_fma(isact4, act4, sn), mn4) * rd4; \
-        *reinterpret_cast<f4 *>(pub0 + xw) = x; \
-        hB[0][0] = x; \
-    } else { \
-        const f4 x = cem_sub4(sn, mn4) * rd4; \
-        *reinterpret_cast<f4 *>(pub0 + xw) = x; \
-        hB[0][0] = x; \
-    }
+#define CEM_LEAN_STEP_ARGS
+#define CEM_LEAN_STEP_LOOP CEM_LEAN_TWO_STEP_ROUNDS()
+#define CEM_LEAN_TAB_DECL
+#define CEM_LEAN_TAB(ROW) CEM_TAB(tabl, ROW, tv)
 #include "cem_rollout_lean_tile.h"
 
 }
diff --git a/ethz_safe_learning_amd/csrc/cem_rollout_lean_tile.h b/ethz_safe_learning_amd/csrc/cem_rollout_lean_tile.h
--- a/ethz_safe_learning_amd/csrc/cem_rollout_lean_tile.h
+++ b/ethz_safe_learning_amd/csrc/cem_rollout_lean_tile.h
@@ -125,7 +125,8 @@
     for (int k = 0; k < 3; ++k) rb0[k] = smem + lane * 16 + (k < w ? 0 : 1024);
     char *const pubh = smem + (2 * w * 64 + lane) * 16, *const pub0 = smem + (w * 64 + lane) * 16;
     CEM_LEAN_PRIO_DECL
-    auto step = [&](auto XW0, const int t, const bool first) __attribute__((always_inline)) {
+    CEM_LEAN_TAB_DECL
+    auto step = [&](auto XW0, const int t, const bool first CEM_LEAN_STEP_ARGS) __attribute__((always_inline)) {
         int xw = decltype(XW0)::value;
         CEM_LEAN_PRIO_STEP
 #define CEM_RELU_PUBLISH() do { \
@@ -163,13 +164,13 @@
         {
             const int tv = tab_v;
             f4 accm[RC], accv[RC];
-            accm[0] = CEM_TAB(tabl, CEM_ET_BMU, tv); accv[0] = CEM_TAB(tabl, CEM_ET_BVAR, tv);
+            accm[0] = CEM_LEAN_TAB(CEM_ET_BMU); accv[0] = CEM_LEAN_TAB(CEM_ET_BVAR);
             if (CEM_LEAN_HEADS) CEM_LEAN_STAGE(CEM_NG, 2, false, 28)(accm, accv, hB, wq, rbh, xw ^ XB);
             else __syncthreads();
             const f4 e4 = cem_normal4(pc0, pc1 + (uint32_t)t, 0u, pc2, 0u, key, prs);
-            const f4 mn4 = CEM_TAB(tabl, CEM_ET_NMIN, tv), rd4 = CEM_TAB(tabl, CEM_ET_RDELTA, tv);
-            const f4 om4 = CEM_TAB(tabl, CEM_ET_OBS, tv); CEM_LEAN_ISACT
-            const f4 sel0 = CEM_TAB(tabl, CEM_ET_SEL0, tv), sel1 = CEM_TAB(tabl, CEM_ET_SEL1, tv);
+            const f4 mn4 = CEM_LEAN_TAB(CEM_ET_NMIN), rd4 = CEM_LEAN_TAB(CEM_ET_RDELTA);
+            const f4 om4 = CEM_LEAN_TAB(CEM_ET_OBS); CEM_LEAN_ISACT
+            const f4 sel0 = CEM_LEAN_TAB(CEM_ET_SEL0), sel1 = CEM_LEAN_TAB(CEM_ET_SEL1);
 
             const f4 mu = accm[0];
             const f4 var = cem_softplus4(accv[0]) + 1e-4f;
@@ -184,11 +185,7 @@
         }
         CEM_LEAN_STORE_TERMS;
     };
-    for (int t = t_begin; t < t_end; t += 2) {
-        step(LeanConst<XB>{}, t, t == t_begin);
-        if (t + 1 >= t_end) break;
-        step(LeanConst<0>{}, t + 1, false);
-    }
+    CEM_LEAN_STEP_LOOP
     __syncthreads();
     CEM_LEAN_BOOKS_END
     if (td.row_base < p.Nloc) {
@@ -224,6 +221,10 @@
 #undef CEM_LEAN_STORE_TERMS
 #undef CEM_LEAN_PRIO_DECL
 #undef CEM_LEAN_PRIO_STEP
+#undef CEM_LEAN_STEP_ARGS
+#undef CEM_LEAN_STEP_LOOP
+#undef CEM_LEAN_TAB_DECL
+#undef CEM_LEAN_TAB
 #undef CEM_LEAN_BOOKS_STEP
 #undef CEM_LEAN_BOOKS_END
 #undef CEM_LEAN_HIDDEN_LAYERS
diff --git a/ethz_safe_learning_amd/planner.py b/ethz_safe_learning_amd/planner.py
--- a/ethz_safe_learning_amd/planner.py
+++ b/ethz_safe_learning_amd/planner.py
@@ -500,6 +500,11 @@
         _capi.check(self.lib.cem_planner_rollout_form(self.h, int(it), C.byref(n)), 'cem_planner_rollout_form')
         return n.value
 
+    def lean_form(self, it=0):
+        n = C.c_int32()
+        _capi.check(self.lib.cem_planner_lean_form(self.h, int(it), C.byref(n)), 'cem_planner_lean_form')
+        return n.value
+
     def set_particle_objective(self, kind='mean', m=0):
         if kind not in PARTICLE_OBJECTIVES:
             raise ValueError("kind is 'mean' or 'lower_tail'")
diff --git a/include/cem_mpc.h b/include/cem_mpc.h
--- a/include/cem_mpc.h
+++ b/include/cem_mpc.h
@@ -143,6 +143,7 @@
 int cem_planner_launches_per_iteration(const cem_planner_t *h, int32_t *launches_out);
 int cem_planner_rollout_path(const cem_planner_t *h, int32_t *path_out);
 int cem_planner_rollout_form(const cem_planner_t *h, int32_t it, int32_t *form_out);
+int cem_planner_lean_form(const cem_planner_t *h, int32_t it, int32_t *form_out);
 
 int cem_unfold_sequences(cem_planner_t *h, const float *s0_dev, const float *actions_dev, int32_t n_rows, int32_t horizon,
                          const float *eps_model_dev, uint64_t seed, uint64_t call,
```

Result: no change. 557.7, median of 6 (+0.7%).
